# hmakelin/gisnav

Hardware: AMD Instinct MI355X
Metric: matched frame-pairs/sec + PnP poses/sec, 640x480 cam-vs-tile (higher is better)
Workload: dtype f32-accurate FFN / out-projection / match-head GEMMs (each f32 operand split into 2 fp16 terms = 22 significant bits, 3 fp16 MFMA partial products, f32 accumulate; fp16-range guard active); attention INPUT projections (q, k, v: 18 of 66 launches) on 2 partial products -- the fp16 high term of the ac

## Files before the change

gisnav_amd/_lib.py:

```python
from __future__ import annotations

import ctypes as C
import os

HERE = os.path.dirname(os.path.abspath(__file__))
LIB_PATH = os.environ.get("GISNAV_AMD_LIB") or os.path.join(HERE, "libgisnav_amd.so")

c_f32p = C.POINTER(C.c_float)
c_f64p = C.POINTER(C.c_double)
c_i32p = C.POINTER(C.c_int32)
c_i64p = C.POINTER(C.c_int64)
c_u8p = C.POINTER(C.c_uint8)
VP = C.c_void_p

SIGNATURES = {
    "gn_version": (C.c_char_p, []),
    "gn_last_error": (C.c_char_p, [VP]),
    "gn_create": (C.c_int, [C.c_int, C.c_int, C.c_int, C.c_int, C.POINTER(VP)]),
    "gn_create_ex": (C.c_int, [C.c_int, C.c_int, C.c_int, C.c_int, C.c_int, C.POINTER(VP)]),
    "gn_set_image_size": (C.c_int, [VP, C.c_float, C.c_float, C.c_float, C.c_float]),
    "gn_resize": (C.c_int, [VP, C.c_int]),
    "gn_destroy": (None, [VP]),
    "gn_load_tensor": (C.c_int, [VP, C.c_char_p, VP, c_i64p, C.c_int]),
    "gn_missing_tensors": (C.c_int, [VP]),
# ... 13 lines not shown
                                    VP, VP, VP, VP, C.c_double, VP, VP, VP, VP]),
    "gn_estimate_cov": (C.c_int, [VP, C.c_int, C.c_int, VP, VP, VP, C.c_int, VP, VP, VP, C.c_int, VP, C.c_int, C.c_int,
                                  c_f64p, C.c_int, VP, VP, VP, VP, VP, C.c_double, VP, VP, VP, VP]),
    "gn_pnp_ransac_report": (C.c_int, [VP, C.c_int, VP, VP, VP, C.c_int, c_f64p, C.c_int, C.c_float, C.c_double, C.c_int,
                                       VP, VP, VP, VP, C.c_double, VP, VP, VP, VP, VP, VP, VP]),
    "gn_estimate_report": (C.c_int, [VP, C.c_int, C.c_int, VP, VP, VP, C.c_int, VP, VP, VP, C.c_int, VP, C.c_int, C.c_int,
                                     c_f64p, C.c_int, VP, VP, VP, VP, VP, C.c_double, VP, VP, VP, VP, VP, VP, VP, VP, VP]),
    "gn_set_distortion": (C.c_int, [VP, c_f64p, C.c_int]),
    "gn_get_distortion": (C.c_int, [VP, c_f64p]),
    "gn_gather_points_scored": (C.c_int, [VP, C.c_int, C.c_int, VP, C.c_int, VP, C.c_int, VP, VP, VP, VP, C.c_int, C.c_int, VP, VP, VP]),
    "gn_set_dem_format": (C.c_int, [VP, C.c_int, C.c_double, C.c_double, C.c_int, C.c_double]),
    "gn_get_dem_format": (C.c_int, [VP, C.POINTER(C.c_int), c_f64p, c_f64p, C.POINTER(C.c_int), c_f64p]),
    "gn_dem_last_dropped": (C.c_int, [VP, C.c_int, c_i32p, VP]),
    "gn_set_ransac": (C.c_int, [VP, C.c_int, C.c_float, C.c_double]),
    "gn_get_ransac": (C.c_int, [VP, C.POINTER(C.c_int), c_f32p, c_f64p]),
    "gn_ransac_last_counts": (C.c_int, [VP, C.c_int, c_i32p, c_i32p, VP]),
    "gn_undistort_points": (C.c_int, [VP, C.c_int, VP, VP, C.c_int, c_f64p, C.c_int, VP, VP]),
    "gn_set_pair_cameras": (C.c_int, [VP, VP, C.c_int, C.c_int]),
    "gn_get_pair_cameras": (C.c_int, [VP, C.POINTER(VP), C.POINTER(C.c_int), C.POINTER(C.c_int)]),
    "gn_set_overlap": (C.c_int, [VP, C.c_int]),
    "gn_flush": (C.c_int, [VP, VP]),
    "gn_set_substreams": (C.c_int, [VP, C.c_int]),
    "gn_set_active_kpts": (C.c_int, [VP, C.c_int]),
    "gn_set_deferred_join": (C.c_int, [VP, C.c_int]),
    "gn_set_guard": (C.c_int, [VP, C.c_int]),
    "gn_get_guard_status": (C.c_int, [VP, VP, C.POINTER(C.c_int32), C.POINTER(C.c_int64)]),
    "gn_set_certify": (C.c_int, [VP, C.c_int, C.c_float, C.c_float]),
    "gn_set_ffn_products": (C.c_int, [VP, C.c_int]),
    "gn_get_ffn_level": (C.c_int, [VP, C.POINTER(C.c_int32), c_f32p, c_f32p, c_i64p]),
    "gn_set_ffn_level_eps": (C.c_int, [VP, C.c_float, C.c_float, C.c_int]),
    "gn_get_ffn_level1": (C.c_int, [VP, c_f32p, c_i64p]),
    "gn_set_ffn_level_eps1": (C.c_int, [VP, C.c_float]),
    "gn_debug_ffn_level_sim": (C.c_int, [C.c_int, C.c_int, VP, VP, VP, C.c_int, VP, VP]),
    "gn_fused_projection_status": (C.c_int, [VP]),
    "gn_device_numa_node": (C.c_int, [C.c_int]),
    "gn_get_certify_stats": (C.c_int, [VP, c_i64p]),
    "gn_reset_certify_stats": (C.c_int, [VP]),
    "gn_set_certify_ladder": (C.c_int, [VP, C.c_int, C.c_float]),
    "gn_get_certify_ladder_stats": (C.c_int, [VP, c_i64p]),
    "gn_calibrate_certify": (C.c_int, [VP, C.c_int, C.c_int, VP, VP, VP, C.c_int, VP, VP, VP, C.c_int, C.c_float, C.c_float, c_f32p, c_f32p, VP]),
    "gn_get_uncertain": (C.c_int, [VP, C.c_int, c_i32p, VP]),
    "gn_source_digest": (C.c_char_p, []),
    "gn_vo_match": (C.c_int, [VP, C.c_int, VP, VP, C.c_int, VP, VP, C.c_int, C.c_double, VP, VP, VP, VP, VP, VP]),
    "gn_vo_estimate": (C.c_int, [VP, C.c_int, C.c_int, VP, VP, VP, C.c_int, VP, VP, VP, C.c_int, c_f64p, C.c_double, C.c_int,
                                 VP, VP, VP, VP, VP, VP]),
    "gn_vo_estimate_cov": (C.c_int, [VP, C.c_int, C.c_int, VP, VP, VP, C.c_int, VP, VP, VP, C.c_int, c_f64p, C.c_double, C.c_int,
                                     VP, VP, VP, VP, VP, C.c_double, VP, VP, VP, VP]),
    "gn_vo_estimate_report": (C.c_int, [VP, C.c_int, C.c_int, VP, VP, VP, C.c_int, VP, VP, VP, C.c_int, c_f64p, C.c_double, C.c_int,
                                        VP, VP, VP, VP, VP, C.c_double, VP, VP, VP, VP, VP, VP, VP, VP, VP]),
    "gn_rotate_crop_center": (C.c_int, [VP, VP, C.c_int, C.c_int, C.c_double, C.c_int, C.c_int, VP, c_f64p, VP]),
    "gn_stereo_reference_dem": (C.c_int, [VP, VP, VP, C.c_int, C.c_int, C.c_double, C.c_int, C.c_int, C.c_double, C.c_int, C.c_int, VP, VP, c_f64p, VP]),
    "gn_stereo_reference": (C.c_int, [VP, VP, VP, C.c_int, C.c_int, C.c_double, C.c_int, C.c_int, VP, VP, c_f64p, VP]),
    "gn_proj_to_affine": (C.c_int, [C.c_char_p, c_f64p]),
    "gn_wgs84_to_ecef": (C.c_int, [C.c_double, C.c_double, C.c_double, c_f64p]),
    "gn_pose_to_earth": (C.c_int, [c_f64p, c_f64p, c_f64p, C.c_int, C.c_int, c_f64p, c_f64p, c_f64p]),
    "gn_pose_cov_to_camera": (C.c_int, [c_f64p, c_f64p, c_f64p, c_f64p]),
    "gn_pose_cov_to_earth": (C.c_int, [c_f64p, c_f64p, c_f64p, c_f64p, C.c_int, C.c_int, c_f64p]),
    "gn_sift_detect_and_compute": (C.c_int, [VP, VP, C.c_int, C.c_int, C.c_int, VP, VP, VP, VP, C.POINTER(C.c_int32), VP]),
    "gn_sift_detect_and_compute_batch": (C.c_int, [VP, VP, C.c_int, C.c_int, C.c_int, C.c_int, VP, VP, VP, VP, C.POINTER(C.c_int32), VP]),
    "gn_sift_last_totals": (C.c_int, [VP, C.c_int, C.POINTER(C.c_int32)]),
    "gn_sift_set_params": (C.c_int, [VP, C.c_int, C.c_double, C.c_double, C.c_double]),
    "gn_sift_get_params": (C.c_int, [VP, C.POINTER(C.c_int), c_f64p, c_f64p, c_f64p]),
    "gn_sp_load_tensor": (C.c_int, [VP, C.c_char_p, VP, c_i64p, C.c_int]),
    "gn_sp_detect_and_describe": (C.c_int, [VP, VP, C.c_int, C.c_int, C.c_int, C.c_int, VP, VP, VP, C.POINTER(C.c_int32), VP]),
    "gn_sp_set_arithmetic": (C.c_int, [VP, C.c_int]),
    "gn_loftr_create": (C.c_int, [C.c_int, C.c_int, C.c_int, C.c_int, C.c_int, C.POINTER(VP)]),
# ... 86 lines not shown
```

gisnav_amd/csrc/gn_api.hip:

```cpp
#include "gn_common.h"

#include <cstdio>
#include <cstring>
#include <cmath>
#include <cctype>
#include <algorithm>
#include <memory>
#include <tuple>

using namespace gn;

namespace {

thread_local std::string g_err;

struct Linear { float* w = nullptr; float* b = nullptr; int out = 0, in = 0; uint16_t* wp = nullptr; float acc_scale = 1.f;
                uint16_t* wf = nullptr; int frag_order = -1;
                uint16_t* wf2 = nullptr;
                uint16_t* wfn = nullptr; };

struct Block {
  Linear proj_in;
  Linear proj_out;
  Linear ffn0;
// ... 44 lines not shown
  o.B = n;
  pair_arrays(o, [&](size_t bytes, bool, auto*& p) { if (p) p = byte_offset(p, b0 * bytes); }, o);
  return o;
}

template <typename... T> struct Restore {
  std::tuple<T&...> ref; std::tuple<T...> val;
  explicit Restore(T&... r) : ref(r...), val(r...) {}
  ~Restore() { ref = val; }
  Restore(const Restore&) = delete;
  Restore& operator=(const Restore&) = delete;
};

enum { kWsAlways = 1, kWsF16x2 = 2 , kWsNotF32 = 4 , kWsFirstUse = 8 , kWsPnpStage = 16  };
inline long long lists_stride_of(long long km) { return gn::kTileListBase + 2 * (km / 128) + 8 * ((km + 255) / 256); }
#define GN_WORKSPACES(X)                                                                                                         \
  X(float, desc, T2 * kInDim, kWsAlways, "desc") X(float, cos_t, T2 * kFreq, kWsAlways, "cos") X(float, sin_t, T2 * kFreq, kWsAlways, "sin") \
  X(float, extent, 4, kWsAlways, "extent") X(int32_t, nvalid, 2, kWsAlways, "nvalid")                                            \
  X(float, x, T2 * kDim, kWsAlways, "x") X(float, qkv, T2 * 3 * kDim, kWsAlways, "qkv") X(float, ctx, T2 * kDim, kWsAlways, "ctx") \
  X(float, msg, T2 * kDim, kWsAlways, "msg") X(float, h, T2 * 2 * kDim, kWsAlways, "h") X(float, md, T2 * kDim, kWsAlways, "md") \
  X(float, ls, T2, kWsAlways, "ls")                                                                                              \
            \
  X(uint16_t, desc_p, 2 * T2 * kInDim, kWsF16x2, "desc_p") X(uint16_t, x_p, 2 * T2 * kDim, kWsF16x2, "x_p")                      \
  X(uint16_t, ctx_p, 2 * T2 * kDim, kWsF16x2, nullptr) X(uint16_t, msg_p, 2 * T2 * kDim, kWsF16x2, "msg_p")                      \
  X(uint16_t, h_p, 2 * T2 * 2 * kDim, kWsF16x2, nullptr) X(uint16_t, md_p, 2 * T2 * kDim, kWsF16x2, nullptr)                     \
   \
  X(float, rot4, slicing ? T2 * 4 : T2 * 2 * kFreq, kWsF16x2, "rot4")                                                            \
  X(uint16_t, qkb, T2 * 2 * kDim, kWsNotF32, "qkb") X(uint16_t, vtb, T2 * kDim, kWsNotF32, "vtb")  \
   \
  X(float, rowmax, np, kWsAlways, "rowmax") X(float, rowlog, np, kWsAlways, "rowlog") X(float, colmax, np, kWsAlways, "colmax")  \
  X(float, collog, np, kWsAlways, "collog") X(float, max0, np, kWsAlways, "max0") X(int32_t, m0, np, kWsAlways, "m0")            \
  X(int32_t, m1, np, kWsAlways, "m1") X(float, max0b, np, kWsAlways, "max0b") X(float, rpart_c, 8 * np, kWsAlways, nullptr)      \
  X(int32_t, uncert, 1, kWsAlways, "uncert") X(int32_t, uncert_alt, 1, kWsAlways, nullptr) X(int32_t, uncert_alt2, 1, kWsAlways, nullptr) \
  X(float, colbest, np, kWsAlways, nullptr) X(float, col2, np, kWsAlways, nullptr)                                               \
                 \
  X(float, cpart_m, (np / 32) * np, kWsAlways, nullptr) X(float, cpart_s, (np / 32) * np, kWsAlways, nullptr)                    \
  X(int32_t, cpart_i, (np / 32) * np, kWsAlways, nullptr) X(float, rpart_a, 8 * np, kWsAlways, nullptr)                          \
  X(float, rpart_b, 8 * np, kWsAlways, nullptr) X(unsigned int, tickets, 2, kWsAlways, nullptr)                                  \
     \
  X(int64_t, e_idx, km * 2, kWsAlways, nullptr) X(float, e_score, km, kWsAlways, "e_score") X(float, e_mkp, km * 2, kWsAlways, "e_mkp") \
  X(float, e_obj, km * 3, kWsAlways, "e_obj") X(uint8_t, mask_ws, km * 16, kWsAlways, nullptr) X(float, pts_ws, km * 5, kWsAlways, nullptr) \
  X(gn::HypResult, hyp_ws, 16, kWsAlways, "hyp")                                                                                 \
   \
  X(int32_t, dem_dropped, 1, kWsAlways, "dem_dropped")                                                                           \
                             \
  X(uint8_t, rmask_ws, km * (gn::kRansacRound + 1), kWsAlways, "ransac_mask") X(gn::RansacState, rstate_ws, 1, kWsAlways, "ransac_state") \
  X(int, lists, lists_stride_of(km), kWsAlways, "lists")  \
   \
  X(int32_t, pr_ind, T2, kWsAlways, "prune_ind") X(int32_t, pr_prune, T2, kWsAlways, nullptr) X(int32_t, pr_dst, T2, kWsAlways, nullptr) \
  X(int32_t, pr_counts, 2 * kMaxLayers, kWsAlways, "prune_counts") X(int32_t, pr_nin, 2, kWsAlways, nullptr) X(float, pr_z, T2, kWsAlways, "prune_z") \
     \
  X(float, sim, np * np, kWsFirstUse, "sim")                                                                                     \
                                                    \
  X(float, o_mkp0, km * 2, kWsPnpStage, nullptr) X(float, o_obj0, km * 3, kWsPnpStage, nullptr) X(int32_t, o_nmatch0, 1, kWsPnpStage, nullptr) \
  X(float, o_mkp1, km * 2, kWsPnpStage, nullptr) X(float, o_obj1, km * 3, kWsPnpStage, nullptr) X(int32_t, o_nmatch1, 1, kWsPnpStage, nullptr) \
           \
  X(double, o_cams0, GN_PAIR_CAMERA_DOUBLES, kWsPnpStage, nullptr) X(double, o_cams1, GN_PAIR_CAMERA_DOUBLES, kWsPnpStage, nullptr)

struct Workspace {
#define X(type, field, per_pair, when, name) type* field = nullptr;
  GN_WORKSPACES(X)
#undef X
};
template <typename F> void for_each_workspace(Workspace& w, long long np, long long km, bool slicing, F&& f) {
  const long long T2 = 2 * np;
#define X(type, field, per_pair, when, name) f(w.field, (long long)(per_pair), (int)(when), (const char*)(name));
// ... 68 lines not shown
  std::map<std::string, bool> loaded;
  std::vector<std::string> required;
  Workspace ws;
  size_t Tmax = 0;
  int planes_mode = 0;
  float* attn_part = nullptr; unsigned int* attn_tickets = nullptr;
  int attn_split = 1;
  int attn_variant = 4;
  int stop_after = 0;
  int launch_count = 0;
  int no_planes = 0;
  int dbg_planes = 0;
  uint16_t* dbg_wp = nullptr; size_t dbg_wp_n = 0;
  int dbg_out = 0;
  uint16_t* dbg_yp = nullptr; size_t dbg_yp_n = 0;
  int dbg_vt_skip = 0;
  int dbg_reuse = 0;
  uint16_t* dbg_ap = nullptr; size_t dbg_ap_n = 0;
  int gemm_variant = -1;
  int defer_join = 0, sub_last_B = 0, sub_last_np = 0;
  int sub_serial = 0;
  int cu_mask_mode = 0;
  int use_lists = 1;
  int ncu = 256;
  int fused_proj_status = -1;
  bool fused_proj_pending = true;
  int fused_proj_off = 0;
  int qkv_in_tail = 1;
  int skinny = 1;
  int auto_level = 3; float cert_eps_lvl[2] = {-1.f, -1.f}, cert_eps_one = -1.f; long long auto_pairs = 0, auto_wide = 0, auto_narrow = 0, auto_one = 0, auto_calls_lvl[2] = {0, 0}, auto_calls_one = 0, auto_switches = 0;
  int auto_ok1 = 0;
  int ffn_products = 3;
  int qkv_products = 2;
  unsigned long long* tile_feedback = nullptr;
  int n_sub = 1; hipStream_t sub_s[8] = {}; hipEvent_t ev_fork = nullptr; hipEvent_t ev_join[8] = {}; bool sub_pending[8] = {};
  int overlap = 0; unsigned long long calls = 0;
  hipStream_t s_pnp = nullptr; hipEvent_t ev_gather[2][8] = {}, ev_pnp[2][8] = {}; bool pnp_pending[2][8] = {}, pnp_recorded[2][8] = {};
  hipEvent_t ev_head[8] = {};
  int prep_fused = 1;
  int sift_h = 0, sift_w = 0; std::vector<void*> sift_allocs; SiftPyramid sift_py; float* sift_tmp = nullptr;
  float* sift_dk = nullptr; std::vector<std::vector<float>> sift_kernels; std::vector<int> sift_koff;
  int sift_layers = 3; double sift_contrast = 0.04, sift_edge = 10.0, sift_sigma = 1.6;
  int sift_ws_layers = 0; double sift_ws_sigma = 0.0;
  int4* sift_cand = nullptr; int* sift_counts = nullptr; SiftKeypoint* sift_kp = nullptr;
  int sift_max_cand = 0, sift_max_kp = 0, sift_raw_cap = 0, sift_batch = 0; long long sift_kp_stride = 0;
  std::vector<int32_t> sift_totals;
  struct SpConv { float* wf = nullptr; float* b = nullptr; int cout = 0, cin = 0, taps = 0, cout_pad = 0; bool have_w = false, have_b = false;
                  uint16_t* wfh = nullptr; float acc_scale = 1.f; };
  SpConv sp[12];
  std::vector<void*> sp_allocs; int sp_h = 0, sp_w = 0, sp_chunk = 0, sp_cap = 0, sp_max = 0;
  float *sp_x = nullptr, *sp_y = nullptr, *sp_z = nullptr, *sp_maps[3] = {};
  int *sp_cand = nullptr, *sp_counts = nullptr, *sp_index = nullptr;
  float* vo_norm2 = nullptr; int32_t* vo_nn_idx = nullptr; float* vo_nn_dist = nullptr; uint8_t* vo_good = nullptr;
  std::vector<void*> allocs;
  std::vector<void*> ws_allocs;
  bool timing = false;
  hipEvent_t ev[2 * 128];
  int ev_stage[128]; int n_ev = 0; bool ev_ready = false;
  float stage_ms[ST_COUNT] = {0};
  bool ktiming = false;
  std::vector<hipEvent_t> kev;
  std::vector<double> kflops;
  std::vector<double> kbytes;
  std::vector<int> kclass;
  std::vector<const char*> kname;
  size_t kused = 0;
// ... 173 lines not shown
  GemmArgs g;
  memset(&g, 0, sizeof g);
  g.Wp = L.wp; g.wp_plane = (long long)L.out * L.in; g.acc_scale = L.acc_scale;
  g.A = A; g.lda = lda; g.A2 = nullptr; g.lda2 = 0; g.K1 = L.in;
  g.W = L.w; g.ldw = L.in; g.bias = L.b; g.Y = Y; g.ldy = ldy; g.M = M; g.N = L.out; g.K = L.in;
  return g;
}

static void attn_split(gn_ctx* c, AttnArgs& a) {
  const int blocks = a.npad / 128 * kHeads * a.BS;
  int S = 1;
  while (S < 4 && S < c->attn_split && blocks * S * 2 <= (c->attn_split >= 8 ? 512 : 256) && a.npad / 64 >= 4 * S) S *= 2;
  if (c->attn_part && c->attn_tickets && c->attn_split && c->n_sub <= 1 && S > 1) { a.nsplit = S; a.part = c->attn_part; a.tickets = c->attn_tickets; }
}

void attention(gn_ctx* c, const AttnArgs& a, hipStream_t s) {
  if (c->precision != GN_PREC_F32 && c->attn_f16 == 2) launch_attention_f16x2(a, s);
  else if (c->precision != GN_PREC_F32) launch_attention_bf16(a, s); else launch_attention_f32(a, s);
}

void timed_attention(gn_ctx* c, const AttnArgs& a, bool bf16v2, hipStream_t s) {
  timed_launch(c, s, 1, 4.0 * a.BS * kHeads * (double)a.npad * a.npad * kHeadDim,
               (double)a.BS * a.npad * kDim * (a.qb ? 2.0 + 2.0 + 2.0 : 12.0) + (double)a.BS * a.npad * kDim * 4.0,
               nullptr, [&] { if (bf16v2) launch_attention_bf16_v2(a, s); else attention(c, a, s); });
}

bool qkv_projection_applies(const gn_ctx* c, const View& w, const Block& blk, int T, int np, int vt_perm) {
  return c->planes_mode && c->qkv_fused && blk.proj_in.wf && w.x_p && w.qkb && w.vtb && w.rot4 && T % 128 == 0 && np % 128 == 0 && (vt_perm & 1) &&
         (T / 128 >= 128 || c->qkv_fused == 2);
}
bool skinny_applies(const gn_ctx* c, int T, int np) {
  return (c->skinny & 3) && c->planes_mode && c->x_planes_only && T % 32 == 0 && np > 0 && ((c->skinny & 3) == 2 || T / np <= 4);
}
bool qkv_projection(gn_ctx* c, const View& w, const Block& blk, bool cross, int T, int np, int vt_perm, hipStream_t s) {
  const bool skinny = skinny_applies(c, T, np) && !(c->skinny & 4) && c->qkv_fused && blk.proj_in.wf && w.x_p && w.qkb && w.vtb && w.rot4 && np % 32 == 0 && vt_perm == 1 && !c->qkv_stamps;
  if (!skinny && !qkv_projection_applies(c, w, blk, T, np, vt_perm)) return false;
  QkvArgs q;
  q.xp = w.x_p; q.wf = blk.proj_in.wf; q.acc_scale = blk.proj_in.acc_scale; q.bias = blk.proj_in.b;
  q.rot4 = w.rot4; q.rot_stride = (long long)c->Tmax; q.qkb = w.qkb; q.ldyb = cross ? kDim : 2 * kDim; q.vt = w.vtb; q.npad = np;
  q.qscale = 0.125f; q.scale = 0.35355339059327373f; q.vt_perm = vt_perm; q.T = T;
  q.half_fmt = c->attn_f16; q.ovf = (c->attn_f16 && c->guard) ? w.ovf : nullptr;
  q.tiles = (c->use_lists && w.lists && !c->qkv_stamps) ? w.lists : nullptr;
  q.products = c->qkv_products == 3 ? 3 : 2; q.ncu = c->ncu;
  q.dbg_ts = (c->qkv_stamps && w.sim) ? reinterpret_cast<long long*>(w.sim) : nullptr;
  const double N = cross ? 2.0 * kDim : 3.0 * kDim;
  timed_launch(c, s, 0, 2.0 * T * N * kDim, 4.0 * T * kDim + 2.0 * T * N + 4.0 * N * kDim + (cross ? 0.0 : 2.0 * 4.0 * T * kFreq),
               nullptr, [&] { if (skinny) launch_skinny_qkv(q, cross, s); else launch_qkv(q, cross, s); });
  return true;
}

int build_composed(gn_ctx* ctx, Block& blk) {
  if (!blk.comp_dirty) return GN_OK;
  const Linear &F = blk.ffn0, &P = blk.proj_out;
  if (!ctx->planes_mode || !F.w || !F.b || !P.w || !P.b || F.out != 2 * kDim || F.in != 2 * kDim || P.out != kDim || P.in != kDim) return GN_OK;
  const int H = 2 * kDim, D = kDim;
  std::vector<float> w1((size_t)H * H), b1(H), wo((size_t)D * D), bo(D);
  GN_HIP(hipMemcpy(w1.data(), F.w, w1.size() * 4, hipMemcpyDeviceToHost));
  GN_HIP(hipMemcpy(b1.data(), F.b, b1.size() * 4, hipMemcpyDeviceToHost));
  GN_HIP(hipMemcpy(wo.data(), P.w, wo.size() * 4, hipMemcpyDeviceToHost));
  GN_HIP(hipMemcpy(bo.data(), P.b, bo.size() * 4, hipMemcpyDeviceToHost));
  std::vector<float> wc((size_t)H * H), bc(H);
  std::vector<double> row(D);
  float mx = 0.f;
  for (int h = 0; h < H; ++h) {
    const float* w1h = &w1[(size_t)h * H];
    for (int k = 0; k < D; ++k) { row[k] = 0.0; wc[(size_t)h * H + k] = w1h[k]; }
    double bb = b1[h];
    for (int f = 0; f < D; ++f) {
      const double wm = w1h[D + f];
      const float* wof = &wo[(size_t)f * D];
      for (int k = 0; k < D; ++k) row[k] += wm * wof[k];
      bb += wm * bo[f];
    }
    for (int k = 0; k < D; ++k) wc[(size_t)h * H + D + k] = (float)row[k];
    bc[h] = (float)bb;
    for (int k = 0; k < H; ++k) { const float av = fabsf(wc[(size_t)h * H + k]); if (av > mx) mx = av; }
// ... 7 lines not shown
  if (!blk.wfc) { int rc = dalloc(ctx, &blk.wfc, frag.size()); if (rc != GN_OK) return rc; }
  if (!blk.b1c) { int rc = dalloc(ctx, &blk.b1c, (size_t)H); if (rc != GN_OK) return rc; }
  GN_HIP(hipMemcpy(blk.wfc, frag.data(), frag.size() * sizeof(uint16_t), hipMemcpyHostToDevice));
  GN_HIP(hipMemcpy(blk.b1c, bc.data(), bc.size() * sizeof(float), hipMemcpyHostToDevice));
  blk.wfc_scale = ldexpf(1.0f, -e);
  blk.comp_dirty = false;
  return GN_OK;
}

int ensure_composed(gn_ctx* ctx) {
  if (!ctx->planes_mode || !ctx->ffn_compose) return GN_OK;
  for (int i = 0; i < ctx->n_layers; ++i) {
    int rc = build_composed(ctx, ctx->self_blk[i]); if (rc != GN_OK) return rc;
    rc = build_composed(ctx, ctx->cross_blk[i]); if (rc != GN_OK) return rc;
  }
  return GN_OK;
}

bool tail_folds_out_proj(const gn_ctx* c, const Block& blk, int T) {
  return c->planes_mode && c->x_planes_only && c->ffn_fused == 3 && c->ffn_fold && blk.ffn0.wf && blk.ffn0.wf2 && blk.ffn3.wf && blk.proj_out.wf &&
         T % 64 == 0 && c->precision != GN_PREC_F32 && c->attn_variant >= 1;
}

bool tail_should_walk(const gn_ctx* c, int g) {
  if (!c->tile_feedback) return false;
  const unsigned long long word = __atomic_load_n(&c->tile_feedback[g], __ATOMIC_RELAXED);
  const unsigned all = (unsigned)(word >> 32), valid = (unsigned)word;
  return all > 0 && (unsigned long long)valid * 10u < (unsigned long long)all * 9u;
}

inline bool ffn_auto(const gn_ctx* c) { return c->ffn_products == 0 && c->cert_eps_lvl[0] >= 0.f && c->cert_eps_lvl[1] >= 0.f && c->certify >= 2; }
inline int ffn_level(const gn_ctx* c) { return c->attn_f16 == 2 ? 3 : c->ffn_products == 0 ? (ffn_auto(c) ? c->auto_level : 3) : c->ffn_products; }
inline float ffn_level_eps(const gn_ctx* c, int lvl) { return lvl == 1 ? c->cert_eps_one : c->cert_eps_lvl[lvl - 2]; }
inline float cert_eps_now(const gn_ctx* c) { return ffn_auto(c) ? ffn_level_eps(c, c->auto_level) : c->cert_eps; }
inline int ffn_alt_level(int lvl, int k) { return lvl == 1 ? 2 + k : (k == 0 ? 5 - lvl : 1); }
inline void ffn_window_reset(gn_ctx* c, int level) { c->auto_level = level; c->auto_pairs = c->auto_wide = c->auto_narrow = c->auto_one = 0; c->auto_ok1 = 0; }

bool ffn(gn_ctx* c, const View& w, const Block& blk, int T, hipStream_t s, bool keep_f32, const Block* next = nullptr, bool next_cross = false, int np = 0, int vt_perm = 0) {
  if (skinny_applies(c, T, np) && !(c->skinny & 8) && c->ffn_fused == 3 && c->ffn_compose && tail_folds_out_proj(c, blk, T) && blk.wfc && blk.b1c && !blk.comp_dirty && blk.ffn3.wfn &&
      w.h && w.ctx_p && gn::g_ffn_stamps == 0 && gn::g_ffn_shape == 0) {
    SkinnyTailArgs a;
    a.xp = w.x_p; a.cp = w.ctx_p; a.w1 = blk.wfc; a.w1_scale = blk.wfc_scale; a.b1 = blk.b1c; a.h = w.h; a.ln_g = blk.ln_g; a.ln_b = blk.ln_b;
    a.w2 = blk.ffn3.wfn; a.w2_scale = blk.ffn3.acc_scale; a.b2 = blk.ffn3.b; a.xp_out = w.x_p; a.y = keep_f32 ? w.x : nullptr;
    a.ovf = c->guard ? w.ovf : nullptr; a.T = T;
    if (!timed_launch(c, s, 0, 2.0 * T * 512.0 * 512.0, 4.0 * T * (256.0 + 256.0 + 512.0) + 4.0 * 512.0 * 512.0, nullptr, [&] { launch_skinny_h(a, s, c->skinny >> 4); })) return false;
    timed_launch(c, s, 0, 2.0 * T * 256.0 * 512.0, 4.0 * T * (512.0 + 256.0 + 256.0) + 4.0 * 256.0 * 512.0, nullptr, [&] { launch_skinny_out(a, s, c->skinny >> 4); });
    return false;
  }
  if (c->planes_mode && c->x_planes_only && c->ffn_fused == 3 && blk.ffn0.wf && blk.ffn3.wf && T % 64 == 0) {
    FfnArgs f;
    const bool fold = tail_folds_out_proj(c, blk, T);
    f.cp = fold ? w.ctx_p : nullptr; f.wos = blk.proj_out.wf; f.wo_scale = blk.proj_out.acc_scale; f.bo = blk.proj_out.b;
    f.xp = w.x_p; f.mp = w.msg_p; f.w1s = fold ? blk.ffn0.wf2 : blk.ffn0.wf; f.w1_scale = blk.ffn0.acc_scale; f.b1 = blk.ffn0.b; f.ln_g = blk.ln_g; f.ln_b = blk.ln_b;
    f.w2s = blk.ffn3.wf; f.w2_scale = blk.ffn3.acc_scale; f.b2 = blk.ffn3.b; f.yp = w.x_p; f.y = keep_f32 ? w.x : nullptr; f.T = T;
    const bool comp = fold && c->ffn_compose && blk.wfc && blk.b1c && !blk.comp_dirty;
    if (comp) { f.composed = 1; f.w1s = blk.wfc; f.w1_scale = blk.wfc_scale; f.b1 = blk.b1c; }
    f.ovf = c->guard ? w.ovf : nullptr;
    f.tiles = (c->use_lists && w.lists && gn::g_ffn_stamps == 0) ? w.lists : nullptr;
    f.walk = c->use_lists == 2 || (c->use_lists == 1 && tail_should_walk(c, w.g));
    f.ncu = c->ncu;
    f.composed = comp ? 1 : 0;
    f.products = (comp && ffn_level(c) <= 2) ? ffn_level(c) : 3;
    const bool fuse_qkv = next != nullptr && c->qkv_in_tail && !c->fused_proj_off && comp && ffn_selects_128(f) && gn::g_ffn_stamps == 0 && c->attn_f16 && c->qkv_products != 3 && !c->qkv_stamps &&
                          c->precision != GN_PREC_F32 && c->attn_variant >= 1 && qkv_projection_applies(c, w, *next, T, np, vt_perm) && !(vt_perm & 2);
    if (fuse_qkv) {
      f.qkv = next_cross ? 2 : 1;
      f.q_wf = next->proj_in.wf; f.q_acc_scale = next->proj_in.acc_scale; f.q_bias = next->proj_in.b;
      f.q_rot4 = w.rot4; f.q_rot_stride = (long long)c->Tmax; f.q_qkb = w.qkb; f.q_vt = w.vtb;
      f.q_qscale = 0.125f; f.q_scale = 0.35355339059327373f;
      f.npad = np;
    }
    if (c->use_lists) { f.nvalid = w.nvalid; f.npad = c->npad_run; }
    f.dbg_ts = gn::g_ffn_stamps ? reinterpret_cast<long long*>(w.sim) : nullptr;
    double flops = 2.0 * T * (512.0 * 512.0 + 256.0 * 512.0 + ((fold && !comp) ? 256.0 * 256.0 : 0.0));
    double bytes = 4.0 * T * (256.0 + 256.0 + 256.0 + 256.0) + 4.0 * (512.0 * 512.0 + 256.0 * 512.0);
    if (fuse_qkv) {
      const double N = next_cross ? 2.0 * kDim : 3.0 * kDim;
      flops += 2.0 * T * N * kDim;
      bytes += 2.0 * T * N + 4.0 * N * kDim + (next_cross ? 0.0 : 2.0 * 4.0 * T * kFreq);
    }
    return timed_launch(c, s, 0, flops, bytes, nullptr, [&] { launch_ffn_fused(f, s); }) && fuse_qkv;
  }
  GemmArgs g = gemm_args(w.x, kDim, blk.ffn0, w.h, 2 * kDim, T);
  g.A2 = w.msg; g.lda2 = kDim; g.K1 = kDim;
  if (c->planes_mode && T % 128 == 0 && (c->ffn_fused == 2 || (c->ffn_fused == 1 && T / 128 >= 256))) {
    g.ln_g = blk.ln_g; g.ln_b = blk.ln_b;
    gemm(c, w, EPI_LN_GELU, g, s);
  } else {
    gemm(c, w, EPI_BIAS, g, s);
    launch_ln_gelu(w.h, blk.ln_g, blk.ln_b, T, s, c->planes_mode ? w.h_p : nullptr, c->planes_mode && c->guard ? w.ovf : nullptr);
  }
  GemmArgs g3 = gemm_args(w.h, 2 * kDim, blk.ffn3, w.x, kDim, T);
  g3.resid = w.x; g3.ldr = kDim;
  if (c->planes_mode && c->x_planes_only) {
    uint16_t* xp = nullptr;
    if (planes_of(c, w, w.x, &xp)) { g3.residp = xp; g3.ldrp = kDim; g3.resid = nullptr; g3.drop_f32 = keep_f32 ? 0 : 1; }
  }
  gemm(c, w, EPI_RESIDUAL, g3, s);
  return false;
// ... 109 lines not shown
      }
      { StageTimer tm(c, s, ST_FFN); qkv_done = ffn(c, w, blk, T, s, i == c->n_layers - 1, (bf16v2 && i + 1 < c->n_layers && !pruning) ? &c->self_blk[i + 1] : nullptr, false, np, vt_perm); }
      if (pruning && i + 1 < c->n_layers && !(c->stop_after && c->launch_count >= c->stop_after)) {
        StageTimer tm(c, s, ST_PREP);
        const bool planes_only = c->planes_mode && c->x_planes_only;
        PruneArgs pa;
        pa.x = planes_only ? nullptr : w.x; pa.xp = c->planes_mode ? w.x_p : nullptr; pa.z_from_planes = planes_only ? 1 : 0;
        pa.cos_t = w.cos_t; pa.sin_t = w.sin_t; pa.rot4 = w.rot4; pa.rot_stride = (long long)c->Tmax;
        pa.ind = w.pr_ind; pa.prune = w.pr_prune; pa.dst = w.pr_dst; pa.nvalid = w.nvalid; pa.counts = w.pr_counts; pa.layer = i; pa.z = w.pr_z;
        pa.w = c->matchability[i].w; pa.b = c->matchability[i].b; pa.thresh = 1.0f - c->width_conf; pa.min_kpts = c->prune_min_kpts; pa.BS = BS; pa.npad = np;
        timed_launch(c, s, 0, 2.0 * T * kDim, (double)T * (pa.x ? 3.0 : 0.0) * 4.0 * kDim + (double)T * (pa.xp ? 3.0 : 0.0) * 4.0 * kDim, "k_prune", [&] { launch_prune(pa, s); });
        if (c->use_lists && w.lists) launch_tile_lists(w.nvalid, BS, np, w.lists, nullptr, s);
      }
    }
  }
  {
    StageTimer tm(c, s, ST_HEAD);
    const int li = c->n_layers - 1;
    GemmArgs g = gemm_args(w.x, kDim, c->final_proj[li], w.md, kDim, T);
    g.scale = 0.25f; g.scale_cols = kDim;
    gemm(c, w, EPI_SCALE_COLS, g, s);
    launch_matchability(w.x, c->matchability[li].w, c->matchability[li].b, w.ls, T, s);
    HeadArgs hd;
    hd.n_in = pruning ? w.pr_nin : nullptr;
    hd.sim = w.sim; hd.ls = w.ls; hd.nvalid = w.nvalid; hd.B = B; hd.npad = np; hd.threshold = c->threshold;
    hd.rowmax = w.rowmax; hd.rowlog = w.rowlog; hd.colmax = w.colmax; hd.collog = w.collog;
    hd.m0 = w.m0; hd.max0 = w.max0; hd.m1 = w.m1;
    hd.ovf = (c->planes_mode && c->guard) ? w.ovf : nullptr;
    hd.max0b = w.max0b; hd.rpart_c = w.rpart_c; hd.uncert = c->certify ? w.uncert : nullptr;
    hd.cert_eps = (c->precision == GN_PREC_F32) ? c->cert_eps_f32 : cert_eps_now(c);
    if (hd.uncert && c->precision != GN_PREC_F32 && ffn_auto(c)) {
      hd.uncert_alt = w.uncert_alt; hd.cert_eps_alt = ffn_level_eps(c, ffn_alt_level(c->auto_level, 0));
      hd.uncert_alt2 = w.uncert_alt2; hd.cert_eps_alt2 = ffn_level_eps(c, ffn_alt_level(c->auto_level, 1));
    }
    hd.idx = v.idx; hd.score = v.score; hd.n_match = v.n_match; hd.kmax = c->npad;
    hd.md = c->planes_mode ? (const void*)w.md_p : (const void*)w.md; hd.md_f32 = c->planes_mode ? 0 : 1;
    hd.cpart_m = w.cpart_m; hd.cpart_s = w.cpart_s; hd.cpart_i = w.cpart_i; hd.rpart_a = w.rpart_a; hd.rpart_b = w.rpart_b; hd.tickets = w.tickets;
    hd.dbg_ts = (c->head_stamps && w.sim) ? reinterpret_cast<long long*>(w.sim) : nullptr;
    if (c->cal_cols) { hd.colbest = w.colbest; hd.col2 = w.col2; }
    if (c->head_fused || !w.sim) {
      timed_launch(c, s, 0, 2.0 * 2.0 * B * (double)np * np * kDim,
                   2.0 * (4.0 * T * kDim) + 4.0 * T * 4.0 + 8.0 * B * np * 3.0,
                   "k_head_fused (2 sweeps)", [&] { launch_match_head_fused(hd, s); });
      if (pruning) launch_unprune_idx(v.idx, v.n_match, w.pr_ind, B, np, c->npad, s);
      return GN_OK;
    }
    GemmArgs gs;
    memset(&gs, 0, sizeof gs);
    gs.A = w.md; gs.lda = kDim; gs.K1 = kDim; gs.W = w.md + (size_t)np * kDim; gs.ldw = kDim;
    gs.Y = w.sim; gs.ldy = np; gs.M = np; gs.N = np; gs.K = kDim; gs.acc_scale = 1.f;
    gs.strideA = gs.strideW = 2LL * np * kDim; gs.strideY = (long long)np * np;
    timed_gemm(c, w, EPI_PLAIN, gs, B, s);
    launch_match_head(hd, s);
    if (pruning) launch_unprune_idx(v.idx, v.n_match, w.pr_ind, B, np, c->npad, s);
  }
  return GN_OK;
}

int alloc_workspaces(gn_ctx* ctx, int when) {
  int rc = GN_OK;
  for_each_workspace(ctx->ws, ctx->npad, ctx->npad, false, [&](auto*& p, long long per_pair, int exists, const char*) {
    if (rc == GN_OK && (exists & when)) rc = ws_alloc(ctx, &p, (size_t)ctx->max_batch * per_pair);
  });
  return rc;
}

// ... 17 lines not shown
  if (ctx->precision == GN_PREC_F16X2_BF16_ATTN) ctx->planes_mode = 1;
  int rc = alloc_workspaces(ctx, kWsAlways | (ctx->planes_mode ? kWsF16x2 : 0) | (ctx->precision != GN_PREC_F32 ? kWsNotF32 : 0) | (ctx->s_pnp ? kWsPnpStage : 0));
  if (rc == GN_OK && ctx->precision != GN_PREC_F32) rc = ws_alloc(ctx, &ctx->attn_part, (size_t)256 * 4 * 34 * 64);
  if (rc == GN_OK && ctx->precision != GN_PREC_F32) rc = ws_alloc(ctx, &ctx->attn_tickets, 256);
  if (rc == GN_OK) rc = ws_alloc(ctx, &ctx->vo_norm2, T);
  if (rc == GN_OK) rc = ws_alloc(ctx, &ctx->vo_nn_idx, B * np * 2);
  if (rc == GN_OK) rc = ws_alloc(ctx, &ctx->vo_nn_dist, B * np * 2);
  if (rc == GN_OK) rc = ws_alloc(ctx, &ctx->vo_good, B * np);
  if (rc == GN_OK) rc = ws_alloc(ctx, &ctx->ovf_base, 16);
  ctx->last_pnp_valid = false;
  ctx->prune_last_np = 0; ctx->prune_last_B = 0; ctx->prune_last_on = false;
  return rc;
}

__global__ void k_count_diff(const uint4* a, const uint4* b, size_t n, unsigned int* cnt) {
  bool d = false;
  for (size_t i = (size_t)blockIdx.x * blockDim.x + threadIdx.x; i < n; i += (size_t)gridDim.x * blockDim.x) {
    const uint4 x = a[i], y = b[i];
    d |= (x.x != y.x) | (x.y != y.y) | (x.z != y.z) | (x.w != y.w);
  }
  const unsigned long long bal = __ballot(d);
  if ((threadIdx.x & 63) == 0 && bal) atomicAdd(cnt, (unsigned int)__popcll(bal));
}

int selfcheck_fused_projection(gn_ctx* c) {
  gn_ctx* ctx = c;
  const View w = view_of(c);
  c->fused_proj_pending = false;
  c->fused_proj_status = -1;
  c->fused_proj_off = 0;
  const int np = c->npad;
  GN_HIP(hipDeviceSynchronize());
  if (!c->planes_mode || !c->qkv_in_tail || !c->attn_f16 || c->attn_f16 == 2 || c->qkv_products == 3 || !c->ffn_compose || c->ffn_fused != 3 || !c->x_planes_only || c->n_layers < 1 ||
      !c->qkv_fused || !w.rot4 || !w.lists || !w.msg_p || !w.h_p || c->feature < 0 || gn::g_ffn_stamps != 0 || gn::g_ffn_shape != 0) return GN_OK;
  int B = (256 * 128 + 2 * np - 1) / (2 * np);
  if (B > c->max_batch) return GN_OK;
  const int T = B * 2 * np;
  std::vector<float> h((size_t)T * kDim);
  unsigned long long st = 0x9E3779B97F4A7C15ull;
  auto rnd = [&]() { st ^= st << 13; st ^= st >> 7; st ^= st << 17; return (float)((st >> 40) & 0xFFFF) * (1.0f / 32768.0f) - 1.0f; };
  for (int pass = 0; pass < 2; ++pass) {
    for (auto& v : h) v = 1.5f * rnd();
    float* dst = pass == 0 ? w.x : w.ctx;
    GN_HIP(hipMemcpy(dst, h.data(), h.size() * sizeof(float), hipMemcpyHostToDevice));
    launch_split_hm16(dst, pass == 0 ? w.x_p : w.ctx_p, T, kDim, 1.0f, 0);
  }
  {
    std::vector<float> cs((size_t)T * kFreq), sn((size_t)T * kFreq);
    for (size_t i = 0; i < cs.size(); ++i) { const float th = 3.14159265f * rnd(); cs[i] = cosf(th); sn[i] = sinf(th); }
    GN_HIP(hipMemcpy(w.cos_t, cs.data(), cs.size() * sizeof(float), hipMemcpyHostToDevice));
    GN_HIP(hipMemcpy(w.sin_t, sn.data(), sn.size() * sizeof(float), hipMemcpyHostToDevice));
    launch_rot_table(w.cos_t, w.sin_t, w.rot4, T, (long long)c->Tmax, 0);
    std::vector<int32_t> nv(2 * (size_t)B, np);
    GN_HIP(hipMemcpy(w.nvalid, nv.data(), nv.size() * sizeof(int32_t), hipMemcpyHostToDevice));
    launch_tile_lists(w.nvalid, 2 * B, np, w.lists, nullptr, 0);
  }
  const size_t xbytes = (size_t)T * kDim * 4, qbytes = (size_t)T * 2 * kDim * 2, vbytes = (size_t)T * kDim * 2;
  uint16_t* const keep_q = w.h_p;
  uint16_t* const keep_v = w.h_p + (size_t)T * 2 * kDim;
  GN_HIP(hipMemcpy(w.msg_p, w.x_p, xbytes, hipMemcpyDeviceToDevice));
  unsigned int* cnt = c->ovf_base + 12;
  GN_HIP(hipMemset(cnt, 0, sizeof(unsigned int)));
  bool applicable = true;
  {
    const Restore keep(c->use_lists, c->qkv_in_tail, c->guard, c->ktiming, c->launch_count, c->stop_after, c->npad_run, c->ffn_products);
    const int prod0 = c->ffn_products;
    c->ktiming = false; c->stop_after = 0; c->guard = 0; c->npad_run = np;
    const int nblk = c->n_layers > 1 ? 1 : 0;
    const int lvs[3] = {3, prod0 == 1 ? 1 : 2, 1};
    const int n_lv = prod0 == 0 ? 3 : (prod0 == 2 || prod0 == 1) ? 2 : 1;
    for (int lv = 0; lv < n_lv && applicable; ++lv)
    for (int cross = 0; cross < 2 && applicable; ++cross)
      for (int walk = 0; walk < 2 && applicable; ++walk) {
        c->ffn_products = lvs[lv];
        const Block& tail = cross ? c->self_blk[0] : c->cross_blk[0];
        const Block* next = cross ? &c->cross_blk[0] : &c->self_blk[nblk];
        c->use_lists = walk ? 2 : 3;
        GN_HIP(hipMemcpyAsync(w.x_p, w.msg_p, xbytes, hipMemcpyDeviceToDevice, 0));
        GN_HIP(hipMemsetAsync(w.qkb, 0, qbytes, 0)); GN_HIP(hipMemsetAsync(w.vtb, 0, vbytes, 0));
        c->qkv_in_tail = 1;
        if (!ffn(c, w, tail, T, 0, false, next, cross != 0, np, 1)) { applicable = false; break; }
        GN_HIP(hipMemcpyAsync(keep_q, w.qkb, qbytes, hipMemcpyDeviceToDevice, 0));
        GN_HIP(hipMemcpyAsync(keep_v, w.vtb, vbytes, hipMemcpyDeviceToDevice, 0));
        GN_HIP(hipMemcpyAsync(w.x_p, w.msg_p, xbytes, hipMemcpyDeviceToDevice, 0));
        GN_HIP(hipMemsetAsync(w.qkb, 0, qbytes, 0)); GN_HIP(hipMemsetAsync(w.vtb, 0, vbytes, 0));
        c->qkv_in_tail = 0;
        ffn(c, w, tail, T, 0, false, next, cross != 0, np, 1);
        if (!qkv_projection(c, w, *next, cross != 0, T, np, 1, 0)) { applicable = false; break; }
        hipLaunchKernelGGL(k_count_diff, dim3(1024), dim3(256), 0, 0, reinterpret_cast<const uint4*>(keep_q), reinterpret_cast<const uint4*>(w.qkb), (cross ? qbytes / 2 : qbytes) / 16, cnt);
        hipLaunchKernelGGL(k_count_diff, dim3(1024), dim3(256), 0, 0, reinterpret_cast<const uint4*>(keep_v), reinterpret_cast<const uint4*>(w.vtb), vbytes / 16, cnt);
      }
  }
  unsigned int diffs = 0;
  GN_HIP(hipStreamSynchronize(0));
  GN_HIP(hipMemcpy(&diffs, cnt, sizeof diffs, hipMemcpyDeviceToHost));
  GN_HIP(hipMemset(w.x_p, 0, xbytes)); GN_HIP(hipMemset(w.ctx_p, 0, xbytes)); GN_HIP(hipMemset(w.msg_p, 0, xbytes)); GN_HIP(hipMemset(w.h_p, 0, qbytes + vbytes));
  GN_HIP(hipMemset(w.qkb, 0, qbytes)); GN_HIP(hipMemset(w.vtb, 0, vbytes)); GN_HIP(hipMemset(w.x, 0, xbytes)); GN_HIP(hipMemset(w.ctx, 0, xbytes));
  GN_HIP(hipMemset(cnt, 0, sizeof(unsigned int)));
  if (!applicable) return GN_OK;
  c->fused_proj_status = diffs == 0 ? 1 : 0;
  if (diffs != 0) {
    c->fused_proj_off = 1;
    fprintf(stderr, "[gisnav_amd] the projection fused behind the block tail differs from the separate k_qkv launches in %u 16-byte words on this context's weights: "
                    "fusion switched off for this context (results stay correct, ~4 %% slower)\n", diffs);
  }
  return GN_OK;
}

int ffn_level_next(int level, int* ok1_run, long long pairs, long long n1, long long n2, long long n3, bool have1) {
  const bool ok2 = (n2 - n3) * 64 <= pairs, ok1 = have1 && (n1 - n3) * 64 <= pairs;
  int next = level;
  if (level == 3) next = ok2 ? 2 : 3;
  else if (level == 2) {
    if (!ok2) next = 3;
    else { *ok1_run = ok1 ? *ok1_run + 1 : 0; next = *ok1_run >= 2 ? 1 : 2; }
  } else next = ok1 ? 1 : (ok2 ? 2 : 3);
  if (next != 2) *ok1_run = 0;
  return next;
}

void ffn_level_update(gn_ctx* c, int B, const int32_t* flags, const int32_t* alt, const int32_t* alt2, int lvl) {
  if (!ffn_auto(c) || c->precision == GN_PREC_F32 || lvl < 1 || lvl > 3) return;
  ++(lvl == 1 ? c->auto_calls_one : c->auto_calls_lvl[lvl - 2]);
  int n[4] = {0, 0, 0, 0};
  const int la = ffn_alt_level(lvl, 0), lb = ffn_alt_level(lvl, 1);
  for (int b = 0; b < B; ++b) { n[lvl] += flags[b] == 1; n[la] += alt[b] == 1; n[lb] += alt2[b] == 1; }
  c->auto_pairs += B; c->auto_one += n[1]; c->auto_wide += n[2]; c->auto_narrow += n[3];
  if (c->auto_pairs < 64) return;
  const int next = ffn_level_next(c->auto_level, &c->auto_ok1, c->auto_pairs, c->auto_one, c->auto_wide, c->auto_narrow, c->cert_eps_one >= 0.f);
  if (next != c->auto_level) ++c->auto_switches;
  c->auto_level = next;
  c->auto_pairs = c->auto_wide = c->auto_narrow = c->auto_one = 0;
}

struct ExactF32 : Restore<int, int, int, int, int> {
  explicit ExactF32(gn_ctx* c) : Restore(c->precision, c->planes_mode, c->gemm_variant, c->no_planes, c->attn_f16) {
    c->precision = GN_PREC_F32; c->planes_mode = 0; c->gemm_variant = 3; c->no_planes = 1; c->attn_f16 = 0;
  }
};
struct MidLevel : Restore<int, int, int, float> {
  explicit MidLevel(gn_ctx* c) : Restore(c->attn_f16, c->ffn_products, c->dbg_trip_group, c->cert_eps) {
    c->attn_f16 = 2; c->ffn_products = 3; c->dbg_trip_group = 0; c->cert_eps = c->cert_eps_mid;
  }
};
struct F32x3 : Restore<int, int, int, int> {
  explicit F32x3(gn_ctx* c) : Restore(c->planes_mode, c->gemm_variant, c->no_planes, c->attn_f16) {
    c->planes_mode = 0; c->gemm_variant = 5; c->no_planes = 1; c->attn_f16 = 0;
  }
};
inline bool ladder_active(const gn_ctx* c) { return c->ladder && c->cert_eps_mid >= 0.f && c->precision != GN_PREC_F32 && c->planes_mode && c->attn_f16 != 2; }

template <typename F> int rerun_pairs(gn_ctx* ctx, hipStream_t s, const Call& v, F& run, const std::vector<int>& flagged, std::vector<int32_t>& rflags) {
  const int nf = (int)flagged.size();
  const bool contiguous = flagged.back() - flagged.front() + 1 == nf;
  int rc = GN_OK;
  Call st = slice(v, 0, nf);
  if (!contiguous) {
    auto place = [&](char* base) {
      size_t off = 0;
      pair_arrays(st, [&](size_t bytes, bool, auto*& p) {
        if (!p) return;
        if (base) p = reinterpret_cast<std::remove_reference_t<decltype(p)>>(base + off);
        off = (off + nf * bytes + 255) & ~(size_t)255;
      }, st);
      return off;
// ... 8 lines not shown
  }
  auto copy_pair = [&](const Call& dst, size_t bd, const Call& src, size_t bs, bool outputs) {
    hipError_t e = hipSuccess;
    pair_arrays(v, [&](size_t bytes, bool out, auto* d, auto* q) {
      if (d && out == outputs && e == hipSuccess)
        e = hipMemcpyAsync(const_cast<void*>(static_cast<const void*>(byte_offset(d, bd * bytes))), byte_offset(q, bs * bytes), bytes, hipMemcpyDeviceToDevice, s);
    }, dst, src);
    return e;
  };
  if (!contiguous)
    for (int k = 0; k < nf; ++k) GN_HIP(copy_pair(st, k, v, flagged[k], false));
  {
    const Restore keep(ctx->cert_inner, ctx->in_group);
    ctx->cert_inner = true; ctx->in_group = true;
    rc = contiguous ? run(view_of(ctx, flagged.front()), slice(v, flagged.front(), nf)) : run(view_of(ctx), st);
  }
  if (rc != GN_OK) return rc;
  if (!contiguous)
    for (int k = 0; k < nf; ++k) GN_HIP(copy_pair(v, flagged[k], st, k, true));
  GN_HIP(hipMemcpyAsync(ctx->uncert_host, ctx->ws.uncert, (size_t)v.B * sizeof(int32_t), hipMemcpyDeviceToHost, s));
  GN_HIP(hipStreamSynchronize(s));
  rflags.resize(nf);
  for (int k = 0; k < nf; ++k) rflags[k] = ctx->uncert_host[contiguous ? flagged[k] : k];
  return GN_OK;
}

template <typename F> int certify_rerun(gn_ctx* ctx, hipStream_t s, const Call& v, F&& run, const int32_t* flags_ready = nullptr, int flags_level = 0) {
  const int B = v.B;
  if (!flags_ready) {
    GN_HIP(hipMemcpyAsync(ctx->uncert_host, ctx->ws.uncert, (size_t)B * sizeof(int32_t), hipMemcpyDeviceToHost, s));
    if (ffn_auto(ctx)) {
      GN_HIP(hipMemcpyAsync(ctx->uncert_host + ctx->max_batch, ctx->ws.uncert_alt, (size_t)B * sizeof(int32_t), hipMemcpyDeviceToHost, s));
      GN_HIP(hipMemcpyAsync(ctx->uncert_host + 2 * ctx->max_batch, ctx->ws.uncert_alt2, (size_t)B * sizeof(int32_t), hipMemcpyDeviceToHost, s));
    }
    GN_HIP(hipStreamSynchronize(s));
    flags_ready = ctx->uncert_host;
  }
  ffn_level_update(ctx, B, flags_ready, flags_ready + ctx->max_batch, flags_ready + 2 * ctx->max_batch, flags_level ? flags_level : ctx->auto_level);
  ++ctx->cert_calls; ctx->cert_pairs += B;
  std::vector<int> flagged, margin;
  for (int b = 0; b < B; ++b) {
    const int f = flags_ready[b];
    if (f == 1) ++ctx->cert_flag_margin; else if (f == 2) ++ctx->cert_flag_range;
    if (f != 0) flagged.push_back(b);
    if (f == 1) margin.push_back(b);
  }
  if (flagged.empty()) return GN_OK;
  if (ctx->precision == GN_PREC_F32) { ctx->cert_f32_marginal += (long long)flagged.size(); return GN_OK; }
  std::vector<int32_t> rflags;
  if (ladder_active(ctx) && !margin.empty()) {
    std::vector<int> still(flagged.size() - margin.size());
    std::copy_if(flagged.begin(), flagged.end(), still.begin(), [&](int b) { return flags_ready[b] != 1; });
    int rc = GN_OK;
    { const MidLevel mid(ctx); rc = rerun_pairs(ctx, s, v, run, margin, rflags); }
    if (rc != GN_OK) return rc;
    ctx->mid_rerun += (long long)margin.size();
    for (size_t k = 0; k < margin.size(); ++k) {
      if (rflags[k] == 0) ++ctx->mid_certified;
      else { ++ctx->mid_passed; still.push_back(margin[k]); }
    }
    std::sort(still.begin(), still.end());
    flagged.swap(still);
    if (flagged.empty()) return GN_OK;
  }
  int rc = GN_OK;
  { const ExactF32 f32(ctx); rc = rerun_pairs(ctx, s, v, run, flagged, rflags); }
  ctx->cert_rerun += (long long)flagged.size();
  if (rc != GN_OK) return rc;
  for (int32_t f : rflags) if (f != 0) ++ctx->cert_f32_marginal;
  return GN_OK;
}

enum { kCalExactF32 = 0, kCalMid = -1 };
struct CalPass { std::vector<float> best, second, colbest, col2; unsigned int trip = 0u; };
int cal_pass(gn_ctx* ctx, const Call& w, int arith, bool cols, std::vector<int32_t>* nv, CalPass& out, hipStream_t s) {
  const View vw = view_of(ctx);
  int rc = GN_OK;
  {
    const Restore keep(ctx->in_group, ctx->cal_cols, ctx->ffn_products);
    ctx->in_group = true;
    ctx->cal_cols = cols;
    if (arith == kCalExactF32) { const ExactF32 f32(ctx); rc = run_matcher(ctx, vw, w, s); }
    else if (arith == kCalMid) { const MidLevel mid(ctx); rc = run_matcher(ctx, vw, w, s); }
    else { ctx->ffn_products = arith; rc = run_matcher(ctx, vw, w, s); }
  }
  if (rc != GN_OK) return rc;
  const size_t n = (size_t)w.B * ctx->npad_run;
  out.best.resize(n); out.second.resize(n);
  if (cols) { out.colbest.resize(n); out.col2.resize(n); }
  auto get = [&](void* dst, const void* src, size_t bytes) { return hipMemcpy(dst, src, bytes, hipMemcpyDeviceToHost) == hipSuccess; };
  const bool ok = hipStreamSynchronize(s) == hipSuccess && get(out.best.data(), vw.max0, n * 4) && get(out.second.data(), vw.max0b, n * 4) &&
                  (!nv || get(nv->data(), vw.nvalid, nv->size() * 4)) &&
                  (!cols || (get(out.colbest.data(), vw.colbest, n * 4) && get(out.col2.data(), vw.col2, n * 4))) &&
                  (arith == kCalExactF32 || !ctx->planes_mode || !ctx->guard || get(&out.trip, vw.ovf, 4));
  return ok ? GN_OK : GN_ERR_HIP;
}

double max_diff(const CalPass& a, const CalPass& e, const std::vector<int32_t>& nv, int Bp, size_t np, bool cols, float L, long long* entries = nullptr) {
  double mx = 0.0, mx_all = 0.0; long long n_near = 0, n_all = 0;
  auto take = [&](float bm, float be, float sm, float se) {
    const double d1 = std::fabs((double)bm - be), d2 = std::fabs((double)sm - se);
    const double d = std::max(std::isfinite(d1) ? d1 : (double)INFINITY, std::isfinite(d2) ? d2 : 0.0);
    ++n_all; mx_all = std::max(mx_all, d);
    if (std::max(bm, be) >= L - 1.f) { ++n_near; mx = std::max(mx, d); }
  };
  for (int b = 0; b < Bp; ++b) {
    const int n0 = nv[2 * b], n1 = nv[2 * b + 1];
    if (n0 < 2 || n1 < 2) continue;
    for (int i = 0; i < n0; ++i) { const size_t o = (size_t)b * np + i; take(a.best[o], e.best[o], a.second[o], e.second[o]); }
    for (int j = 0; cols && j < n1; ++j) { const size_t o = (size_t)b * np + j; take(a.colbest[o], e.colbest[o], a.col2[o], e.col2[o]); }
  }
  if (entries) *entries = n_near ? n_near : n_all;
  return n_near ? mx : mx_all;
}

int check_fwd(gn_ctx* ctx, int B, int stride_q, int stride_r) {
  if (!ctx) return fail(nullptr, GN_ERR_ARG, "null context");
// ... 99 lines not shown
    a.dist = ctx->dist_on;
    for (int i = 0; i < 5; ++i) a.dk[i] = ctx->dist[i];
  }
  a.to_pixels = to_pixels ? 1 : 0; a.out = out;
  launch_undistort(a, (hipStream_t)stream);
  GN_HIP(hipGetLastError());
  return GN_OK;
}

int gn_create_ex(int device, int max_batch, int max_kpts, int precision, int feature, gn_ctx** out) {
  gn_ctx* ctx = nullptr;
  if (!out || max_batch < 1 || max_kpts < 2) return fail(nullptr, GN_ERR_ARG, "bad gn_create argument");
  if (precision != GN_PREC_F32 && precision != GN_PREC_BF16_ATTN && precision != GN_PREC_F32X3_BF16_ATTN &&
      precision != GN_PREC_F16X2_BF16_ATTN && precision != GN_PREC_F16X2_F16_ATTN && precision != GN_PREC_F16X2_F16X2_ATTN)
    return fail(nullptr, GN_ERR_ARG, "bad precision");
  if (precision == GN_PREC_F16X2_F16X2_ATTN && feature != GN_FEATURE_SIFT)
    return fail(nullptr, GN_ERR_ARG, "GN_PREC_F16X2_F16X2_ATTN: SIFT-LightGlue contexts only (the SuperPoint extractor has no split-attention schedule)");
  const int precision_api = precision;
  if (precision == GN_PREC_F16X2_F16_ATTN || precision == GN_PREC_F16X2_F16X2_ATTN) precision = GN_PREC_F16X2_BF16_ATTN;
  GN_HIP(hipSetDevice(device));
  hipDeviceProp_t prop;
  GN_HIP(hipGetDeviceProperties(&prop, device));
  if (strncmp(prop.gcnArchName, "gfx950", 6) != 0)
    return fail(nullptr, GN_ERR_ARCH, std::string("device is ") + prop.gcnArchName + ", this library is built for gfx950 only");
  ctx = new gn_ctx();
  if (feature != GN_FEATURE_SIFT && feature != GN_FEATURE_SUPERPOINT) { delete ctx; return fail(nullptr, GN_ERR_ARG, "bad feature type"); }
  ctx->device = device; ctx->max_batch = max_batch; ctx->precision = precision; ctx->feature = feature;
  ctx->precision_api = precision_api; ctx->attn_f16 = precision_api == GN_PREC_F16X2_F16_ATTN ? 1 : precision_api == GN_PREC_F16X2_F16X2_ATTN ? 2 : 0;
  ctx->gemm_variant = precision == GN_PREC_F16X2_BF16_ATTN ? 6 : precision == GN_PREC_F32X3_BF16_ATTN ? 5 : 3;
  { const int rc_ws = alloc_workspace(ctx, max_kpts); if (rc_ws != GN_OK) { gn_destroy(ctx); return rc_ws; } }
  if (hipHostMalloc((void**)&ctx->ovf_host, (16 + 4096 + 16) * sizeof(unsigned int), hipHostMallocDefault) != hipSuccess) { gn_destroy(ctx); return fail(nullptr, GN_ERR_HIP, "hipHostMalloc failed"); }
  memset(ctx->ovf_host, 0, (16 + 4096 + 16) * sizeof(unsigned int));
  ctx->tile_feedback = reinterpret_cast<unsigned long long*>(ctx->ovf_host + 16 + 4096);
  if (hipHostMalloc((void**)&ctx->uncert_host, (size_t)3 * max_batch * sizeof(int32_t), hipHostMallocDefault) != hipSuccess) { gn_destroy(ctx); return fail(nullptr, GN_ERR_HIP, "hipHostMalloc failed"); }
  memset(ctx->uncert_host, 0, (size_t)3 * max_batch * sizeof(int32_t));
  for (auto& pd : ctx->cert_pend) {
    if (hipHostMalloc((void**)&pd.flags, (size_t)3 * max_batch * sizeof(int32_t), hipHostMallocDefault) != hipSuccess ||
        hipEventCreateWithFlags(&pd.ev, hipEventDisableTiming) != hipSuccess) { gn_destroy(ctx); return fail(nullptr, GN_ERR_HIP, "certificate slots: allocation failed"); }
  }
  ctx->ncu = prop.multiProcessorCount > 0 ? prop.multiProcessorCount : 256;
  for (int i = 0; i < 256; ++i) hipEventCreate(&ctx->ev[i]);
  ctx->ev_ready = true;
  auto req = [&](const std::string& n) { ctx->required.push_back(n + ".weight"); ctx->required.push_back(n + ".bias"); };
  if (feature == GN_FEATURE_SIFT) req("input_proj");
  ctx->required.push_back("posenc.Wr.weight");
  for (int i = 0; i < kMaxLayers; ++i) {
    const std::string ps = "transformers." + std::to_string(i) + ".self_attn.", pc = "transformers." + std::to_string(i) + ".cross_attn.";
    req(ps + "Wqkv"); req(ps + "out_proj"); req(ps + "ffn.0"); req(ps + "ffn.1"); req(ps + "ffn.3");
    req(pc + "to_qk"); req(pc + "to_v"); req(pc + "to_out"); req(pc + "ffn.0"); req(pc + "ffn.1"); req(pc + "ffn.3");
    req("log_assignment." + std::to_string(i) + ".final_proj");
    req("log_assignment." + std::to_string(i) + ".matchability");
  }
  *out = ctx;
  return GN_OK;
}

int gn_resize(gn_ctx* ctx, int max_kpts) {
  if (!ctx || max_kpts < 2) return fail(ctx, GN_ERR_ARG, "bad gn_resize argument");
  if (((max_kpts + 127) / 128) * 128 == ctx->npad) return GN_OK;
  GN_HIP(hipSetDevice(ctx->device));
  GN_HIP(hipDeviceSynchronize());
  for (void* p : ctx->ws_allocs) hipFree(p);
  ctx->ws_allocs.clear();
  for (bool& b : ctx->sub_pending) b = false;
  auto broken = [&](int rc) { for (void* p : ctx->ws_allocs) hipFree(p); ctx->ws_allocs.clear(); ctx->npad = 0; ctx->npad_run = 0; return rc; };
  { const int rc = alloc_workspace(ctx, max_kpts); if (rc != GN_OK) return broken(rc); }
  if (ctx->s_pnp) for (auto& slot : ctx->pnp_pending) for (bool& b : slot) b = false;
  return GN_OK;
}

// ... 154 lines not shown
          for (int s3 = 0; s3 < 3; ++s3) {
            const int src = hh * 192 + d * 3 + s3, dst = s3 * kDim + hh * kHeadDim + d;
            memcpy(&tmp[(size_t)dst * in], host + (size_t)src * in, in * sizeof(float));
          }
      Linear& L = blk.proj_in;
      L.frag_order = 0;
      if (is_w) { rc = upload(&L.w, tmp.data(), tmp.size()); } else { rc = upload(&L.b, tmp.data(), tmp.size()); }
      L.out = 3 * kDim; L.in = kDim;
      if (is_w && rc == GN_OK) rc = build_planes(ctx, L);
    } else if (self && leaf == "out_proj") { blk.comp_dirty = true; blk.proj_out.frag_order = 0; rc = load_linear(blk.proj_out, kDim, kDim, 0, kDim); }
    else if (cross && leaf == "to_qk") { blk.proj_in.frag_order = 0; rc = load_linear(blk.proj_in, kDim, kDim, 0, 2 * kDim); }
    else if (cross && leaf == "to_v") { blk.proj_in.frag_order = 0; rc = load_linear(blk.proj_in, kDim, kDim, kDim, 2 * kDim); }
    else if (cross && leaf == "to_out") { blk.comp_dirty = true; blk.proj_out.frag_order = 0; rc = load_linear(blk.proj_out, kDim, kDim, 0, kDim); }
    else if (leaf == "ffn.0") { blk.comp_dirty = true; blk.ffn0.frag_order = 0; rc = load_linear(blk.ffn0, 2 * kDim, 2 * kDim, 0, 2 * kDim); }
    else if (leaf == "ffn.3") { blk.ffn3.frag_order = 1; rc = load_linear(blk.ffn3, kDim, 2 * kDim, 0, kDim); }
    else if (leaf == "ffn.1") {
      if (d0 != 2 * kDim || d1 != 1) return shape_err();
      rc = upload(is_w ? &blk.ln_g : &blk.ln_b, host, 2 * kDim);
    } else return fail(ctx, GN_ERR_NAME, "unknown tensor " + name);
  } else if (base.compare(0, 15, "log_assignment.") == 0) {
    const int i = atoi(base.c_str() + 15);
    if (i < 0 || i >= kMaxLayers) return fail(ctx, GN_ERR_NAME, "layer index out of range in " + name);
    const std::string leaf = base.substr(base.find('.', 15) + 1);
    if (leaf == "final_proj") rc = load_linear(ctx->final_proj[i], kDim, kDim, 0, kDim);
    else if (leaf == "matchability") {
      if (is_w) { if (ndim != 2 || d0 != 1 || d1 != kDim) return shape_err(); rc = upload(&ctx->matchability[i].w, host, kDim); }
      else { if (d0 != 1) return shape_err(); rc = upload(&ctx->matchability[i].b, host, 1); }
    } else return fail(ctx, GN_ERR_NAME, "unknown tensor " + name);
  } else {
    return fail(ctx, GN_ERR_NAME, "unknown tensor " + name);
  }
  if (rc == GN_OK) {
    ctx->loaded[name] = true; ctx->fused_proj_pending = true;
    ctx->cert_eps_lvl[0] = ctx->cert_eps_lvl[1] = ctx->cert_eps_one = -1.f; ffn_window_reset(ctx, 3);
    ctx->cert_eps_mid = -1.f;
    if (ctx->cert_eps_src >= 2) { ctx->cert_eps = INFINITY; ctx->cert_eps_src = 3; }
  }
  return rc;
}

namespace {
int match_impl(gn_ctx* ctx, const View& vw, int B, int kpt_format,
               const float* desc_q, const float* kpt_q, const int32_t* n_q, int stride_q,
               const float* desc_r, const float* kpt_r, const int32_t* n_r, int stride_r,
               int64_t* idx, float* score, int32_t* n_match, void* stream) {
  int rc = check_fwd(ctx, B, stride_q, stride_r);
  if (rc != GN_OK) return rc;
  const int kfmt = kpt_format & 0xff;
  if (kfmt != GN_KPT_LAF && kfmt != GN_KPT_XYSA && kfmt != GN_KPT_RECORD) return fail(ctx, GN_ERR_ARG, "bad kpt_format");
  if (kfmt == GN_KPT_RECORD && ctx->feature != GN_FEATURE_SIFT) return fail(ctx, GN_ERR_ARG, "GN_KPT_RECORD (KEYPOINT_DTYPE wire records) needs a SIFT context");
  if (((!desc_q || !desc_r) && kfmt != GN_KPT_RECORD) || !kpt_q || !n_q || !kpt_r || !n_r || !idx || !score || !n_match)
    return fail(ctx, GN_ERR_ARG, "null pointer passed to gn_match");
  hipStream_t s = (hipStream_t)stream;
  ctx->n_ev = 0;
  if (!ctx->in_group) ctx->ovf_groups_last = 1;
  Call v(ctx->feature, ctx->npad, B, kpt_format, desc_q, kpt_q, n_q, stride_q, desc_r, kpt_r, n_r, stride_r);
  v.idx = idx; v.score = score; v.n_match = n_match;
  rc = run_matcher(ctx, vw, v, s);
  if (rc != GN_OK) return rc;
  if (ctx->certify >= 2 && !ctx->in_group && !ctx->cert_inner) {
    rc = certify_rerun(ctx, s, v, [&](const View& rw, const Call& w) { return run_matcher(ctx, rw, w, s); });
    if (rc != GN_OK) return rc;
  } else if (ctx->planes_mode && ctx->guard == 2 && ctx->certify < 2) {
    GN_HIP(hipMemcpyAsync(ctx->ovf_host, vw.ovf, sizeof(unsigned int), hipMemcpyDeviceToHost, s));
    GN_HIP(hipStreamSynchronize(s));
    if (*ctx->ovf_host != 0u) {
      ++ctx->guard_trips;
// ... 45 lines not shown
  for (char* c = bus; *c; ++c) *c = (char)tolower((unsigned char)*c);
  const std::string path = std::string("/sys/bus/pci/devices/") + bus + "/numa_node";
  FILE* f = fopen(path.c_str(), "r");
  if (!f) return -1;
  int node = -1;
  if (fscanf(f, "%d", &node) != 1) node = -1;
  fclose(f);
  return node;
}

int gn_fused_projection_status(const gn_ctx* ctx) { return ctx ? ctx->fused_proj_status : GN_ERR_ARG; }

int gn_set_ffn_products(gn_ctx* ctx, int products) {
  if (!ctx || products < 0 || products > 3) return GN_ERR_ARG;
  if (products != ctx->ffn_products) {
    ffn_window_reset(ctx, 3);
    ctx->fused_proj_pending = true;
  }
  ctx->ffn_products = products;
  return GN_OK;
}

int gn_set_ffn_level_eps(gn_ctx* ctx, float eps2, float eps3, int level) {
  if (!ctx || !(eps2 >= 0.f) || !(eps3 >= 0.f) || level < 1 || level > 3) return GN_ERR_ARG;
  ctx->cert_eps_lvl[0] = std::max(eps2, eps3); ctx->cert_eps_lvl[1] = eps3;
  if (ctx->cert_eps_one >= 0.f) ctx->cert_eps_one = std::max(ctx->cert_eps_one, ctx->cert_eps_lvl[0]);
  ffn_window_reset(ctx, (level == 1 && !(ctx->cert_eps_one >= 0.f)) ? 2 : level);
  return GN_OK;
}

int gn_set_ffn_level_eps1(gn_ctx* ctx, float eps1) {
  if (!ctx || !(eps1 >= 0.f)) return GN_ERR_ARG;
  ctx->cert_eps_one = std::max(eps1, std::max(ctx->cert_eps_lvl[0], ctx->cert_eps_lvl[1]));
  return GN_OK;
}

int gn_get_ffn_level1(gn_ctx* ctx, float* eps1, int64_t* calls1) {
  if (!ctx) return GN_ERR_ARG;
  if (eps1) *eps1 = ctx->cert_eps_one;
  if (calls1) *calls1 = ctx->auto_calls_one;
  return GN_OK;
}

int gn_debug_ffn_level_sim(int n_calls, int B, const int32_t* f1, const int32_t* f2, const int32_t* f3, int have1, int32_t* levels_out, int64_t* out4) {
  if (n_calls < 0 || B < 1 || !f1 || !f2 || !f3) return GN_ERR_ARG;
  std::unique_ptr<gn_ctx> c(new gn_ctx);
  c->ffn_products = 0; c->certify = 2; c->precision = GN_PREC_F16X2_BF16_ATTN;
  c->cert_eps_lvl[0] = 2.f; c->cert_eps_lvl[1] = 1.f; c->cert_eps_one = have1 ? 3.f : -1.f;
  const int32_t* f[4] = {nullptr, f1, f2, f3};
  for (int i = 0; i < n_calls; ++i) {
    const int lvl = c->auto_level;
    if (levels_out) levels_out[i] = lvl;
    const size_t o = (size_t)i * B;
    ffn_level_update(c.get(), B, f[lvl] + o, f[ffn_alt_level(lvl, 0)] + o, f[ffn_alt_level(lvl, 1)] + o, lvl);
  }
  if (out4) { out4[0] = c->auto_level; out4[1] = c->auto_switches; out4[2] = c->auto_calls_lvl[0]; out4[3] = c->auto_calls_one; }
  return GN_OK;
}

int gn_get_ffn_level(gn_ctx* ctx, int32_t* level, float* eps2, float* eps3, int64_t* out4) {
  if (!ctx) return GN_ERR_ARG;
  if (level) *level = ffn_level(ctx);
  if (eps2) *eps2 = ctx->cert_eps_lvl[0];
  if (eps3) *eps3 = ctx->cert_eps_lvl[1];
  if (out4) { out4[0] = ctx->auto_calls_lvl[0]; out4[1] = ctx->auto_calls_lvl[1]; out4[2] = ctx->auto_switches; out4[3] = ffn_auto(ctx) ? 1 : 0; }
  return GN_OK;
}

int gn_set_certify(gn_ctx* ctx, int mode, float eps, float eps_f32) {
  if (!ctx || mode < 0 || mode > 3) return GN_ERR_ARG;
  if (ctx->certify == 3 && mode != 3 && (ctx->cert_pend[0].active || ctx->cert_pend[1].active))
    return fail(ctx, GN_ERR_ARG, "gn_set_certify: deferred certificates are still open -- gn_flush first");
  if (mode > 0 && ctx->width_conf > 0.f)
    return fail(ctx, GN_ERR_ARG, "gn_set_certify: the margin certificate cannot run with point pruning on (gn_set_width_pruning): its eps bounds |P - P_f32| on the same "
                                 "token set, and a fast mode may prune a different set -- gn_set_width_pruning(ctx, -1, -1) first");
  ctx->certify = mode;
  if (eps >= 0.f) { ctx->cert_eps = eps; ctx->cert_eps_src = 1; }
  if (eps_f32 >= 0.f) ctx->cert_eps_f32 = eps_f32;
  return GN_OK;
}

int gn_calibrate_certify(gn_ctx* ctx, int B, int kpt_format,
                         const float* desc_q, const float* kpt_q, const int32_t* n_q, int stride_q,
                         const float* desc_r, const float* kpt_r, const int32_t* n_r, int stride_r,
                         float safety, float floor_eps, float* measured_host, float* eps_host, void* stream) {
  int rc = check_fwd(ctx, B, stride_q, stride_r);
  if (rc != GN_OK) return rc;
  if (!(safety >= 1.f) || !(floor_eps >= 0.f)) return fail(ctx, GN_ERR_ARG, "gn_calibrate_certify: safety must be >= 1, floor_eps >= 0");
  if (ctx->precision == GN_PREC_F32) return fail(ctx, GN_ERR_ARG, "gn_calibrate_certify: this context already computes in exact f32");
  if (ctx->width_conf > 0.f)
    return fail(ctx, GN_ERR_ARG, "gn_calibrate_certify: point pruning is on (gn_set_width_pruning): the measured eps would compare scores of different token sets -- "
                                 "gn_set_width_pruning(ctx, -1, -1) first");
  if (ctx->n_sub > 1 || ctx->overlap) { const int rcf = gn_flush(ctx, stream); if (rcf != GN_OK) return rcf; }
  hipStream_t s = (hipStream_t)stream;
  const size_t np = (size_t)ctx->npad_run;
  int32_t* nm = nullptr;
  GN_HIP(hipMalloc((void**)&nm, (size_t)B * sizeof(int32_t)));
  Call v(ctx->feature, ctx->npad, B, kpt_format, desc_q, kpt_q, n_q, stride_q, desc_r, kpt_r, n_r, stride_r);
  v.idx = ctx->ws.e_idx; v.score = ctx->ws.e_score; v.n_match = nm;
  const int setting = ctx->ffn_products;
  const int n_lv = setting == 0 ? 3 : 1;
  const int lv[3] = {setting == 0 ? 1 : setting, 2, 3};
  const float L = ctx->threshold > 0.f ? logf(ctx->threshold) : -INFINITY;
  CalPass whole[4];
  std::vector<int32_t> nv(2 * (size_t)B);
  unsigned int tripped = 0u;
  const bool lad = ctx->ladder && ctx->planes_mode && ctx->attn_f16 != 2;
  for (int pass = 0; pass <= n_lv && rc == GN_OK; ++pass) {
    rc = cal_pass(ctx, v, pass == n_lv ? kCalExactF32 : lv[pass], pass == n_lv && lad, &nv, whole[pass], s);
    tripped |= whole[pass].trip;
  }
  double mid_mx = -1.0;
  for (int mp = 0; lad && mp < 2 && rc == GN_OK && !tripped; ++mp) {
    CalPass mid;
    rc = cal_pass(ctx, slice(v, 0, mp == 0 ? B : 1), kCalMid, true, nullptr, mid, s);
    if (rc != GN_OK) break;
    tripped |= mid.trip;
    mid_mx = std::max(mid_mx, max_diff(mid, whole[n_lv], nv, mp == 0 ? B : 1, np, true, L));
  }
  double var_mx[3] = {0.0, 0.0, 0.0};
  int32_t* nr1 = nullptr;
  if (rc == GN_OK && !tripped && nv[0] >= 2 && nv[1] >= 2 && hipMalloc((void**)&nr1, sizeof(int32_t)) != hipSuccess) rc = GN_ERR_HIP;
  Call v1 = slice(v, 0, 1);
  v1.n_r = nr1;
  for (int var = 0; nr1 && rc == GN_OK && var < 3; ++var) {
    const int32_t nr_cut = var == 0 ? nv[1] : std::min(nv[1], var == 1 ? 128 : 2);
    if (hipMemcpy(nr1, &nr_cut, sizeof nr_cut, hipMemcpyHostToDevice) != hipSuccess) { rc = GN_ERR_HIP; break; }
    CalPass p[4];
    unsigned int trip = 0u;
    for (int pass = 0; pass <= n_lv && rc == GN_OK; ++pass) {
      rc = cal_pass(ctx, v1, pass == n_lv ? kCalExactF32 : lv[pass], false, nullptr, p[pass], s);
      trip |= p[pass].trip;
    }
    if (rc != GN_OK || trip) continue;
    for (int k = 0; k < n_lv; ++k) var_mx[k] = std::max(var_mx[k], max_diff(p[k], p[n_lv], nv, 1, np, false, L));
  }
  if (nr1) hipFree(nr1);
  hipFree(nm);
  if (rc != GN_OK) return rc == GN_ERR_HIP ? fail(ctx, rc, "gn_calibrate_certify: a HIP call failed") : rc;
  if (tripped) return fail(ctx, GN_ERR_ARG, "gn_calibrate_certify: the sample left the fp16 range of this precision mode (nothing to calibrate: such calls are re-run as a whole)");
  float eps_of[3] = {0.f, 0.f, 0.f}, mx_of[3] = {0.f, 0.f, 0.f};
  for (int k = 0; k < n_lv; ++k) {
    long long rows = 0;
    double mx = max_diff(whole[k], whole[n_lv], nv, B, np, false, L, &rows);
    if (!std::isfinite(mx)) return fail(ctx, GN_ERR_ARG, "gn_calibrate_certify: non-finite scores in the sample");
    if (rows == 0) return fail(ctx, GN_ERR_ARG, "gn_calibrate_certify: the sample holds no pair with at least two keypoints per side (nothing to measure)");
    if (!std::isfinite(var_mx[k])) return fail(ctx, GN_ERR_ARG, "gn_calibrate_certify: non-finite scores in the one-pair passes");
    mx = std::max(mx, var_mx[k]);
    mx_of[k] = (float)mx; eps_of[k] = std::max(floor_eps, safety * (float)mx);
  }
  if (setting == 0) {
    ctx->cert_eps_lvl[1] = eps_of[2]; ctx->cert_eps_lvl[0] = std::max(eps_of[1], eps_of[2]); ctx->cert_eps_one = std::max(eps_of[0], ctx->cert_eps_lvl[0]);
    ffn_window_reset(ctx, 3);
  }
  if (lad && mid_mx >= 0.0) {
    if (!std::isfinite(mid_mx)) return fail(ctx, GN_ERR_ARG, "gn_calibrate_certify: non-finite scores in the middle level's pass");
    ctx->cert_eps_mid = std::max(floor_eps, safety * (float)mid_mx);
    ctx->cert_mid_measured = (float)mid_mx;
  }
  const int rep = n_lv - 1;
  ctx->cert_eps = eps_of[rep]; ctx->cert_eps_src = 2;
  if (measured_host) *measured_host = mx_of[rep];
  if (eps_host) *eps_host = eps_of[rep];
  return GN_OK;
}

int gn_get_certify_stats(gn_ctx* ctx, int64_t* out8) {
  if (!ctx || !out8) return GN_ERR_ARG;
  out8[0] = ctx->cert_calls; out8[1] = ctx->cert_pairs; out8[2] = ctx->cert_flag_margin; out8[3] = ctx->cert_flag_range;
  out8[4] = ctx->cert_rerun; out8[5] = ctx->cert_f32_marginal; out8[6] = ctx->certify; out8[7] = ctx->cert_eps_src;
  return GN_OK;
}

int gn_set_certify_ladder(gn_ctx* ctx, int enable, float eps_mid) {
  if (!ctx) return GN_ERR_ARG;
  if (enable && (!ctx->planes_mode || ctx->attn_f16 == 2 || ctx->feature != GN_FEATURE_SIFT))
    return fail(ctx, GN_ERR_ARG, "gn_set_certify_ladder: the ladder needs a SIFT context of GN_PREC_F16X2_BF16_ATTN or GN_PREC_F16X2_F16_ATTN "
                                 "(its middle level is GN_PREC_F16X2_F16X2_ATTN's arithmetic on the same planes; exact f32 has nothing to ladder)");
  ctx->ladder = enable ? 1 : 0;
  if (eps_mid >= 0.f) ctx->cert_eps_mid = eps_mid;
  return GN_OK;
}

int gn_get_certify_ladder_stats(gn_ctx* ctx, int64_t* out4) {
  if (!ctx || !out4) return GN_ERR_ARG;
  uint32_t bits = 0;
  memcpy(&bits, &ctx->cert_eps_mid, sizeof bits);
  out4[0] = ctx->mid_rerun; out4[1] = ctx->mid_certified; out4[2] = ctx->mid_passed; out4[3] = ctx->cert_eps_mid >= 0.f ? (int64_t)bits : -1;
  return GN_OK;
}

int gn_reset_certify_stats(gn_ctx* ctx) {
  if (!ctx) return GN_ERR_ARG;
  ctx->cert_calls = ctx->cert_pairs = ctx->cert_flag_margin = ctx->cert_flag_range = ctx->cert_rerun = ctx->cert_f32_marginal = 0;
  ctx->mid_rerun = ctx->mid_certified = ctx->mid_passed = 0;
  ctx->auto_calls_lvl[0] = ctx->auto_calls_lvl[1] = ctx->auto_calls_one = ctx->auto_switches = 0;
  return GN_OK;
}

int gn_get_uncertain(gn_ctx* ctx, int B, int32_t* host_flags, void* stream) {
  if (!ctx || !host_flags || B < 1 || B > ctx->max_batch) return GN_ERR_ARG;
  if (!ctx->certify) return fail(ctx, GN_ERR_ARG, "gn_get_uncertain: the certificate is off (gn_set_certify)");
  GN_HIP(hipSetDevice(ctx->device));
  GN_HIP(hipMemcpyAsync(ctx->uncert_host, ctx->ws.uncert, (size_t)B * sizeof(int32_t), hipMemcpyDeviceToHost, (hipStream_t)stream));
  GN_HIP(hipStreamSynchronize((hipStream_t)stream));
  memcpy(host_flags, ctx->uncert_host, (size_t)B * sizeof(int32_t));
  return GN_OK;
}

namespace {
int gather_impl(gn_ctx* ctx, const DemFormat& f, int32_t* dropped, int B, int kpt_format, const float* kpt_q, int stride_q, const float* kpt_r, int stride_r,
                int64_t* idx, float* score, int32_t* n_match, const uint8_t* dem, int H, int W, float* mkp_q, float* obj, void* stream) {
  if (!ctx || !kpt_q || !kpt_r || !idx || !n_match || !mkp_q || !obj || B < 1 || B > ctx->max_batch)
    return fail(ctx, GN_ERR_ARG, "bad gn_gather_points argument");
  if (dem && (H < 1 || W < 1)) return fail(ctx, GN_ERR_ARG, "bad DEM shape");
  GN_HIP(hipSetDevice(ctx->device));
  DemGatherArgs d;
  GatherArgs& g = d.g;
  g.kpt_q = kpt_q; g.stride_q = stride_q; g.kpt_r = kpt_r; g.stride_r = stride_r; g.kpt_format = kpt_format & 0xff;
  g.idx = idx; g.n_match = n_match; g.kmax = ctx->npad; g.B = B; g.dem = dem; g.H = H; g.W = W; g.mkp_q = mkp_q; g.obj = obj;
  StageTimer tm(ctx, (hipStream_t)stream, ST_GATHER);
  if (!dem || dem_format_is_default(f)) launch_gather(g, (hipStream_t)stream);
  else {
    d.f = f; d.idx = idx; d.score = score; d.n_match = n_match; d.dropped = dropped;
    launch_gather_dem(d, (hipStream_t)stream);
  }
  GN_HIP(hipGetLastError());
  return GN_OK;
}
// ... 257 lines not shown
  hipStream_t s = (hipStream_t)stream;
  if ((ctx->defer_join || ctx->certify == 3) && (ctx->sub_last_B != B || ctx->sub_last_np != ctx->npad_run)) {
    const int rcj = gn_flush(ctx, stream);
    if (rcj != GN_OK) return rcj;
  }
  ctx->sub_last_B = B; ctx->sub_last_np = ctx->npad_run;
  ctx->prune_last_B = B;
  ctx->ovf_groups_last = groups;
  GN_HIP(hipEventRecord(ctx->ev_fork, s));
  const int slot = (int)(ctx->calls++ & 1);
  if (ctx->certify == 3) { const int rcj = join_pnp(ctx, s); if (rcj != GN_OK) return rcj; }
  int rc_all = GN_OK, b0 = 0;
  for (int g = 0; g < groups; ++g) {
    const int Bg = B / groups + (g < B % groups ? 1 : 0);
    hipStream_t sg = ctx->sub_serial ? ctx->sub_s[0] : ctx->sub_s[g];
    GN_HIP(hipStreamWaitEvent(sg, ctx->ev_fork, 0));
    ctx->in_group = true;
    const int rc = estimate_impl(ctx, view_of(ctx, b0, g), slice(v, b0, Bg), sg, slot);
    ctx->in_group = false;
    if (rc != GN_OK && rc_all == GN_OK) rc_all = rc;
    GN_HIP(hipEventRecord(ctx->ev_join[g], sg));
    ctx->sub_pending[g] = true;
    b0 += Bg;
  }
  if (ctx->certify == 3 && rc_all == GN_OK) {
    for (int g = 0; g < groups; ++g) GN_HIP(hipStreamWaitEvent(s, ctx->ev_head[g], 0));
    const int slot = ctx->cert_slot;
    gn_ctx::CertPending& p = ctx->cert_pend[slot];
    if (p.active) { const int rcr = cert_resolve(ctx, slot, s); if (rcr != GN_OK) return rcr; }
    GN_HIP(hipMemcpyAsync(p.flags, ctx->ws.uncert, (size_t)B * sizeof(int32_t), hipMemcpyDeviceToHost, s));
    if (ffn_auto(ctx)) {
      GN_HIP(hipMemcpyAsync(p.flags + ctx->max_batch, ctx->ws.uncert_alt, (size_t)B * sizeof(int32_t), hipMemcpyDeviceToHost, s));
      GN_HIP(hipMemcpyAsync(p.flags + 2 * ctx->max_batch, ctx->ws.uncert_alt2, (size_t)B * sizeof(int32_t), hipMemcpyDeviceToHost, s));
    } else memset(p.flags + ctx->max_batch, 0, (size_t)2 * ctx->max_batch * sizeof(int32_t));
    GN_HIP(hipEventRecord(p.ev, s));
    p.active = true; p.level = ffn_auto(ctx) ? ctx->auto_level : -1; p.npad_run = ctx->npad_run;
    p.call = v;
    if (K9) { memcpy(p.K9, K9, sizeof p.K9); p.call.K9 = p.K9; }
    ctx->cert_slot ^= 1;
    return cert_resolve(ctx, slot ^ 1, s);
  }
  if (!ctx->defer_join || ctx->certify == 2) { const int rcj = gn_flush(ctx, stream); if (rcj != GN_OK && rc_all == GN_OK) rc_all = rcj; }
  if (ctx->certify == 2 && rc_all == GN_OK) {
    rc_all = certify_rerun(ctx, s, v, [&](const View& rw, const Call& w) { return estimate_impl(ctx, rw, w, s); });
  }
  return rc_all;
}
}

int gn_estimate(gn_ctx* ctx, int B, int kpt_format,
                const float* desc_q, const float* kpt_q, const int32_t* n_q, int stride_q,
                const float* desc_r, const float* kpt_r, const int32_t* n_r, int stride_r,
                const uint8_t* dem, int H, int W, const double* K9, int min_matches,
                double* R, double* t, int32_t* n_match, int32_t* n_inliers, uint8_t* ok, void* stream) {
  return estimate_call(ctx, B, kpt_format, desc_q, kpt_q, n_q, stride_q, desc_r, kpt_r, n_r, stride_r, dem, H, W, K9, min_matches,
                       R, t, n_match, n_inliers, ok, 0.0, nullptr, nullptr, nullptr, stream);
}

int gn_estimate_cov(gn_ctx* ctx, int B, int kpt_format,
                    const float* desc_q, const float* kpt_q, const int32_t* n_q, int stride_q,
                    const float* desc_r, const float* kpt_r, const int32_t* n_r, int stride_r,
                    const uint8_t* dem, int H, int W, const double* K9, int min_matches,
                    double* R, double* t, int32_t* n_match, int32_t* n_inliers, uint8_t* ok,
                    double sigma_px, double* cov_rt, double* sigma_hat, uint8_t* cov_ok, void* stream) {
  if (!cov_rt || !sigma_hat || !cov_ok) return fail(ctx, GN_ERR_ARG, "gn_estimate_cov: null covariance output");
  return estimate_call(ctx, B, kpt_format, desc_q, kpt_q, n_q, stride_q, desc_r, kpt_r, n_r, stride_r, dem, H, W, K9, min_matches,
                       R, t, n_match, n_inliers, ok, sigma_px, cov_rt, sigma_hat, cov_ok, stream);
}

// ... 673 lines not shown
  else if (which == 5) ctx->planes_mode = (value && ctx->ws.x_p) ? 1 : 0;
  else if (which == 6) ctx->dbg_reuse = value;
  else if (which == 7) ctx->dbg_out = value;
  else if (which == 10) ctx->ffn_fused = value;
  else if (which == 11) ctx->x_planes_only = value;
  else if (which == 8) gn::g_p2_wide = value;
  else if (which == 9) ctx->dbg_vt_skip = value;
  else if (which == 12) gn::g_ffn_stamps = value;
  else if (which == 13) ctx->ffn_fold = value;
  else if (which == 14) gn::g_ffn_shape = value;
  else if (which == 15) ctx->pnp_stamps = value;
  else if (which == 16) ctx->head_fused = value;
  else if (which == 17) ctx->head_stamps = value;
  else if (which == 19) ctx->qkv_fused = value;
  else if (which == 20) ctx->qkv_stamps = value;
  else if (which == 21) ctx->sp_split = value;
  else if (which == 34) gn::g_sp_conv_s = value;
  else if (which == 40) gn::g_sp_select_stream = value;
  else if (which == 41) gn::g_gemm_m64 = value;
  else if (which == 42) gn::g_lf_conv_knob = value;
  else if (which == 43) gn::g_attn_f32_ks = value;
  else if (which == 44) gn::g_gemm_r64 = value;
  else if (which == 46) gn::g_sp_fuse1 = value;
  else if (which == 47) { ctx->fused_proj_pending = value == 0; }
  else if (which == 39) ctx->sp_stop = value;
  else if (which == 35) {
    ctx->sp_ts_layer = value;
    if (value > 0 && ctx->sp_ts == nullptr) { void* q = nullptr; if (hipMalloc(&q, (size_t)8192 * 32 * sizeof(long long)) == hipSuccess) { ctx->sp_ts = (long long*)q; ctx->sp_allocs_dbg = q; } }
    if (ctx->sp_ts != nullptr) hipMemset(ctx->sp_ts, 0, (size_t)8192 * 32 * sizeof(long long));
  }
  else if (which == 23) ctx->attn_split = value;
  else if (which == 25) ctx->dbg_trip_group = value;
  else if (which == 26) ctx->sub_serial = value;
  else if (which == 27) ctx->qkv_products = value == 3 ? 3 : 2;
  else if (which == 28) ctx->ffn_compose = value;
  else if (which == 31) ctx->use_lists = value;
  else if (which == 32) ctx->qkv_in_tail = value ? 1 : 0;
  else if (which == 33) ctx->skinny = value;
  else if (which == 48) ctx->prep_fused = value ? 1 : 0;
  else if (which == 49) ctx->pnp_rounds = value ? 1 : 0;
  else if (which == 50) gn::g_sift_general_blur = value ? 1 : 0;
  else if (which == 29) {
    GN_HIP(hipSetDevice(ctx->device));
    for (int i = 0; i < 8; ++i) if (ctx->sub_s[i]) { hipStreamSynchronize(ctx->sub_s[i]); hipEventDestroy(ctx->ev_join[i]); hipStreamDestroy(ctx->sub_s[i]); ctx->sub_s[i] = nullptr; ctx->ev_join[i] = nullptr; }
    ctx->cu_mask_mode = value;
    if (ctx->n_sub > 1) { const int n = ctx->n_sub; ctx->n_sub = 1; return gn_set_substreams(ctx, n); }
  }
  else return GN_ERR_ARG;
  return GN_OK;
}

int gn_debug_epnp(gn_ctx* ctx, int n, const double* pws, const double* us, double* out, void* stream) {
  if (!ctx || n < 1 || !pws || !us || !out) return GN_ERR_ARG;
  GN_HIP(hipSetDevice(ctx->device));
  launch_epnp_debug(pws, us, out, n, (hipStream_t)stream);
  GN_HIP(hipGetLastError());
  return GN_OK;
}

int gn_debug_lds_dma_probe(gn_ctx* ctx, const float* pattern, unsigned int* out, int blocks, int spin, void* stream) {
  if (!ctx || !pattern || !out || blocks < 1) return GN_ERR_ARG;
  GN_HIP(hipSetDevice(ctx->device));
  launch_lds_dma_probe(pattern, out, blocks, spin, (hipStream_t)stream);
  GN_HIP(hipGetLastError());
  return GN_OK;
}

// ... 96 lines not shown
```

gisnav_amd/csrc/gn_common.h:

```cpp
#pragma once
#include <hip/hip_runtime.h>
#include <stdint.h>
#include <string>
#include <vector>
#include <map>

#include "../../include/gisnav_amd.h"

namespace gn {

constexpr int kDim = 256;
constexpr int kHeads = 4;
constexpr int kHeadDim = 64;
constexpr int kInDim = 128;
constexpr int kFreq = 32;
constexpr int kMaxLayers = 9;
constexpr int kRecordFloats = 133;

typedef float f32x4 __attribute__((ext_vector_type(4)));
typedef float f32x16 __attribute__((ext_vector_type(16)));
typedef short bf16x8 __attribute__((ext_vector_type(8)));

__device__ __forceinline__ float gelu_erf(float y) {
  const float t = fminf(fabsf(y) * 0.70710678118654752440f, 4.0f);
// ... 204 lines not shown
  float* x; uint16_t* xp;
  uint16_t* desc_p;
  float* rot4; long long rot_stride;
  unsigned int* ovf_clear; unsigned int ovf_init;
};
void launch_prep(const PrepArgs& a, hipStream_t s);
void launch_ln_gelu(float* h, const float* gamma, const float* beta, int rows, hipStream_t s,
                    uint16_t* hp = nullptr, unsigned int* ovf = nullptr);
void launch_matchability(const float* x, const float* w, const float* b, float* ls, int rows, hipStream_t s);

struct HeadArgs {
  const float* sim;
  const float* ls;
  const int32_t* nvalid;
  int B; int npad; float threshold;
  float* rowmax; float* rowlog; float* colmax; float* collog;
  int32_t* m0; float* max0; int32_t* m1;
  int64_t* idx; float* score; int32_t* n_match; int kmax;
  const unsigned int* ovf;
  const void* md;
  int md_f32;
  float* cpart_m; float* cpart_s; int32_t* cpart_i;
  float* rpart_a; float* rpart_b;
  unsigned int* tickets;
  long long* dbg_ts;
  float* max0b;
  float* rpart_c;
  int32_t* uncert;
  float cert_eps;
  int32_t* uncert_alt = nullptr;
  float cert_eps_alt = -1.f;
  int32_t* uncert_alt2 = nullptr;
  float cert_eps_alt2 = -1.f;
  float* colbest = nullptr;
  float* col2 = nullptr;
  const int32_t* n_in = nullptr;
};
void launch_match_head(const HeadArgs& a, hipStream_t s);
void launch_match_head_fused(const HeadArgs& a, hipStream_t s);

struct GatherArgs {
  const float* kpt_q; int stride_q; const float* kpt_r; int stride_r; int kpt_format;
  const int64_t* idx; const int32_t* n_match; int kmax; int B;
  const uint8_t* dem; int H; int W;
  float* mkp_q; float* obj;
};
void launch_gather(const GatherArgs& a, hipStream_t s);

struct DemFormat { int type = 0; double scale = 1.0, offset = 0.0; int has_nodata = 0; double nodata = 0.0; };
inline bool dem_format_is_default(const DemFormat& f) { return f.type == 0 && f.scale == 1.0 && f.offset == 0.0 && !f.has_nodata; }
inline size_t dem_elem_bytes(int type) { return type == 0 ? 1 : type == 3 ? 4 : 2; }
struct DemGatherArgs {
  GatherArgs g;
  DemFormat f;
  int64_t* idx = nullptr; float* score = nullptr; int32_t* n_match = nullptr; int32_t* dropped = nullptr;
};
void launch_gather_dem(const DemGatherArgs& a, hipStream_t s);

struct HypResult { double R[9]; double t[3]; int good; int valid; };

#ifndef GN_RANSAC_ROUND
#define GN_RANSAC_ROUND 64
#endif
constexpr int kRansacRound = GN_RANSAC_ROUND;
struct RansacState {
  int niters;
// ... 114 lines not shown
```

gisnav_amd/csrc/gn_ffn128.hip:

```cpp
#include "gn_common.h"
#include <algorithm>
#include "gn_ffn_util.h"

namespace gn {

namespace {

#define GN_PIN() __builtin_amdgcn_sched_barrier(0)

__device__ __forceinline__ float resid_lo(unsigned int h, float y) { float r; asm("v_fma_mix_f32 %0, %1, -1.0, %2 op_sel:[0,0,0] op_sel_hi:[1,0,0]" : "=v"(r) : "v"(h), "v"(y)); return r; }
__device__ __forceinline__ float addh_lo(unsigned int h, float y) { float r; asm("v_fma_mix_f32 %0, %1, 1.0, %2 op_sel:[0,0,0] op_sel_hi:[1,0,0]" : "=v"(r) : "v"(h), "v"(y)); return r; }
__device__ __forceinline__ float addh_hi(unsigned int h, float y) { float r; asm("v_fma_mix_f32 %0, %1, 1.0, %2 op_sel:[1,0,0] op_sel_hi:[1,0,0]" : "=v"(r) : "v"(h), "v"(y)); return r; }
__device__ __forceinline__ float resid_hi(unsigned int h, float y) { float r; asm("v_fma_mix_f32 %0, %1, -1.0, %2 op_sel:[1,0,0] op_sel_hi:[1,0,0]" : "=v"(r) : "v"(h), "v"(y)); return r; }

constexpr float kErf2C[5] = {1.1510913372039795f, 0.4592547118663788f, 0.05256116762757301f, -0.007397464942187071f, 0.0005204487242735922f};
constexpr float kErf2Clamp = 5.75f;

template <int ABL, bool COMP, bool LOOP = false, int QKV = 0, int PROD = 3>
__global__ __launch_bounds__(256) void k_ffn128(FfnArgs a_in) {
  static_assert(PROD == 3 || ((PROD == 2 || PROD == 1) && COMP), "two partial products / one: composed form only");
  constexpr bool HI = PROD != 3;
  constexpr int NJ = 4, NI = 4, NO = 2, NW = 4, TM = 128;
  constexpr int KT = TM * 128;
  constexpr int RING = 8 * KT;
// ... 639 lines not shown
  float amax2 = 0.f;
  uint4 xh[QKV != 0 ? RW / 2 : 1];
#pragma unroll
  for (int it = 0; it < RW / 2; ++it) {
    const int rowl = RW * wave + 2 * it;
    const f32x4 ya = *reinterpret_cast<const f32x4*>(yt + (rowl + hh) * YP + f0), yb = *reinterpret_cast<const f32x4*>(yt + (rowl + hh) * YP + f0 + 4);
    const unsigned int xhw[4] = {rh[it].x, rh[it].y, rh[it].z, rh[it].w}, xmw[4] = {rm[it].x, rm[it].y, rm[it].z, rm[it].w};
    f32x2v v[4], t[4];
#pragma unroll
    for (int k = 0; k < 4; ++k) {
      const f32x2v yk = k < 2 ? (f32x2v){ya[2 * k], ya[2 * k + 1]} : (f32x2v){yb[2 * k - 4], yb[2 * k - 3]};
      const f32x2v bk = k < 2 ? (f32x2v){bias_a[2 * k], bias_a[2 * k + 1]} : (f32x2v){bias_b[2 * k - 4], bias_b[2 * k - 3]};
      const f32x2v f = yk * splat2(s2) + bk;
      v[k] = (f32x2v){addh_lo(xhw[k], addh_lo(xmw[k], f[0])), addh_hi(xhw[k], addh_hi(xmw[k], f[1]))};
    }
    unsigned int hw[4], mw[4];
#pragma unroll
    for (int k = 0; k < 4; ++k) { amax2 = fmaxf(amax2, fmaxf(fabsf(v[k][0]), fabsf(v[k][1]))); hw[k] = __builtin_bit_cast(unsigned int, __builtin_convertvector(v[k], f16x2v)); }
#pragma unroll
    for (int k = 0; k < 4; ++k) t[k] = (f32x2v){resid_lo(hw[k], v[k][0]), resid_hi(hw[k], v[k][1])};
#pragma unroll
    for (int k = 0; k < 4; ++k) mw[k] = __builtin_bit_cast(unsigned int, __builtin_convertvector(t[k], f16x2v));
    __builtin_amdgcn_raw_buffer_store_b128((u32x4_t){hw[0], hw[1], hw[2], hw[3]}, yrs, roff, rowl * 1024, 0);
    __builtin_amdgcn_raw_buffer_store_b128((u32x4_t){mw[0], mw[1], mw[2], mw[3]}, yrs, roff + 32, rowl * 1024, 0);
    if constexpr (QKV != 0) xh[it] = make_uint4(hw[0], hw[1], hw[2], hw[3]);
    if (a.y != nullptr) {
      __builtin_amdgcn_raw_buffer_store_b128(__builtin_bit_cast(u32x4_t, (f32x4){v[0][0], v[0][1], v[1][0], v[1][1]}), frs, foff, rowl * 1024, 0);
      __builtin_amdgcn_raw_buffer_store_b128(__builtin_bit_cast(u32x4_t, (f32x4){v[2][0], v[2][1], v[3][0], v[3][1]}), frs, foff + 16, rowl * 1024, 0);
    }
    GN_PIN();
  }
  ovf_commit(a.ovf, amax2);
  if constexpr (QKV != 0) {
    constexpr bool CROSS = QKV == 2;
    constexpr int NPASS = CROSS ? 2 : 3;
    constexpr int NQK = CROSS ? kDim : 2 * kDim;
    constexpr int ROT = 8 * KT;
    constexpr int RQ = 4;
    const int slot = bm / a.npad, i0 = bm - slot * a.npad;
    f32x4 rq[CROSS ? 1 : 8];
    if constexpr (!CROSS) {
#pragma unroll
      for (int k = 0; k < 8; ++k) {
        const int e = tid + 256 * k;
        rq[k] = reinterpret_cast<const f32x4*>(a.q_rot4)[(size_t)(e >> 7) * a.q_rot_stride + (size_t)(bm + (e & 127))];
      }
    }
    __syncthreads();
    {
      int l_ = lane;
      asm volatile("" : "+v"(l_));
      const int oc = l_ & 31, rp = l_ >> 5;
      const int ch = 4 * ((oc >> 1) & 1) + (oc & 1);
#pragma unroll
      for (int it = 0; it < RW / 2; ++it) {
        const int row = RW * wave + 2 * it + rp;
        *reinterpret_cast<uint4*>(smem + (oc >> 2) * KT + row * 128 + ((ch ^ swz(row)) * 16)) = xh[it];
      }
    }
    if constexpr (!CROSS) {
#pragma unroll
      for (int k = 0; k < 8; ++k) *reinterpret_cast<f32x4*>(smem + ROT + (tid + 256 * k) * 16) = rq[k];
    }
    window(0);
    window(1);
    f16x8 qa[RQ][2][2];
    f16x8 qb[3][2];
    auto read_q = [&](int gp) __attribute__((always_inline)) {
      const int ks = gp >> 1, jp = gp & 1;
      const int off = (ks >> 1) * KT + jp * 8192;
#pragma unroll
      for (int jl = 0; jl < 2; ++jl) qb[gp % 3][jl] = *reinterpret_cast<const f16x8*>(smem + bo[off >> 16][jl][2 * (ks & 1)] + (off & 65535));
    };
    const float ascale = a.q_acc_scale;
    const __amdgpu_buffer_rsrc_t qrs = __builtin_amdgcn_make_buffer_rsrc(a.q_qkb + (size_t)bm * NQK, 0, TM * NQK * 2, 0x00020000);
    float amaxq = 0.f;
    __syncthreads();
#pragma unroll
    for (int pass = 0; pass < NPASS; ++pass) {
      const bool vpass = pass == NPASS - 1;
      const __amdgpu_buffer_rsrc_t wq = __builtin_amdgcn_make_buffer_rsrc(const_cast<uint16_t*>(a.q_wf) + (size_t)(8 * pass + 2 * wave) * 16 * 2 * 512, 0, 2 * 16 * 2 * 1024, 0x00020000);
      auto load_q = [&](int slot_, int ks, int i2, int pl) __attribute__((always_inline)) { qa[slot_][i2][pl] = ldw(wq, ((i2 * 16 + ks) * 2 + pl) * 1024); };
#pragma unroll
      for (int q = 0; q < RQ; ++q)
#pragma unroll
        for (int i2 = 0; i2 < 2; ++i2)
#pragma unroll
          for (int pl = 0; pl < 2; ++pl) load_q(q, q, i2, pl);
      f32x4 bias4[2][4];
      if (!vpass) {
#pragma unroll
        for (int i2 = 0; i2 < 2; ++i2)
#pragma unroll
          for (int g = 0; g < 4; ++g) bias4[i2][g] = *reinterpret_cast<const f32x4*>(a.q_bias + 32 * (8 * pass + 2 * wave + i2) + 8 * g + 4 * hh);
      }
      f32x16 qacc[2][NJ];
#pragma unroll
      for (int i2 = 0; i2 < 2; ++i2)
#pragma unroll
        for (int j = 0; j < NJ; ++j)
#pragma unroll
          for (int r = 0; r < 16; ++r) qacc[i2][j][r] = 0.f;
      read_q(0);
      read_q(1);
      GN_PIN();
#pragma unroll
      for (int ks = 0; ks < 16; ++ks) {
#pragma unroll
        for (int jp = 0; jp < 2; ++jp) {
          const int gp = 2 * ks + jp;
          if (gp + 2 < 32) read_q(gp + 2);
#pragma unroll
          for (int p = 0; p < 2; ++p)
#pragma unroll
            for (int jl = 0; jl < 2; ++jl)
#pragma unroll
              for (int i2 = 0; i2 < 2; ++i2) {
                const int j = 2 * jp + jl, m = 8 * jp + 4 * p + 2 * jl + i2;
                const f16x8 w = qa[ks % RQ][i2][p == 0 ? 1 : 0], x = qb[gp % 3][jl];
                qacc[i2][j] = vpass ? __builtin_amdgcn_mfma_f32_32x32x16_f16(x, w, qacc[i2][j], 0, 0, 0)
                                    : __builtin_amdgcn_mfma_f32_32x32x16_f16(w, x, qacc[i2][j], 0, 0, 0);
                if (m % 4 == 1 && ks >= 1 && ks + RQ - 1 < 16) load_q((ks - 1) % RQ, ks + RQ - 1, (m / 4) >> 1, (m / 4) & 1);
                GN_PIN();
              }
        }
      }
      if (!vpass) {
        const unsigned int qlo = (unsigned int)((ql * NQK + 8 * hh) * 2);
#pragma unroll
        for (int i2 = 0; i2 < 2; ++i2) {
          const int tile = 8 * pass + 2 * wave + i2;
#pragma unroll
          for (int j = 0; j < NJ; ++j) {
            uint2 pk[4];
#pragma unroll
            for (int g = 0; g < 4; ++g) {
              f32x4 v = {qacc[i2][j][4 * g], qacc[i2][j][4 * g + 1], qacc[i2][j][4 * g + 2], qacc[i2][j][4 * g + 3]};
              v.x = v.x * ascale; v.y = v.y * ascale; v.z = v.z * ascale; v.w = v.w * ascale;
              asm volatile("" : "+v"(v.x), "+v"(v.y), "+v"(v.z), "+v"(v.w));
              v.x += bias4[i2][g].x; v.y += bias4[i2][g].y; v.z += bias4[i2][g].z; v.w += bias4[i2][g].w;
              asm volatile("" : "+v"(v.x), "+v"(v.y), "+v"(v.z), "+v"(v.w));
              if (CROSS) {
                v.x *= a.q_scale; v.y *= a.q_scale; v.z *= a.q_scale; v.w *= a.q_scale;
                asm volatile("" : "+v"(v.x), "+v"(v.y), "+v"(v.z), "+v"(v.w));
              } else {
                const f32x4 rot = *reinterpret_cast<const f32x4*>(smem + ROT + ((8 * i2 + 2 * g + hh) * 128 + 32 * j + ql) * 16);
                f32x4 o;
                o.x = v.x * rot.x + (-v.y) * rot.z;
                o.y = v.y * rot.x + v.x * rot.z;
                o.z = v.z * rot.y + (-v.w) * rot.w;
                o.w = v.w * rot.y + v.z * rot.w;
                v = o;
                if (pass == 0) { v.x *= a.q_qscale; v.y *= a.q_qscale; v.z *= a.q_qscale; v.w *= a.q_qscale; asm volatile("" : "+v"(v.x), "+v"(v.y), "+v"(v.z), "+v"(v.w)); }
              }
              pk[g].x = pack16<true>(v.x, v.y);
// ... 27 lines not shown
                const float lo = qacc[i2][j][8 * m + 2 * e] * ascale + bias;
                const float hi = qacc[i2][j][8 * m + 2 * e + 1] * ascale + bias;
                w4[e] = pack16<true>(lo, hi);
                ovf_track(amaxq, lo, hi);
              }
              __builtin_amdgcn_raw_buffer_store_b128((u32x4_t){w4[0], w4[1], w4[2], w4[3]}, vrs, vlo, (32 * j + 16 * m) * 2, 0);
            }
        }
      }
      GN_PIN();
    }
    ovf_commit(a.ovf, amaxq);
  }
  if (ABL & 8) {
    stamp(9);
    if (a.dbg_ts != nullptr && lane == 0)
      for (int k = 0; k < 12; ++k) a.dbg_ts[((size_t)blockIdx.x * NW + wave) * 12 + k] = ts[k];
    if ((ABL & 128) && a.dbg_ts != nullptr && lane == 0)
      for (int k = 0; k < 16; ++k) a.dbg_ts[(size_t)gridDim.x * NW * 12 + ((size_t)blockIdx.x * NW + wave) * 16 + k] = ts2[k];
  }
  if (!LOOP) break;
  __syncthreads();
  }
}
#undef GN_PIN
}

#ifdef GN_FFN128_LEVEL1_TU
void launch_ffn128_level1(const FfnArgs& b, dim3 grid, bool walk, int stamps, int qv, hipStream_t s) {
  const dim3 block(256);
#define GN_F1(Q) do { if (stamps == 8) hipLaunchKernelGGL((k_ffn128<8, true, false, 0, 1>), grid, block, 0, s, b); \
                      else if (walk) hipLaunchKernelGGL((k_ffn128<0, true, true, Q, 1>), grid, block, 0, s, b); \
                      else hipLaunchKernelGGL((k_ffn128<0, true, false, Q, 1>), grid, block, 0, s, b); } while (0)
  if (qv == 1) { GN_F1(1); g_last_kernel = walk ? "k_ffn128<0, true, true, 1, 1>" : "k_ffn128<0, true, false, 1, 1>"; }
  else if (qv == 2) { GN_F1(2); g_last_kernel = walk ? "k_ffn128<0, true, true, 2, 1>" : "k_ffn128<0, true, false, 2, 1>"; }
  else { GN_F1(0); g_last_kernel = walk ? "k_ffn128<0, true, true, 0, 1>" : "k_ffn128<0, true, false, 0, 1>"; }
#undef GN_F1
}
#else
void launch_ffn128_level1(const FfnArgs& b, dim3 grid, bool walk, int stamps, int qv, hipStream_t s);

void launch_ffn128(const FfnArgs& a, int stamps, hipStream_t s) {
  const int ncu = a.ncu > 0 ? a.ncu : device_cu_count();
  const bool walk = a.tiles != nullptr && a.walk && stamps == 0;
  const dim3 grid(walk ? std::min(a.T / 128, ncu) : a.T / 128), block(256);
  FfnArgs b = a;
  if (!walk) b.tiles = nullptr;
  if (walk || stamps != 0) b.nvalid = nullptr;
  if (a.composed && a.products == 1 && (stamps == 0 || stamps == 8)) {
    launch_ffn128_level1(b, grid, walk, stamps, stamps == 0 ? a.qkv : 0, s);
    return;
  }
  if (a.composed && a.products == 2 && (stamps == 0 || stamps == 8)) {
#define GN_F2(Q) do { if (stamps == 8) hipLaunchKernelGGL((k_ffn128<8, true, false, Q, 2>), grid, block, 0, s, b); \
                      else if (walk) hipLaunchKernelGGL((k_ffn128<0, true, true, Q, 2>), grid, block, 0, s, b); \
                      else hipLaunchKernelGGL((k_ffn128<0, true, false, Q, 2>), grid, block, 0, s, b); } while (0)
    const int qv = stamps == 0 ? a.qkv : 0;
    if (qv == 1) { GN_F2(1); g_last_kernel = walk ? "k_ffn128<0, true, true, 1, 2>" : "k_ffn128<0, true, false, 1, 2>"; }
    else if (qv == 2) { GN_F2(2); g_last_kernel = walk ? "k_ffn128<0, true, true, 2, 2>" : "k_ffn128<0, true, false, 2, 2>"; }
    else { GN_F2(0); g_last_kernel = walk ? "k_ffn128<0, true, true, 0, 2>" : "k_ffn128<0, true, false, 0, 2>"; }
#undef GN_F2
    return;
  }
  if (a.composed && a.qkv != 0 && stamps == 0) {
    if (a.qkv == 1) {
      if (walk) hipLaunchKernelGGL((k_ffn128<0, true, true, 1>), grid, block, 0, s, b); else hipLaunchKernelGGL((k_ffn128<0, true, false, 1>), grid, block, 0, s, b);
      g_last_kernel = walk ? "k_ffn128<0, true, true, 1, 3>" : "k_ffn128<0, true, false, 1, 3>";
// ... 27 lines not shown
```

gisnav_amd/csrc/gn_match_head.hip:

```cpp
#include <type_traits>

#include "gn_common.h"

namespace gn {

namespace {
__device__ inline float wave_sum(float v) {
#pragma unroll
  for (int o = 32; o > 0; o >>= 1) v += __shfl_xor(v, o);
  return v;
}
__device__ inline float wave_max(float v) {
#pragma unroll
  for (int o = 32; o > 0; o >>= 1) v = fmaxf(v, __shfl_xor(v, o));
  return v;
}

__global__ __launch_bounds__(256) void k_row_stats(HeadArgs a) {
  const int lane = threadIdx.x & 63, b = blockIdx.y;
  const int i = blockIdx.x * 4 + (threadIdx.x >> 6);
  const int n0 = a.nvalid[2 * b], n1 = a.nvalid[2 * b + 1];
  if (i >= n0) return;
  const float* row = a.sim + ((size_t)b * a.npad + i) * a.npad;
  float m = -INFINITY;
// ... 75 lines not shown
  float best = -INFINITY; int bi = 0x7fffffff;
  if (j < n1) {
    const float* base = a.sim + ro * a.npad + j;
    const float cm = a.colmax[ro + j], cl = a.collog[ro + j];
    const float lj = a.ls[(size_t)(2 * b + 1) * a.npad + j];
    const float* lsi = a.ls + (size_t)(2 * b) * a.npad;
    for (int i = g; i < n0; i += kColGroups) {
      const float p = score_at(base[(size_t)i * a.npad], a.rowmax[ro + i], a.rowlog[ro + i], cm, cl, lsi[i], lj);
      if (p > best || bi == 0x7fffffff) { best = p; bi = i; }
    }
  }
  rv[g][c] = best; ri[g][c] = bi;
  __syncthreads();
  if (g == 0 && j < n1) {
#pragma unroll
    for (int k = 1; k < kColGroups; ++k) {
      const float ob = rv[k][c]; const int oi = ri[k][c];
      if (oi != 0x7fffffff && (bi == 0x7fffffff || ob > best || (ob == best && oi < bi))) { best = ob; bi = oi; }
    }
    a.m1[ro + j] = bi;
  }
}

__global__ __launch_bounds__(256) void k_compact(HeadArgs a) {
  __shared__ int wcount[4];
  __shared__ int base_s;
  const int b = blockIdx.x, tid = threadIdx.x, lane = tid & 63, wave = tid >> 6;
  const int n0 = a.nvalid[2 * b], n1 = a.nvalid[2 * b + 1];
  const size_t ro = (size_t)b * a.npad;
  if (tid == 0) base_s = 0;
  __syncthreads();
  const bool nomatch = (a.n_in ? a.n_in[2 * b] : n0) < 2 || (a.n_in ? a.n_in[2 * b + 1] : n1) < 2 || n0 < 1 || n1 < 1;
  if (nomatch || (a.ovf != nullptr && *a.ovf != 0u)) {
    if (tid == 0) { a.n_match[b] = 0; if (a.uncert) a.uncert[b] = nomatch ? 0 : 2; if (a.uncert_alt) a.uncert_alt[b] = 0; if (a.uncert_alt2) a.uncert_alt2[b] = 0; }
    return;
  }
  if (tid == 0 && a.uncert) a.uncert[b] = 1;
  if (tid == 0 && a.uncert_alt) a.uncert_alt[b] = 1;
  if (tid == 0 && a.uncert_alt2) a.uncert_alt2[b] = 1;
  for (int i0 = 0; i0 < n0; i0 += 256) {
    const int i = i0 + tid;
    bool valid = false; int j = 0; float sc = 0.f;
    if (i < n0) {
      j = a.m0[ro + i];
      sc = expf(a.max0[ro + i]);
      valid = (a.m1[ro + j] == i) && (sc > a.threshold);
    }
    const unsigned long long bal = __ballot(valid);
    const int before = __popcll(bal & ((1ull << lane) - 1ull));
    if (lane == 0) wcount[wave] = __popcll(bal);
    __syncthreads();
    int off = base_s;
    for (int w = 0; w < wave; ++w) off += wcount[w];
    if (valid) {
      const size_t k = (size_t)b * a.kmax + off + before;
      a.idx[2 * k] = i; a.idx[2 * k + 1] = j;
      a.score[k] = sc;
    }
    __syncthreads();
    if (tid == 0) base_s += wcount[0] + wcount[1] + wcount[2] + wcount[3];
    __syncthreads();
  }
  if (tid == 0) a.n_match[b] = base_s;
}

typedef _Float16 f16x8 __attribute__((ext_vector_type(8)));
typedef __attribute__((address_space(1))) const void* gptr_t;
typedef __attribute__((address_space(3))) void* lptr_t;
constexpr int kHeadKT = 64 * 128;
constexpr int kHeadTile = 8 * kHeadKT;
constexpr int kHeadRows = 128;
constexpr int kHeadMaxSplit = 8;
// ... 260 lines not shown
  __syncthreads();
  stamp(4);
  if (!s_last) return;
  const int nparts = nact;
  int* const m1s = reinterpret_cast<int*>(smem) + 64;
  for (int i = tid; S > 1 && i < n0; i += 512) {
    float pa[kHeadMaxSplit], pb[kHeadMaxSplit], pc[kHeadMaxSplit];
#pragma unroll
    for (int e = 0; e < kHeadMaxSplit; ++e) {
      const size_t pr = ((size_t)b * kHeadMaxSplit + min(e, S - 1)) * np + i;
      pa[e] = ld_dev(a.rpart_a + pr); pb[e] = ld_dev(a.rpart_b + pr);
      pc[e] = SWEEP == 2 ? ld_dev(a.rpart_c + pr) : 0.f;
    }
    if (SWEEP == 1) {
      float m = -INFINITY, sm = 0.f;
#pragma unroll
      for (int e = 0; e < kHeadMaxSplit; ++e) if (e < S) lse_merge(m, sm, pa[e], pb[e]);
      a.rowmax[ro + i] = m; a.rowlog[ro + i] = logf(sm);
    } else {
      float bv = -INFINITY; int bj = 0x7fffffff; float b2 = -INFINITY;
#pragma unroll
      for (int e = 0; e < kHeadMaxSplit; ++e) {
        if (e >= S) continue;
        b2 = fmaxf(fmaxf(b2, pc[e]), fminf(bv, pa[e]));
        if (arg_better(pa[e], __float_as_int(pb[e]), bv, bj)) { bv = pa[e]; bj = __float_as_int(pb[e]); }
      }
      st_dev(a.m0 + ro + i, bj); st_dev(a.max0 + ro + i, bv); st_dev(a.max0b + ro + i, b2);
    }
  }
  const bool cert = a.uncert != nullptr && a.cert_eps >= 0.f;
  const bool cert2 = cert && a.uncert_alt != nullptr && a.cert_eps_alt >= 0.f;
  const float Lth = a.threshold > 0.f ? logf(a.threshold) : -INFINITY;
  const bool cert3 = cert && a.uncert_alt2 != nullptr && a.cert_eps_alt2 >= 0.f;
  int unc = 0, unc2 = 0, unc3 = 0;
  for (int j = tid; j < n1; j += 512) {
    float m = -INFINITY, sm = 0.f; int bi = 0x7fffffff; float m2 = -INFINITY;
    for (int p0 = 0; p0 < nparts; p0 += 16) {
      float pm[16], ps[16], p2[16];
#pragma unroll
      for (int e = 0; e < 16; ++e) {
        const size_t po = ((size_t)b * npart + min(p0 + e, nparts - 1)) * np + j;
        pm[e] = ld_dev(a.cpart_m + po);
        ps[e] = SWEEP == 1 ? ld_dev(a.cpart_s + po) : __int_as_float(ld_dev(a.cpart_i + po));
        p2[e] = SWEEP == 2 ? ld_dev(a.cpart_s + po) : 0.f;
      }
#pragma unroll
      for (int e = 0; e < 16; ++e) {
        if (p0 + e >= nparts) continue;
        if (SWEEP == 1) lse_merge(m, sm, pm[e], ps[e]);
        else {
          m2 = fmaxf(fmaxf(m2, p2[e]), fminf(m, pm[e]));
          if (arg_better(pm[e], __float_as_int(ps[e]), m, bi)) { m = pm[e]; bi = __float_as_int(ps[e]); }
        }
      }
    }
    if (SWEEP == 1) { a.colmax[ro + j] = m; a.collog[ro + j] = logf(sm); }
    else {
      a.m1[ro + j] = bi; m1s[j] = bi;
      if (a.colbest != nullptr) { a.colbest[ro + j] = m; a.col2[ro + j] = m2; }
      if (cert && m >= Lth - a.cert_eps && !(m - m2 > 2.f * a.cert_eps)) unc = 1;
      if (cert2 && m >= Lth - a.cert_eps_alt && !(m - m2 > 2.f * a.cert_eps_alt)) unc2 = 1;
      if (cert3 && m >= Lth - a.cert_eps_alt2 && !(m - m2 > 2.f * a.cert_eps_alt2)) unc3 = 1;
    }
  }
  stamp(5);
  if (SWEEP == 1) return;
  asm volatile("s_waitcnt vmcnt(0)" ::: "memory");
  __syncthreads();
  int* const wcount = reinterpret_cast<int*>(smem);
  int* const base_s = wcount + 8;
  if (tid == 0) *base_s = 0;
  __syncthreads();
  if (nomatch || (a.ovf != nullptr && *a.ovf != 0u)) {
    if (tid == 0) { a.n_match[b] = 0; if (a.uncert) a.uncert[b] = nomatch ? 0 : 2; if (a.uncert_alt) a.uncert_alt[b] = 0; if (a.uncert_alt2) a.uncert_alt2[b] = 0; }
    return;
  }
  for (int ib = 0; ib < n0; ib += 512) {
    const int i = ib + tid;
    bool valid = false; int j = 0; float sc = 0.f;
    if (i < n0) {
      j = ld_dev(a.m0 + ro + i);
      const float best = ld_dev(a.max0 + ro + i);
      sc = expf(best);
      valid = (m1s[j] == i) && (sc > a.threshold);
      if (cert) {
        const float second = ld_dev(a.max0b + ro + i);
        if (best >= Lth - a.cert_eps && !(best - second > 2.f * a.cert_eps)) unc = 1;
        if (fabsf(best - Lth) <= a.cert_eps) unc = 1;
        if (cert2 && ((best >= Lth - a.cert_eps_alt && !(best - second > 2.f * a.cert_eps_alt)) || fabsf(best - Lth) <= a.cert_eps_alt)) unc2 = 1;
        if (cert3 && ((best >= Lth - a.cert_eps_alt2 && !(best - second > 2.f * a.cert_eps_alt2)) || fabsf(best - Lth) <= a.cert_eps_alt2)) unc3 = 1;
      }
    }
    const unsigned long long bal = __ballot(valid);
    const int before = __popcll(bal & ((1ull << lane) - 1ull));
    if (lane == 0) wcount[wave] = __popcll(bal);
    __syncthreads();
    int off = *base_s;
    for (int w = 0; w < wave; ++w) off += wcount[w];
    if (valid) {
      const size_t k = (size_t)b * a.kmax + off + before;
      a.idx[2 * k] = i; a.idx[2 * k + 1] = j;
      a.score[k] = sc;
    }
    __syncthreads();
    if (tid == 0) { int tot = 0; for (int w = 0; w < 8; ++w) tot += wcount[w]; *base_s += tot; }
    __syncthreads();
  }
  if (tid == 0) a.n_match[b] = *base_s;
  if (a.uncert) {
    const int any = __syncthreads_or(unc);
    if (tid == 0) a.uncert[b] = (cert && any) ? 1 : 0;
    if (a.uncert_alt) {
      const int any2 = __syncthreads_or(unc2);
      if (tid == 0) a.uncert_alt[b] = (cert2 && any2) ? 1 : 0;
    }
    if (a.uncert_alt2) {
      const int any3 = __syncthreads_or(unc3);
      if (tid == 0) a.uncert_alt2[b] = (cert3 && any3) ? 1 : 0;
    }
  }
  stamp(6);
}

__global__ __launch_bounds__(256) void k_gather(GatherArgs a) {
  const int b = blockIdx.y, k = blockIdx.x * 256 + threadIdx.x;
  if (k >= a.n_match[b]) return;
  const size_t o = (size_t)b * a.kmax + k;
  const int iq = (int)a.idx[2 * o], ir = (int)a.idx[2 * o + 1];
  const int w = a.kpt_format == GN_KPT_LAF ? 6 : a.kpt_format == GN_KPT_RECORD ? kRecordFloats : 4;
  const int xo = a.kpt_format == GN_KPT_LAF ? 2 : 0, yo = a.kpt_format == GN_KPT_LAF ? 5 : 1;
  const float* kq = a.kpt_q + ((size_t)b * a.stride_q + iq) * w;
  const float* kr = a.kpt_r + ((size_t)b * a.stride_r + ir) * w;
  a.mkp_q[2 * o] = kq[xo]; a.mkp_q[2 * o + 1] = kq[yo];
  const float xr = kr[xo], yr = kr[yo];
  float z = 0.f;
  if (a.dem != nullptr) {
    int xi = (int)floorf(xr), yi = (int)floorf(yr);
    xi = min(max(xi, 0), a.W - 1); yi = min(max(yi, 0), a.H - 1);
    z = (float)a.dem[((size_t)b * a.H + yi) * a.W + xi];
  }
  a.obj[3 * o] = xr; a.obj[3 * o + 1] = yr; a.obj[3 * o + 2] = z;
}
}

void launch_match_head_fused(const HeadArgs& a, hipStream_t s) {
  const int nrb = a.npad / kHeadRows, ntile = a.npad / 64;
  int S = 1;
  while (S < kHeadMaxSplit && 2 * S <= ntile && nrb * a.B * S < 256) S *= 2;
  const dim3 grid(nrb, a.B, S), block(512);
  if (a.md_f32) {
    hipLaunchKernelGGL((k_head_fused<true, 1>), grid, block, 0, s, a);
// ... 23 lines not shown
```

gisnav_amd/csrc/gn_qkv.hip:

```cpp
#include "gn_common.h"
#include <algorithm>

namespace gn {

namespace {
typedef _Float16 f16x8 __attribute__((ext_vector_type(8)));

__device__ __forceinline__ int swz(int row) { return (row ^ (row >> 3)) & 7; }

constexpr int TM = 128;
constexpr int KT = TM * 128;
constexpr int NJ = TM / 32;

template <bool CROSS, bool F16 = false, int NP = 3>
__global__ __launch_bounds__(512) void k_qkv(QkvArgs a) {
  constexpr int NQK = CROSS ? kDim : 2 * kDim;
  constexpr int NPASS = CROSS ? 2 : 3;
  __shared__ __attribute__((aligned(1024))) unsigned char smem[8 * KT + (CROSS ? 0 : 32768)];
  const int n_work = a.tiles != nullptr ? a.tiles[0] : a.T / TM;
#pragma unroll 1
  for (int work = blockIdx.x; work < n_work; work += gridDim.x) {
  int tid = threadIdx.x;
  asm volatile("" : "+v"(tid));
  const int lane = tid & 63, wave = __builtin_amdgcn_readfirstlane(tid >> 6);
  const int hh = lane >> 5, ql = lane & 31;
  const int bm = (a.tiles != nullptr ? a.tiles[kTileListBase + work] : work) * TM;
  long long ts[8];
  auto stamp = [&](int k) __attribute__((always_inline)) { if (a.dbg_ts) ts[k] = (long long)__builtin_amdgcn_s_memtime(); };
  stamp(0);

  {
    const int srow = tid >> 3, schunk = tid & 7;
#pragma unroll
    for (int half = 0; half < 2; ++half) {
      const int row = srow + 64 * half;
      const unsigned char* xsrc = reinterpret_cast<const unsigned char*>(a.xp) + (size_t)(bm + row) * 1024 + schunk * 16;
      const int sdst = row * 128 + ((schunk ^ swz(row)) * 16);
      uint4 xt[8];
#pragma unroll
      for (int q = 0; q < 8; ++q) xt[q] = *reinterpret_cast<const uint4*>(xsrc + q * 128);
#pragma unroll
      for (int q = 0; q < 8; ++q) *reinterpret_cast<uint4*>(smem + q * KT + sdst) = xt[q];
    }
  }
  int brow[NJ], bsw[NJ];
#pragma unroll
  for (int j = 0; j < NJ; ++j) { brow[j] = (32 * j + ql) * 128; bsw[j] = swz(32 * j + ql); }
  f16x8 fb[2][NJ][2];
  auto read_b = [&](int buf, int ks) __attribute__((always_inline)) {
#pragma unroll
    for (int j = 0; j < NJ; ++j)
#pragma unroll
      for (int pl = 0; pl < 2; ++pl)
        fb[buf][j][pl] = *reinterpret_cast<const f16x8*>(smem + (ks >> 1) * KT + brow[j] + (((4 * (ks & 1) + 2 * pl + hh) ^ bsw[j]) * 16));
  };
  const uint4* const wf = reinterpret_cast<const uint4*>(a.wf) + lane;
  constexpr int RA = CROSS ? 8 : 6;
  f16x8 fa[RA][2];
  const float ascale = a.acc_scale;
  const int slot = bm / a.npad, i0 = bm - slot * a.npad;
  __syncthreads();
  stamp(1);

  f32x4 rot[NJ][4];
  f32x4* const rot_park = reinterpret_cast<f32x4*>(smem + 8 * KT) + (wave & 1) * 16 * 64 + lane;
#pragma unroll
  for (int pass = 0; pass < NPASS; ++pass) {
    const bool vpass = pass == NPASS - 1;
    const int tile = 8 * pass + wave;
    auto load_a = [&](int slot_, int ks) __attribute__((always_inline)) {
#pragma unroll
      for (int pl = 0; pl < 2; ++pl) fa[slot_][pl] = __builtin_bit_cast(f16x8, wf[(size_t)((tile * 16 + ks) * 2 + pl) * 64]);
    };
#pragma unroll
    for (int q = 0; q < RA; ++q) load_a(q, q);
    f32x16 acc[NJ];
#pragma unroll
    for (int j = 0; j < NJ; ++j)
#pragma unroll
      for (int r = 0; r < 16; ++r) acc[j][r] = 0.f;
    read_b(0, 0);
#pragma unroll
    for (int ks = 0; ks < 16; ++ks) {
      const int rs = ks % RA, cb = ks & 1;
      if (ks + 1 < 16) read_b(cb ^ 1, ks + 1);
#pragma unroll
      for (int p = 0; p < 3; ++p)
#pragma unroll
        for (int j = 0; j < NJ; ++j) {
          if (NP == 2 && p == 1) continue;
          const f16x8 w = fa[rs][p == 0 ? 1 : 0], x = fb[cb][j][p == 1 ? 1 : 0];
          acc[j] = vpass ? __builtin_amdgcn_mfma_f32_32x32x16_f16(x, w, acc[j], 0, 0, 0)
                         : __builtin_amdgcn_mfma_f32_32x32x16_f16(w, x, acc[j], 0, 0, 0);
        }
      if (ks + RA < 16) load_a(rs, ks + RA);
      __builtin_amdgcn_sched_barrier(0);
    }
    stamp(2 + 2 * pass);
    float amax = 0.f;
    if (!vpass) {
      f32x4 bias4[4];
#pragma unroll
      for (int g = 0; g < 4; ++g) bias4[g] = *reinterpret_cast<const f32x4*>(a.bias + 32 * tile + 8 * g + 4 * hh);
      if (!CROSS && pass == 0) {
#pragma unroll
        for (int j = 0; j < NJ; ++j)
#pragma unroll
          for (int g = 0; g < 4; ++g) {
            const int fg = ((32 * wave + 8 * g + 4 * hh) & 63) >> 2;
            rot[j][g] = *reinterpret_cast<const f32x4*>(a.rot4 + ((size_t)fg * a.rot_stride + (size_t)(bm + 32 * j + ql)) * 4);
          }
      }
      if (!CROSS && pass == 1) {
#pragma unroll
        for (int j = 0; j < NJ; ++j)
#pragma unroll
          for (int g = 0; g < 4; ++g) rot[j][g] = rot_park[(4 * j + g) * 64];
      }
      __builtin_amdgcn_sched_barrier(0);
#pragma unroll
      for (int j = 0; j < NJ; ++j) {
        const size_t row = (size_t)(bm + 32 * j + ql);
        uint2 pk[4];
#pragma unroll
// ... 45 lines not shown
          for (int e = 0; e < 4; ++e) {
            const float lo = acc[j][8 * m + 2 * e] * ascale + bias;
            const float hi = acc[j][8 * m + 2 * e + 1] * ascale + bias;
            w4[e] = pack16<F16>(lo, hi);
            if (F16) ovf_track(amax, lo, hi);
          }
          if (!(a.vt_perm & 2)) *reinterpret_cast<uint4*>(dst + 32 * j + 8 * (2 * m + hh)) = make_uint4(w4[0], w4[1], w4[2], w4[3]);
        }
    }
    if (F16) ovf_commit(a.ovf, amax);
    stamp(3 + 2 * pass);
  }
  if (a.dbg_ts && lane == 0) {
    for (int k = 0; k < 8; ++k) a.dbg_ts[((size_t)blockIdx.x * 8 + wave) * 8 + k] = ts[k];
  }
  __syncthreads();
  }
}
}

int device_cu_count() {
  static int cache[64] = {0};
  int dev = 0;
  if (hipGetDevice(&dev) != hipSuccess || dev < 0 || dev >= 64) return 256;
  int n = __atomic_load_n(&cache[dev], __ATOMIC_RELAXED);
  if (n > 0) return n;
  if (hipDeviceGetAttribute(&n, hipDeviceAttributeMultiprocessorCount, dev) != hipSuccess || n <= 0) n = 256;
  __atomic_store_n(&cache[dev], n, __ATOMIC_RELAXED);
  return n;
}
void launch_qkv(const QkvArgs& a, bool cross, hipStream_t s) {
  const int ncu = a.ncu > 0 ? a.ncu : device_cu_count();
  const dim3 grid(a.tiles != nullptr ? std::min(a.T / TM, ncu) : a.T / TM), block(512);
  const int sel = (a.half_fmt ? 4 : 0) | (cross ? 2 : 0) | (a.products == 2 ? 1 : 0);
  switch (sel) {
    case 7: hipLaunchKernelGGL((k_qkv<true, true, 2>), grid, block, 0, s, a); g_last_kernel = "k_qkv<true, true, 2>"; break;
    case 6: hipLaunchKernelGGL((k_qkv<true, true, 3>), grid, block, 0, s, a); g_last_kernel = "k_qkv<true, true, 3>"; break;
    case 5: hipLaunchKernelGGL((k_qkv<false, true, 2>), grid, block, 0, s, a); g_last_kernel = "k_qkv<false, true, 2>"; break;
    case 4: hipLaunchKernelGGL((k_qkv<false, true, 3>), grid, block, 0, s, a); g_last_kernel = "k_qkv<false, true, 3>"; break;
    case 3: hipLaunchKernelGGL((k_qkv<true, false, 2>), grid, block, 0, s, a); g_last_kernel = "k_qkv<true, false, 2>"; break;
    case 2: hipLaunchKernelGGL((k_qkv<true, false, 3>), grid, block, 0, s, a); g_last_kernel = "k_qkv<true, false, 3>"; break;
    case 1: hipLaunchKernelGGL((k_qkv<false, false, 2>), grid, block, 0, s, a); g_last_kernel = "k_qkv<false, false, 2>"; break;
    default: hipLaunchKernelGGL((k_qkv<false, false, 3>), grid, block, 0, s, a); g_last_kernel = "k_qkv<false, false, 3>"; break;
  }
}

}
```

gisnav_amd/engine.py:

```python
from __future__ import annotations

import contextlib
import ctypes as C
import struct
from typing import Dict, Optional, Tuple

import numpy as np
import torch

from . import _lib
from .weights import canonical_state_dict

MIN_MATCHES = 15
FILTER_THRESHOLD = 0.5
RANSAC_ITERATIONS = 10
RANSAC_REPROJ_PX = 8.0
RANSAC_CONFIDENCE = 0.99



def check_ransac_iterations(iterations) -> int:
    if isinstance(iterations, bool) or not isinstance(iterations, (int, np.integer)):
        raise TypeError(f"ransac iterations must be an integer, got {type(iterations).__name__}")
    if not 1 <= int(iterations) <= _lib.GN_RANSAC_MAX_ITERATIONS:
# ... 233 lines not shown
        self._guard = {"off": 0, "flag": 1, "sync": 2}[guard]
        self.feature = feature
        self._feature = {"sift": _lib.GN_FEATURE_SIFT, "superpoint": _lib.GN_FEATURE_SUPERPOINT}[feature]
        self.desc_dim = 128 if feature == "sift" else 256
        ctx = C.c_void_p()
        _lib.check(None, self.lib.gn_create_ex(device, max_batch, max_kpts, _PRECISIONS[precision], self._feature, C.byref(ctx)), "gn_create_ex")
        self.ctx = ctx
        self.kmax = self.lib.gn_kmax(ctx)
        _lib.check(ctx, self.lib.gn_set_num_layers(ctx, n_layers), "gn_set_num_layers")
        _lib.check(ctx, self.lib.gn_set_filter_threshold(ctx, filter_threshold), "gn_set_filter_threshold")
        _lib.check(ctx, self.lib.gn_set_guard(ctx, self._guard), "gn_set_guard")
        if state_dict is not None:
            self.load_state_dict(state_dict)

    def guard_status(self):
        last, total = C.c_int32(0), C.c_int64(0)
        _lib.check(self.ctx, self.lib.gn_get_guard_status(self.ctx, self._stream(), C.byref(last), C.byref(total)), "gn_get_guard_status")
        return bool(last.value), int(total.value)

    def set_certify(self, mode, eps: Optional[float] = None, eps_f32: Optional[float] = None) -> None:
        m = {"off": 0, "flag": 1, "rerun": 2, "deferred": 3}.get(mode, mode)
        self._certify_mode, self._last_out_ptr = int(m), None
        _lib.check(self.ctx, self.lib.gn_set_certify(self.ctx, int(m), -1.0 if eps is None else float(eps), -1.0 if eps_f32 is None else float(eps_f32)),
                   "gn_set_certify")

    def fused_projection_status(self) -> int:
        return int(self.lib.gn_fused_projection_status(self.ctx))

    def set_ffn_products(self, products) -> None:
        p = 0 if products in ("auto", 0) else int(products)
        self._ffn_auto = p == 0
        _lib.check(self.ctx, self.lib.gn_set_ffn_products(self.ctx, p), "gn_set_ffn_products")

    def set_ffn_level_eps(self, eps_two: float, eps_three: float, level: int = 3, eps_one: Optional[float] = None) -> None:
        if eps_one is not None:
            _lib.check(self.ctx, self.lib.gn_set_ffn_level_eps1(self.ctx, float(eps_one)), "gn_set_ffn_level_eps1")
        _lib.check(self.ctx, self.lib.gn_set_ffn_level_eps(self.ctx, float(eps_two), float(eps_three), int(level)), "gn_set_ffn_level_eps")

    def ffn_level(self) -> Dict[str, float]:
        lvl, e2, e3, buf = C.c_int32(0), C.c_float(0.0), C.c_float(0.0), (C.c_int64 * 4)()
        _lib.check(self.ctx, self.lib.gn_get_ffn_level(self.ctx, C.byref(lvl), C.byref(e2), C.byref(e3), buf), "gn_get_ffn_level")
        e1, c1 = C.c_float(0.0), C.c_int64(0)
        _lib.check(self.ctx, self.lib.gn_get_ffn_level1(self.ctx, C.byref(e1), C.byref(c1)), "gn_get_ffn_level1")
        return {"level": int(lvl.value), "eps_two_products": float(e2.value), "eps_three_products": float(e3.value), "eps_one_product": float(e1.value),
                "calls_two_products": int(buf[0]), "calls_three_products": int(buf[1]), "calls_one_product": int(c1.value),
                "switches": int(buf[2]), "automatic": bool(buf[3])}

    def calibrate_certify(self, inputs: dict, safety: float = 4.0, floor_eps: float = 1.0e-5) -> Dict[str, float]:
        B = inputs["kpt_q"].shape[0]
        m, e = C.c_float(0.0), C.c_float(0.0)
        rc = self.lib.gn_calibrate_certify(self.ctx, B, inputs["kpt_format"],
                                           _ptr(inputs.get("desc_q")), _ptr(inputs["kpt_q"]), _ptr(inputs["n_q"]), inputs["kpt_q"].shape[1],
                                           _ptr(inputs.get("desc_r")), _ptr(inputs["kpt_r"]), _ptr(inputs["n_r"]), inputs["kpt_r"].shape[1],
                                           float(safety), float(floor_eps), C.byref(m), C.byref(e), self._stream())
        _lib.check(self.ctx, rc, "gn_calibrate_certify")
        lv = self.ffn_level()
        d = {"measured": float(m.value), "eps": float(e.value), "safety": float(safety)}
        if getattr(self, "_certify_ladder", False):
            d["eps_mid"] = self.certify_ladder_stats()["eps_mid"]
        if getattr(self, "_ffn_auto", False):
            d["eps_two_products"], d["eps_three_products"] = lv["eps_two_products"], lv["eps_three_products"]
            d["eps_one_product"] = lv["eps_one_product"]
        return d

    def set_certify_ladder(self, enable: bool, eps_mid: Optional[float] = None) -> None:
        _lib.check(self.ctx, self.lib.gn_set_certify_ladder(self.ctx, int(bool(enable)), -1.0 if eps_mid is None else float(eps_mid)),
                   "gn_set_certify_ladder")
        self._certify_ladder = bool(enable)

    def certify_ladder_stats(self) -> Dict[str, float]:
        buf = (C.c_int64 * 4)()
        _lib.check(self.ctx, self.lib.gn_get_certify_ladder_stats(self.ctx, buf), "gn_get_certify_ladder_stats")
        eps = None if buf[3] < 0 else struct.unpack("<f", struct.pack("<I", int(buf[3])))[0]
        return {"mid_rerun": int(buf[0]), "mid_certified": int(buf[1]), "passed_to_f32": int(buf[2]), "eps_mid": eps}

    def certify_stats(self, reset: bool = False) -> Dict[str, int]:
        buf = (C.c_int64 * 8)()
        _lib.check(self.ctx, self.lib.gn_get_certify_stats(self.ctx, buf), "gn_get_certify_stats")
        if reset:
            _lib.check(self.ctx, self.lib.gn_reset_certify_stats(self.ctx), "gn_reset_certify_stats")
        keys = ("calls", "pairs", "flagged_margin", "flagged_fp16_range", "rerun_pairs", "f32_marginal_pairs", "mode")
        d = {k: int(buf[i]) for i, k in enumerate(keys)}
        d["eps_source"] = {0: "default", 1: "stated", 2: "calibrated", 3: "discarded"}.get(int(buf[7]), str(int(buf[7])))
        d["rerun_fraction"] = (d["rerun_pairs"] / d["pairs"]) if d["pairs"] else 0.0
        return d

    def uncertain(self, B: int) -> np.ndarray:
        out = np.zeros(B, np.int32)
        _lib.check(self.ctx, self.lib.gn_get_uncertain(self.ctx, int(B), out.ctypes.data_as(_lib.c_i32p), self._stream()), "gn_get_uncertain")
        return out

    def __del__(self):
        ctx, self.ctx = getattr(self, "ctx", None), None
        if ctx:
            self.lib.gn_destroy(ctx)
# ... 554 lines not shown
```

include/gisnav_amd.h:

```cpp
#ifndef GISNAV_AMD_H
#define GISNAV_AMD_H

#include <stdint.h>

#ifdef __cplusplus
extern "C" {
#endif

typedef struct gn_ctx gn_ctx;

enum gn_status {
  GN_OK = 0,
  GN_ERR_ARG = -1,
  GN_ERR_HIP = -2,
  GN_ERR_NAME = -3,
  GN_ERR_SHAPE = -4,
  GN_ERR_WEIGHTS = -5,
  GN_ERR_ARCH = -6
};

enum gn_precision {
  GN_PREC_F32 = 0,
  GN_PREC_BF16_ATTN = 1,
  GN_PREC_F32X3_BF16_ATTN = 2,
  GN_PREC_F16X2_BF16_ATTN = 3,
  GN_PREC_F16X2_F16_ATTN = 4  ,
  GN_PREC_F16X2_F16X2_ATTN = 5
};

enum gn_kpt_format {
  GN_KPT_LAF = 0,
  GN_KPT_XYSA = 1,
  GN_KPT_RECORD = 2
};
#define GN_DESC_ROOTSIFT 0x100

const char* gn_version(void);
const char* gn_last_error(const gn_ctx* ctx);

int gn_set_guard(gn_ctx* ctx, int mode);
int gn_get_guard_status(gn_ctx* ctx, void* stream, int32_t* last_call_tripped, int64_t* trips_total);

int gn_set_certify(gn_ctx* ctx, int mode, float eps, float eps_f32);
int gn_set_ffn_products(gn_ctx* ctx, int products);
int gn_get_ffn_level(gn_ctx* ctx, int32_t* level, float* eps2, float* eps3, int64_t* out4);
int gn_set_ffn_level_eps(gn_ctx* ctx, float eps2, float eps3, int level);
int gn_get_ffn_level1(gn_ctx* ctx, float* eps1, int64_t* calls1);
int gn_set_ffn_level_eps1(gn_ctx* ctx, float eps1);
int gn_debug_ffn_level_sim(int n_calls, int B, const int32_t* f1, const int32_t* f2, const int32_t* f3, int have1, int32_t* levels_out, int64_t* out4);
int gn_fused_projection_status(const gn_ctx* ctx);
int gn_device_numa_node(int device);
int gn_get_certify_stats(gn_ctx* ctx, int64_t* out8);
int gn_reset_certify_stats(gn_ctx* ctx);
int gn_set_certify_ladder(gn_ctx* ctx, int enable, float eps_mid);
int gn_get_certify_ladder_stats(gn_ctx* ctx, int64_t* out4);
int gn_calibrate_certify(gn_ctx* ctx, int B, int kpt_format,
                         const float* desc_q, const float* kpt_q, const int32_t* n_q, int stride_q,
                         const float* desc_r, const float* kpt_r, const int32_t* n_r, int stride_r,
                         float safety, float floor_eps, float* measured_host, float* eps_host, void* stream);
int gn_get_uncertain(gn_ctx* ctx, int B, int32_t* host_flags, void* stream);
const char* gn_source_digest(void);

int gn_create(int device, int max_batch, int max_kpts, int precision, gn_ctx** out);
enum gn_feature { GN_FEATURE_SIFT = 0, GN_FEATURE_SUPERPOINT = 1 };
int gn_create_ex(int device, int max_batch, int max_kpts, int precision, int feature, gn_ctx** out);
int gn_set_image_size(gn_ctx* ctx, float w_q, float h_q, float w_r, float h_r);
int gn_resize(gn_ctx* ctx, int max_kpts);
void gn_destroy(gn_ctx* ctx);

int gn_load_tensor(gn_ctx* ctx, const char* name, const float* host_data, const int64_t* shape, int ndim);
int gn_missing_tensors(const gn_ctx* ctx);

int gn_set_num_layers(gn_ctx* ctx, int n_layers);
int gn_set_filter_threshold(gn_ctx* ctx, float th);

int gn_set_width_pruning(gn_ctx* ctx, float width_confidence, int min_kpts);
int gn_get_width_pruning(const gn_ctx* ctx, float* width_confidence, int* min_kpts);
int gn_get_prune(gn_ctx* ctx, int B, int32_t* prune_q, int32_t* prune_r);

int gn_match(gn_ctx* ctx, int B, int kpt_format,
             const float* desc_q, const float* kpt_q, const int32_t* n_q, int stride_q,
             const float* desc_r, const float* kpt_r, const int32_t* n_r, int stride_r,
// ... 175 lines not shown
```

Baseline: 6964.

## Add certified single-product QKV projection rung to adaptive FFN precision ladder

Result: faster. 7379, median of 6 (+6.0%).

```diff
diff --git a/gisnav_amd/_lib.py b/gisnav_amd/_lib.py
--- a/gisnav_amd/_lib.py
+++ b/gisnav_amd/_lib.py
@@ -69,6 +69,10 @@
     "gn_get_ffn_level1": (C.c_int, [VP, c_f32p, c_i64p]),
     "gn_set_ffn_level_eps1": (C.c_int, [VP, C.c_float]),
     "gn_debug_ffn_level_sim": (C.c_int, [C.c_int, C.c_int, VP, VP, VP, C.c_int, VP, VP]),
+    "gn_set_qkv_products": (C.c_int, [VP, C.c_int]),
+    "gn_get_qkv_level": (C.c_int, [VP, C.POINTER(C.c_int32), C.POINTER(C.c_int32), c_f32p, c_i64p]),
+    "gn_set_qkv_level_eps": (C.c_int, [VP, C.c_float]),
+    "gn_debug_ffn_level_sim_rung": (C.c_int, [C.c_int, C.c_int, VP, VP, VP, VP, C.c_int, C.c_int, VP, VP, VP]),
     "gn_fused_projection_status": (C.c_int, [VP]),
     "gn_device_numa_node": (C.c_int, [C.c_int]),
     "gn_get_certify_stats": (C.c_int, [VP, c_i64p]),
diff --git a/gisnav_amd/csrc/gn_api.hip b/gisnav_amd/csrc/gn_api.hip
--- a/gisnav_amd/csrc/gn_api.hip
+++ b/gisnav_amd/csrc/gn_api.hip
@@ -100,6 +100,7 @@
   X(float, collog, np, kWsAlways, "collog") X(float, max0, np, kWsAlways, "max0") X(int32_t, m0, np, kWsAlways, "m0")            \
   X(int32_t, m1, np, kWsAlways, "m1") X(float, max0b, np, kWsAlways, "max0b") X(float, rpart_c, 8 * np, kWsAlways, nullptr)      \
   X(int32_t, uncert, 1, kWsAlways, "uncert") X(int32_t, uncert_alt, 1, kWsAlways, nullptr) X(int32_t, uncert_alt2, 1, kWsAlways, nullptr) \
+  X(int32_t, uncert_alt3, 1, kWsAlways, nullptr)                                                                                 \
   X(float, colbest, np, kWsAlways, nullptr) X(float, col2, np, kWsAlways, nullptr)                                               \
                  \
   X(float, cpart_m, (np / 32) * np, kWsAlways, nullptr) X(float, cpart_s, (np / 32) * np, kWsAlways, nullptr)                    \
@@ -234,6 +235,8 @@
   int auto_ok1 = 0;
   int ffn_products = 3;
   int qkv_products = 2;
+  int qkv_set = 0, auto_rung = 0, qkv_force = 0;
+  float cert_eps_proj1 = -1.f; long long auto_proj1 = 0, auto_calls_proj1 = 0;
   unsigned long long* tile_feedback = nullptr;
   int n_sub = 1; hipStream_t sub_s[8] = {}; hipEvent_t ev_fork = nullptr; hipEvent_t ev_join[8] = {}; bool sub_pending[8] = {};
   int overlap = 0; unsigned long long calls = 0;
@@ -473,8 +476,11 @@
 bool skinny_applies(const gn_ctx* c, int T, int np) {
   return (c->skinny & 3) && c->planes_mode && c->x_planes_only && T % 32 == 0 && np > 0 && ((c->skinny & 3) == 2 || T / np <= 4);
 }
+inline bool proj_one(const gn_ctx* c);
+inline bool tail_is_bulk(const gn_ctx* c, int T);
 bool qkv_projection(gn_ctx* c, const View& w, const Block& blk, bool cross, int T, int np, int vt_perm, hipStream_t s) {
-  const bool skinny = skinny_applies(c, T, np) && !(c->skinny & 4) && c->qkv_fused && blk.proj_in.wf && w.x_p && w.qkb && w.vtb && w.rot4 && np % 32 == 0 && vt_perm == 1 && !c->qkv_stamps;
+  const bool one = c->qkv_products != 3 && proj_one(c) && tail_is_bulk(c, T) && qkv_projection_applies(c, w, blk, T, np, vt_perm);
+  const bool skinny = !one && skinny_applies(c, T, np) && !(c->skinny & 4) && c->qkv_fused && blk.proj_in.wf && w.x_p && w.qkb && w.vtb && w.rot4 && np % 32 == 0 && vt_perm == 1 && !c->qkv_stamps;
   if (!skinny && !qkv_projection_applies(c, w, blk, T, np, vt_perm)) return false;
   QkvArgs q;
   q.xp = w.x_p; q.wf = blk.proj_in.wf; q.acc_scale = blk.proj_in.acc_scale; q.bias = blk.proj_in.b;
@@ -482,7 +488,7 @@
   q.qscale = 0.125f; q.scale = 0.35355339059327373f; q.vt_perm = vt_perm; q.T = T;
   q.half_fmt = c->attn_f16; q.ovf = (c->attn_f16 && c->guard) ? w.ovf : nullptr;
   q.tiles = (c->use_lists && w.lists && !c->qkv_stamps) ? w.lists : nullptr;
-  q.products = c->qkv_products == 3 ? 3 : 2; q.ncu = c->ncu;
+  q.products = c->qkv_products == 3 ? 3 : one ? 1 : 2; q.ncu = c->ncu;
   q.dbg_ts = (c->qkv_stamps && w.sim) ? reinterpret_cast<long long*>(w.sim) : nullptr;
   const double N = cross ? 2.0 * kDim : 3.0 * kDim;
   timed_launch(c, s, 0, 2.0 * T * N * kDim, 4.0 * T * kDim + 2.0 * T * N + 4.0 * N * kDim + (cross ? 0.0 : 2.0 * 4.0 * T * kFreq),
@@ -556,9 +562,20 @@
 inline bool ffn_auto(const gn_ctx* c) { return c->ffn_products == 0 && c->cert_eps_lvl[0] >= 0.f && c->cert_eps_lvl[1] >= 0.f && c->certify >= 2; }
 inline int ffn_level(const gn_ctx* c) { return c->attn_f16 == 2 ? 3 : c->ffn_products == 0 ? (ffn_auto(c) ? c->auto_level : 3) : c->ffn_products; }
 inline float ffn_level_eps(const gn_ctx* c, int lvl) { return lvl == 1 ? c->cert_eps_one : c->cert_eps_lvl[lvl - 2]; }
-inline float cert_eps_now(const gn_ctx* c) { return ffn_auto(c) ? ffn_level_eps(c, c->auto_level) : c->cert_eps; }
+inline bool proj_one(const gn_ctx* c) {
+  if (c->attn_f16 != 1 || c->qkv_products == 3 || ffn_level(c) != 1) return false;
+  if (c->qkv_force != 0) return c->qkv_force > 0;
+  return c->qkv_set == 1 || (c->qkv_set == 0 && ffn_auto(c) && c->auto_rung != 0 && c->cert_eps_proj1 >= 0.f);
+}
+enum { kRung = 4 };
+inline int ffn_auto_state(const gn_ctx* c) { return (c->auto_level == 1 && proj_one(c)) ? (int)kRung : c->auto_level; }
+inline float cert_eps_now(const gn_ctx* c) { return ffn_auto(c) ? (ffn_auto_state(c) == kRung ? c->cert_eps_proj1 : ffn_level_eps(c, c->auto_level)) : c->cert_eps; }
+inline bool tail_is_bulk(const gn_ctx* c, int T) {
+  return c->planes_mode && c->x_planes_only && c->ffn_fused == 3 && c->ffn_fold && c->ffn_compose && T % 128 == 0 &&
+         (gn::g_ffn_shape == 128 || (gn::g_ffn_shape == 0 && T / 128 >= 256));
+}
 inline int ffn_alt_level(int lvl, int k) { return lvl == 1 ? 2 + k : (k == 0 ? 5 - lvl : 1); }
-inline void ffn_window_reset(gn_ctx* c, int level) { c->auto_level = level; c->auto_pairs = c->auto_wide = c->auto_narrow = c->auto_one = 0; c->auto_ok1 = 0; }
+inline void ffn_window_reset(gn_ctx* c, int level) { c->auto_level = level; c->auto_rung = 0; c->auto_pairs = c->auto_wide = c->auto_narrow = c->auto_one = c->auto_proj1 = 0; c->auto_ok1 = 0; }
 
 bool ffn(gn_ctx* c, const View& w, const Block& blk, int T, hipStream_t s, bool keep_f32, const Block* next = nullptr, bool next_cross = false, int np = 0, int vt_perm = 0) {
   if (skinny_applies(c, T, np) && !(c->skinny & 8) && c->ffn_fused == 3 && c->ffn_compose && tail_folds_out_proj(c, blk, T) && blk.wfc && blk.b1c && !blk.comp_dirty && blk.ffn3.wfn &&
@@ -589,6 +606,7 @@
                           c->precision != GN_PREC_F32 && c->attn_variant >= 1 && qkv_projection_applies(c, w, *next, T, np, vt_perm) && !(vt_perm & 2);
     if (fuse_qkv) {
       f.qkv = next_cross ? 2 : 1;
+      if (f.products == 1 && proj_one(c)) f.qkv += 2;
       f.q_wf = next->proj_in.wf; f.q_acc_scale = next->proj_in.acc_scale; f.q_bias = next->proj_in.b;
       f.q_rot4 = w.rot4; f.q_rot_stride = (long long)c->Tmax; f.q_qkb = w.qkb; f.q_vt = w.vtb;
       f.q_qscale = 0.125f; f.q_scale = 0.35355339059327373f;
@@ -764,6 +782,7 @@
     if (hd.uncert && c->precision != GN_PREC_F32 && ffn_auto(c)) {
       hd.uncert_alt = w.uncert_alt; hd.cert_eps_alt = ffn_level_eps(c, ffn_alt_level(c->auto_level, 0));
       hd.uncert_alt2 = w.uncert_alt2; hd.cert_eps_alt2 = ffn_level_eps(c, ffn_alt_level(c->auto_level, 1));
+      hd.uncert_alt3 = w.uncert_alt3; hd.cert_eps_alt3 = ffn_auto_state(c) == kRung ? c->cert_eps_one : (c->qkv_set == 0 ? c->cert_eps_proj1 : -1.f);
     }
     hd.idx = v.idx; hd.score = v.score; hd.n_match = v.n_match; hd.kmax = c->npad;
     hd.md = c->planes_mode ? (const void*)w.md_p : (const void*)w.md; hd.md_f32 = c->planes_mode ? 0 : 1;
@@ -847,7 +866,7 @@
   const int np = c->npad;
   GN_HIP(hipDeviceSynchronize());
   if (!c->planes_mode || !c->qkv_in_tail || !c->attn_f16 || c->attn_f16 == 2 || c->qkv_products == 3 || !c->ffn_compose || c->ffn_fused != 3 || !c->x_planes_only || c->n_layers < 1 ||
-      !c->qkv_fused || !w.rot4 || !w.lists || !w.msg_p || !w.h_p || c->feature < 0 || gn::g_ffn_stamps != 0 || gn::g_ffn_shape != 0) return GN_OK;
+      !c->qkv_fused || !w.rot4 || !w.lists || !w.msg_p || !w.h_p || c->feature < 0 || gn::g_ffn_stamps != 0 || (gn::g_ffn_shape != 0 && gn::g_ffn_shape != 128)) return GN_OK;
   int B = (256 * 128 + 2 * np - 1) / (2 * np);
   if (B > c->max_batch) return GN_OK;
   const int T = B * 2 * np;
@@ -878,16 +897,18 @@
   GN_HIP(hipMemset(cnt, 0, sizeof(unsigned int)));
   bool applicable = true;
   {
-    const Restore keep(c->use_lists, c->qkv_in_tail, c->guard, c->ktiming, c->launch_count, c->stop_after, c->npad_run, c->ffn_products);
+    const Restore keep(c->use_lists, c->qkv_in_tail, c->guard, c->ktiming, c->launch_count, c->stop_after, c->npad_run, c->ffn_products, c->qkv_force);
     const int prod0 = c->ffn_products;
     c->ktiming = false; c->stop_after = 0; c->guard = 0; c->npad_run = np;
     const int nblk = c->n_layers > 1 ? 1 : 0;
-    const int lvs[3] = {3, prod0 == 1 ? 1 : 2, 1};
+    int lvs[4] = {3, prod0 == 1 ? 1 : 2, 1, 1};
     const int n_lv = prod0 == 0 ? 3 : (prod0 == 2 || prod0 == 1) ? 2 : 1;
-    for (int lv = 0; lv < n_lv && applicable; ++lv)
+    const bool rung = c->attn_f16 == 1 && (c->qkv_set == 1 ? (prod0 == 0 || prod0 == 1) : (c->qkv_set == 0 && prod0 == 0));
+    lvs[n_lv] = 1;
+    for (int lv = 0; lv < n_lv + (rung ? 1 : 0) && applicable; ++lv)
     for (int cross = 0; cross < 2 && applicable; ++cross)
       for (int walk = 0; walk < 2 && applicable; ++walk) {
-        c->ffn_products = lvs[lv];
+        c->ffn_products = lvs[lv]; c->qkv_force = lv == n_lv ? 1 : -1;
         const Block& tail = cross ? c->self_blk[0] : c->cross_blk[0];
         const Block* next = cross ? &c->cross_blk[0] : &c->self_blk[nblk];
         c->use_lists = walk ? 2 : 3;
@@ -934,18 +955,31 @@
   return next;
 }
 
-void ffn_level_update(gn_ctx* c, int B, const int32_t* flags, const int32_t* alt, const int32_t* alt2, int lvl) {
-  if (!ffn_auto(c) || c->precision == GN_PREC_F32 || lvl < 1 || lvl > 3) return;
-  ++(lvl == 1 ? c->auto_calls_one : c->auto_calls_lvl[lvl - 2]);
-  int n[4] = {0, 0, 0, 0};
-  const int la = ffn_alt_level(lvl, 0), lb = ffn_alt_level(lvl, 1);
-  for (int b = 0; b < B; ++b) { n[lvl] += flags[b] == 1; n[la] += alt[b] == 1; n[lb] += alt2[b] == 1; }
-  c->auto_pairs += B; c->auto_one += n[1]; c->auto_wide += n[2]; c->auto_narrow += n[3];
+int ffn_level_next_rung(int level, int* rung, int* ok1_run, long long pairs, long long n0, long long n1, long long n2, long long n3, bool have1, bool have0) {
+  const bool ok0 = have0 && have1 && (n0 - n3) * 64 <= pairs;
+  if (level == 1 && *rung && ok0) return 1;
+  const bool was_rung = level == 1 && *rung;
+  const int next = ffn_level_next(level, ok1_run, pairs, n1, n2, n3, have1);
+  *rung = (level == 1 && !was_rung && next == 1 && ok0) ? 1 : 0;
+  return next;
+}
+
+void ffn_level_update(gn_ctx* c, int B, const int32_t* flags, const int32_t* alt, const int32_t* alt2, const int32_t* alt3, int lvl) {
+  if (!ffn_auto(c) || c->precision == GN_PREC_F32 || lvl < 1 || lvl > kRung) return;
+  const int tail = lvl == kRung ? 1 : lvl;
+  ++(tail == 1 ? c->auto_calls_one : c->auto_calls_lvl[tail - 2]);
+  if (lvl == kRung) ++c->auto_calls_proj1;
+  int n[5] = {0, 0, 0, 0, 0};
+  const int la = ffn_alt_level(tail, 0), lb = ffn_alt_level(tail, 1), lc = lvl == kRung ? 1 : (int)kRung;
+  for (int b = 0; b < B; ++b) { n[lvl] += flags[b] == 1; n[la] += alt[b] == 1; n[lb] += alt2[b] == 1; n[lc] += alt3 != nullptr && alt3[b] == 1; }
+  c->auto_pairs += B; c->auto_one += n[1]; c->auto_wide += n[2]; c->auto_narrow += n[3]; c->auto_proj1 += n[kRung];
   if (c->auto_pairs < 64) return;
-  const int next = ffn_level_next(c->auto_level, &c->auto_ok1, c->auto_pairs, c->auto_one, c->auto_wide, c->auto_narrow, c->cert_eps_one >= 0.f);
-  if (next != c->auto_level) ++c->auto_switches;
+  const int rung0 = c->auto_rung;
+  const int next = ffn_level_next_rung(c->auto_level, &c->auto_rung, &c->auto_ok1, c->auto_pairs, c->auto_proj1, c->auto_one, c->auto_wide, c->auto_narrow, c->cert_eps_one >= 0.f,
+                                       c->qkv_set == 0 && c->cert_eps_proj1 >= 0.f && c->attn_f16 == 1 && c->qkv_products != 3);
+  if (next != c->auto_level || c->auto_rung != rung0) ++c->auto_switches;
   c->auto_level = next;
-  c->auto_pairs = c->auto_wide = c->auto_narrow = c->auto_one = 0;
+  c->auto_pairs = c->auto_wide = c->auto_narrow = c->auto_one = c->auto_proj1 = 0;
 }
 
 struct ExactF32 : Restore<int, int, int, int, int> {
@@ -1020,11 +1054,13 @@
     if (ffn_auto(ctx)) {
       GN_HIP(hipMemcpyAsync(ctx->uncert_host + ctx->max_batch, ctx->ws.uncert_alt, (size_t)B * sizeof(int32_t), hipMemcpyDeviceToHost, s));
       GN_HIP(hipMemcpyAsync(ctx->uncert_host + 2 * ctx->max_batch, ctx->ws.uncert_alt2, (size_t)B * sizeof(int32_t), hipMemcpyDeviceToHost, s));
+      GN_HIP(hipMemcpyAsync(ctx->uncert_host + 3 * ctx->max_batch, ctx->ws.uncert_alt3, (size_t)B * sizeof(int32_t), hipMemcpyDeviceToHost, s));
     }
     GN_HIP(hipStreamSynchronize(s));
     flags_ready = ctx->uncert_host;
   }
-  ffn_level_update(ctx, B, flags_ready, flags_ready + ctx->max_batch, flags_ready + 2 * ctx->max_batch, flags_level ? flags_level : ctx->auto_level);
+  ffn_level_update(ctx, B, flags_ready, flags_ready + ctx->max_batch, flags_ready + 2 * ctx->max_batch, flags_ready + 3 * ctx->max_batch,
+                   flags_level ? flags_level : ffn_auto_state(ctx));
   ++ctx->cert_calls; ctx->cert_pairs += B;
   std::vector<int> flagged, margin;
   for (int b = 0; b < B; ++b) {
@@ -1059,18 +1095,19 @@
   return GN_OK;
 }
 
-enum { kCalExactF32 = 0, kCalMid = -1 };
+enum { kCalExactF32 = 0, kCalMid = -1, kCalProj1 = 4 };
 struct CalPass { std::vector<float> best, second, colbest, col2; unsigned int trip = 0u; };
 int cal_pass(gn_ctx* ctx, const Call& w, int arith, bool cols, std::vector<int32_t>* nv, CalPass& out, hipStream_t s) {
   const View vw = view_of(ctx);
   int rc = GN_OK;
   {
-    const Restore keep(ctx->in_group, ctx->cal_cols, ctx->ffn_products);
+    const Restore keep(ctx->in_group, ctx->cal_cols, ctx->ffn_products, ctx->qkv_force);
+    ctx->qkv_force = arith == kCalProj1 ? 1 : (ctx->ffn_products == 0 ? -1 : 0);
     ctx->in_group = true;
     ctx->cal_cols = cols;
     if (arith == kCalExactF32) { const ExactF32 f32(ctx); rc = run_matcher(ctx, vw, w, s); }
     else if (arith == kCalMid) { const MidLevel mid(ctx); rc = run_matcher(ctx, vw, w, s); }
-    else { ctx->ffn_products = arith; rc = run_matcher(ctx, vw, w, s); }
+    else { ctx->ffn_products = arith == kCalProj1 ? 1 : arith; rc = run_matcher(ctx, vw, w, s); }
   }
   if (rc != GN_OK) return rc;
   const size_t n = (size_t)w.B * ctx->npad_run;
@@ -1236,10 +1273,10 @@
   if (hipHostMalloc((void**)&ctx->ovf_host, (16 + 4096 + 16) * sizeof(unsigned int), hipHostMallocDefault) != hipSuccess) { gn_destroy(ctx); return fail(nullptr, GN_ERR_HIP, "hipHostMalloc failed"); }
   memset(ctx->ovf_host, 0, (16 + 4096 + 16) * sizeof(unsigned int));
   ctx->tile_feedback = reinterpret_cast<unsigned long long*>(ctx->ovf_host + 16 + 4096);
-  if (hipHostMalloc((void**)&ctx->uncert_host, (size_t)3 * max_batch * sizeof(int32_t), hipHostMallocDefault) != hipSuccess) { gn_destroy(ctx); return fail(nullptr, GN_ERR_HIP, "hipHostMalloc failed"); }
-  memset(ctx->uncert_host, 0, (size_t)3 * max_batch * sizeof(int32_t));
+  if (hipHostMalloc((void**)&ctx->uncert_host, (size_t)4 * max_batch * sizeof(int32_t), hipHostMallocDefault) != hipSuccess) { gn_destroy(ctx); return fail(nullptr, GN_ERR_HIP, "hipHostMalloc failed"); }
+  memset(ctx->uncert_host, 0, (size_t)4 * max_batch * sizeof(int32_t));
   for (auto& pd : ctx->cert_pend) {
-    if (hipHostMalloc((void**)&pd.flags, (size_t)3 * max_batch * sizeof(int32_t), hipHostMallocDefault) != hipSuccess ||
+    if (hipHostMalloc((void**)&pd.flags, (size_t)4 * max_batch * sizeof(int32_t), hipHostMallocDefault) != hipSuccess ||
         hipEventCreateWithFlags(&pd.ev, hipEventDisableTiming) != hipSuccess) { gn_destroy(ctx); return fail(nullptr, GN_ERR_HIP, "certificate slots: allocation failed"); }
   }
   ctx->ncu = prop.multiProcessorCount > 0 ? prop.multiProcessorCount : 256;
@@ -1460,7 +1497,7 @@
   }
   if (rc == GN_OK) {
     ctx->loaded[name] = true; ctx->fused_proj_pending = true;
-    ctx->cert_eps_lvl[0] = ctx->cert_eps_lvl[1] = ctx->cert_eps_one = -1.f; ffn_window_reset(ctx, 3);
+    ctx->cert_eps_lvl[0] = ctx->cert_eps_lvl[1] = ctx->cert_eps_one = ctx->cert_eps_proj1 = -1.f; ffn_window_reset(ctx, 3);
     ctx->cert_eps_mid = -1.f;
     if (ctx->cert_eps_src >= 2) { ctx->cert_eps = INFINITY; ctx->cert_eps_src = 3; }
   }
@@ -1572,6 +1609,32 @@
 int gn_set_ffn_level_eps1(gn_ctx* ctx, float eps1) {
   if (!ctx || !(eps1 >= 0.f)) return GN_ERR_ARG;
   ctx->cert_eps_one = std::max(eps1, std::max(ctx->cert_eps_lvl[0], ctx->cert_eps_lvl[1]));
+  if (ctx->cert_eps_proj1 >= 0.f) ctx->cert_eps_proj1 = std::max(ctx->cert_eps_proj1, ctx->cert_eps_one);
+  return GN_OK;
+}
+
+int gn_set_qkv_products(gn_ctx* ctx, int products) {
+  if (!ctx || products < 0 || products > 2) return GN_ERR_ARG;
+  if (products != ctx->qkv_set) {
+    ffn_window_reset(ctx, 3);
+    ctx->fused_proj_pending = true;
+  }
+  ctx->qkv_set = products;
+  return GN_OK;
+}
+
+int gn_set_qkv_level_eps(gn_ctx* ctx, float eps_proj1) {
+  if (!ctx || !(eps_proj1 >= 0.f)) return GN_ERR_ARG;
+  ctx->cert_eps_proj1 = std::max(eps_proj1, std::max(ctx->cert_eps_one, std::max(ctx->cert_eps_lvl[0], ctx->cert_eps_lvl[1])));
+  return GN_OK;
+}
+
+int gn_get_qkv_level(gn_ctx* ctx, int32_t* setting, int32_t* on_rung, float* eps_proj1, int64_t* calls_proj1) {
+  if (!ctx) return GN_ERR_ARG;
+  if (setting) *setting = ctx->qkv_set;
+  if (on_rung) *on_rung = proj_one(ctx) ? 1 : 0;
+  if (eps_proj1) *eps_proj1 = ctx->cert_eps_proj1;
+  if (calls_proj1) *calls_proj1 = ctx->auto_calls_proj1;
   return GN_OK;
 }
 
@@ -1592,9 +1655,26 @@
     const int lvl = c->auto_level;
     if (levels_out) levels_out[i] = lvl;
     const size_t o = (size_t)i * B;
-    ffn_level_update(c.get(), B, f[lvl] + o, f[ffn_alt_level(lvl, 0)] + o, f[ffn_alt_level(lvl, 1)] + o, lvl);
+    ffn_level_update(c.get(), B, f[lvl] + o, f[ffn_alt_level(lvl, 0)] + o, f[ffn_alt_level(lvl, 1)] + o, nullptr, lvl);
   }
   if (out4) { out4[0] = c->auto_level; out4[1] = c->auto_switches; out4[2] = c->auto_calls_lvl[0]; out4[3] = c->auto_calls_one; }
+  return GN_OK;
+}
+
+int gn_debug_ffn_level_sim_rung(int n_calls, int B, const int32_t* f0, const int32_t* f1, const int32_t* f2, const int32_t* f3, int have1, int have0, int32_t* levels_out, int32_t* rung_out, int64_t* out5) {
+  if (n_calls < 0 || B < 1 || !f0 || !f1 || !f2 || !f3) return GN_ERR_ARG;
+  std::unique_ptr<gn_ctx> c(new gn_ctx);
+  c->ffn_products = 0; c->certify = 2; c->precision = GN_PREC_F16X2_BF16_ATTN; c->attn_f16 = 1;
+  c->cert_eps_lvl[0] = 2.f; c->cert_eps_lvl[1] = 1.f; c->cert_eps_one = have1 ? 3.f : -1.f; c->cert_eps_proj1 = have0 ? 4.f : -1.f;
+  const int32_t* f[5] = {nullptr, f1, f2, f3, f0};
+  for (int i = 0; i < n_calls; ++i) {
+    const int st = ffn_auto_state(c.get()), tail = st == kRung ? 1 : st;
+    if (levels_out) levels_out[i] = tail;
+    if (rung_out) rung_out[i] = st == kRung ? 1 : 0;
+    const size_t o = (size_t)i * B;
+    ffn_level_update(c.get(), B, f[st] + o, f[ffn_alt_level(tail, 0)] + o, f[ffn_alt_level(tail, 1)] + o, f[st == kRung ? 1 : (int)kRung] + o, st);
+  }
+  if (out5) { out5[0] = c->auto_level; out5[1] = c->auto_switches; out5[2] = c->auto_calls_lvl[0]; out5[3] = c->auto_calls_one; out5[4] = ffn_auto_state(c.get()) == kRung ? 1 : 0; }
   return GN_OK;
 }
 
@@ -1639,10 +1719,11 @@
   Call v(ctx->feature, ctx->npad, B, kpt_format, desc_q, kpt_q, n_q, stride_q, desc_r, kpt_r, n_r, stride_r);
   v.idx = ctx->ws.e_idx; v.score = ctx->ws.e_score; v.n_match = nm;
   const int setting = ctx->ffn_products;
-  const int n_lv = setting == 0 ? 3 : 1;
-  const int lv[3] = {setting == 0 ? 1 : setting, 2, 3};
+  const bool rung = setting == 0 && ctx->qkv_set == 0 && ctx->attn_f16 == 1 && ctx->qkv_products != 3;
+  const int n_lv = setting == 0 ? (rung ? 4 : 3) : 1;
+  const int lv[4] = {setting == 0 ? 1 : setting, 2, 3, kCalProj1};
   const float L = ctx->threshold > 0.f ? logf(ctx->threshold) : -INFINITY;
-  CalPass whole[4];
+  CalPass whole[5];
   std::vector<int32_t> nv(2 * (size_t)B);
   unsigned int tripped = 0u;
   const bool lad = ctx->ladder && ctx->planes_mode && ctx->attn_f16 != 2;
@@ -1658,7 +1739,7 @@
     tripped |= mid.trip;
     mid_mx = std::max(mid_mx, max_diff(mid, whole[n_lv], nv, mp == 0 ? B : 1, np, true, L));
   }
-  double var_mx[3] = {0.0, 0.0, 0.0};
+  double var_mx[4] = {0.0, 0.0, 0.0, 0.0};
   int32_t* nr1 = nullptr;
   if (rc == GN_OK && !tripped && nv[0] >= 2 && nv[1] >= 2 && hipMalloc((void**)&nr1, sizeof(int32_t)) != hipSuccess) rc = GN_ERR_HIP;
   Call v1 = slice(v, 0, 1);
@@ -1666,7 +1747,7 @@
   for (int var = 0; nr1 && rc == GN_OK && var < 3; ++var) {
     const int32_t nr_cut = var == 0 ? nv[1] : std::min(nv[1], var == 1 ? 128 : 2);
     if (hipMemcpy(nr1, &nr_cut, sizeof nr_cut, hipMemcpyHostToDevice) != hipSuccess) { rc = GN_ERR_HIP; break; }
-    CalPass p[4];
+    CalPass p[5];
     unsigned int trip = 0u;
     for (int pass = 0; pass <= n_lv && rc == GN_OK; ++pass) {
       rc = cal_pass(ctx, v1, pass == n_lv ? kCalExactF32 : lv[pass], false, nullptr, p[pass], s);
@@ -1679,7 +1760,7 @@
   hipFree(nm);
   if (rc != GN_OK) return rc == GN_ERR_HIP ? fail(ctx, rc, "gn_calibrate_certify: a HIP call failed") : rc;
   if (tripped) return fail(ctx, GN_ERR_ARG, "gn_calibrate_certify: the sample left the fp16 range of this precision mode (nothing to calibrate: such calls are re-run as a whole)");
-  float eps_of[3] = {0.f, 0.f, 0.f}, mx_of[3] = {0.f, 0.f, 0.f};
+  float eps_of[4] = {0.f, 0.f, 0.f, 0.f}, mx_of[4] = {0.f, 0.f, 0.f, 0.f};
   for (int k = 0; k < n_lv; ++k) {
     long long rows = 0;
     double mx = max_diff(whole[k], whole[n_lv], nv, B, np, false, L, &rows);
@@ -1691,6 +1772,7 @@
   }
   if (setting == 0) {
     ctx->cert_eps_lvl[1] = eps_of[2]; ctx->cert_eps_lvl[0] = std::max(eps_of[1], eps_of[2]); ctx->cert_eps_one = std::max(eps_of[0], ctx->cert_eps_lvl[0]);
+    ctx->cert_eps_proj1 = rung ? std::max(eps_of[3], ctx->cert_eps_one) : -1.f;
     ffn_window_reset(ctx, 3);
   }
   if (lad && mid_mx >= 0.0) {
@@ -1698,7 +1780,7 @@
     ctx->cert_eps_mid = std::max(floor_eps, safety * (float)mid_mx);
     ctx->cert_mid_measured = (float)mid_mx;
   }
-  const int rep = n_lv - 1;
+  const int rep = setting == 0 ? 2 : 0;
   ctx->cert_eps = eps_of[rep]; ctx->cert_eps_src = 2;
   if (measured_host) *measured_host = mx_of[rep];
   if (eps_host) *eps_host = eps_of[rep];
@@ -1734,7 +1816,7 @@
   if (!ctx) return GN_ERR_ARG;
   ctx->cert_calls = ctx->cert_pairs = ctx->cert_flag_margin = ctx->cert_flag_range = ctx->cert_rerun = ctx->cert_f32_marginal = 0;
   ctx->mid_rerun = ctx->mid_certified = ctx->mid_passed = 0;
-  ctx->auto_calls_lvl[0] = ctx->auto_calls_lvl[1] = ctx->auto_calls_one = ctx->auto_switches = 0;
+  ctx->auto_calls_lvl[0] = ctx->auto_calls_lvl[1] = ctx->auto_calls_one = ctx->auto_calls_proj1 = ctx->auto_switches = 0;
   return GN_OK;
 }
 
@@ -2058,9 +2140,10 @@
     if (ffn_auto(ctx)) {
       GN_HIP(hipMemcpyAsync(p.flags + ctx->max_batch, ctx->ws.uncert_alt, (size_t)B * sizeof(int32_t), hipMemcpyDeviceToHost, s));
       GN_HIP(hipMemcpyAsync(p.flags + 2 * ctx->max_batch, ctx->ws.uncert_alt2, (size_t)B * sizeof(int32_t), hipMemcpyDeviceToHost, s));
-    } else memset(p.flags + ctx->max_batch, 0, (size_t)2 * ctx->max_batch * sizeof(int32_t));
+      GN_HIP(hipMemcpyAsync(p.flags + 3 * ctx->max_batch, ctx->ws.uncert_alt3, (size_t)B * sizeof(int32_t), hipMemcpyDeviceToHost, s));
+    } else memset(p.flags + ctx->max_batch, 0, (size_t)3 * ctx->max_batch * sizeof(int32_t));
     GN_HIP(hipEventRecord(p.ev, s));
-    p.active = true; p.level = ffn_auto(ctx) ? ctx->auto_level : -1; p.npad_run = ctx->npad_run;
+    p.active = true; p.level = ffn_auto(ctx) ? ffn_auto_state(ctx) : -1; p.npad_run = ctx->npad_run;
     p.call = v;
     if (K9) { memcpy(p.K9, K9, sizeof p.K9); p.call.K9 = p.K9; }
     ctx->cert_slot ^= 1;
@@ -2800,7 +2883,7 @@
   else if (which == 23) ctx->attn_split = value;
   else if (which == 25) ctx->dbg_trip_group = value;
   else if (which == 26) ctx->sub_serial = value;
-  else if (which == 27) ctx->qkv_products = value == 3 ? 3 : 2;
+  else if (which == 27) { ctx->qkv_products = value == 3 ? 3 : 2; if (value == 1) ctx->qkv_set = 1; ctx->fused_proj_pending = true; }
   else if (which == 28) ctx->ffn_compose = value;
   else if (which == 31) ctx->use_lists = value;
   else if (which == 32) ctx->qkv_in_tail = value ? 1 : 0;
diff --git a/gisnav_amd/csrc/gn_common.h b/gisnav_amd/csrc/gn_common.h
--- a/gisnav_amd/csrc/gn_common.h
+++ b/gisnav_amd/csrc/gn_common.h
@@ -260,6 +260,8 @@
   float cert_eps_alt = -1.f;
   int32_t* uncert_alt2 = nullptr;
   float cert_eps_alt2 = -1.f;
+  int32_t* uncert_alt3 = nullptr;
+  float cert_eps_alt3 = -1.f;
   float* colbest = nullptr;
   float* col2 = nullptr;
   const int32_t* n_in = nullptr;
diff --git a/gisnav_amd/csrc/gn_ffn128.hip b/gisnav_amd/csrc/gn_ffn128.hip
--- a/gisnav_amd/csrc/gn_ffn128.hip
+++ b/gisnav_amd/csrc/gn_ffn128.hip
@@ -695,11 +695,14 @@
   }
   ovf_commit(a.ovf, amax2);
   if constexpr (QKV != 0) {
-    constexpr bool CROSS = QKV == 2;
+    static_assert(QKV < 3 || PROD == 1, "the one-product projection exists beside the one-product tail only");
+    constexpr bool CROSS = QKV == 2 || QKV == 4;
+    constexpr bool Q1 = QKV >= 3;
+    constexpr int QPL = Q1 ? 1 : 2;
     constexpr int NPASS = CROSS ? 2 : 3;
     constexpr int NQK = CROSS ? kDim : 2 * kDim;
     constexpr int ROT = 8 * KT;
-    constexpr int RQ = 4;
+    constexpr int RQ = Q1 ? 8 : 4;
     const int slot = bm / a.npad, i0 = bm - slot * a.npad;
     f32x4 rq[CROSS ? 1 : 8];
     if constexpr (!CROSS) {
@@ -727,7 +730,7 @@
     }
     window(0);
     window(1);
-    f16x8 qa[RQ][2][2];
+    f16x8 qa[RQ][2][QPL];
     f16x8 qb[3][2];
     auto read_q = [&](int gp) __attribute__((always_inline)) {
       const int ks = gp >> 1, jp = gp & 1;
@@ -749,7 +752,7 @@
 #pragma unroll
         for (int i2 = 0; i2 < 2; ++i2)
 #pragma unroll
-          for (int pl = 0; pl < 2; ++pl) load_q(q, q, i2, pl);
+          for (int pl = 0; pl < QPL; ++pl) load_q(q, q, i2, pl);
       f32x4 bias4[2][4];
       if (!vpass) {
 #pragma unroll
@@ -779,11 +782,15 @@
             for (int jl = 0; jl < 2; ++jl)
 #pragma unroll
               for (int i2 = 0; i2 < 2; ++i2) {
-                const int j = 2 * jp + jl, m = 8 * jp + 4 * p + 2 * jl + i2;
-                const f16x8 w = qa[ks % RQ][i2][p == 0 ? 1 : 0], x = qb[gp % 3][jl];
+                if (Q1 && p == 0) continue;
+                const int j = 2 * jp + jl, m = Q1 ? 4 * jp + 2 * jl + i2 : 8 * jp + 4 * p + 2 * jl + i2;
+                const f16x8 w = qa[ks % RQ][i2][(p == 0 && QPL == 2) ? 1 : 0], x = qb[gp % 3][jl];
                 qacc[i2][j] = vpass ? __builtin_amdgcn_mfma_f32_32x32x16_f16(x, w, qacc[i2][j], 0, 0, 0)
                                     : __builtin_amdgcn_mfma_f32_32x32x16_f16(w, x, qacc[i2][j], 0, 0, 0);
-                if (m % 4 == 1 && ks >= 1 && ks + RQ - 1 < 16) load_q((ks - 1) % RQ, ks + RQ - 1, (m / 4) >> 1, (m / 4) & 1);
+                if (m % 4 == 1 && ks >= 1 && ks + RQ - 1 < 16) {
+                  if (Q1) load_q((ks - 1) % RQ, ks + RQ - 1, m / 4, 0);
+                  else load_q((ks - 1) % RQ, ks + RQ - 1, (m / 4) >> 1, (m / 4) & 1);
+                }
                 GN_PIN();
               }
         }
@@ -877,7 +884,9 @@
 #define GN_F1(Q) do { if (stamps == 8) hipLaunchKernelGGL((k_ffn128<8, true, false, 0, 1>), grid, block, 0, s, b); \
                       else if (walk) hipLaunchKernelGGL((k_ffn128<0, true, true, Q, 1>), grid, block, 0, s, b); \
                       else hipLaunchKernelGGL((k_ffn128<0, true, false, Q, 1>), grid, block, 0, s, b); } while (0)
-  if (qv == 1) { GN_F1(1); g_last_kernel = walk ? "k_ffn128<0, true, true, 1, 1>" : "k_ffn128<0, true, false, 1, 1>"; }
+  if (qv == 3) { GN_F1(3); g_last_kernel = walk ? "k_ffn128<0, true, true, 3, 1>" : "k_ffn128<0, true, false, 3, 1>"; }
+  else if (qv == 4) { GN_F1(4); g_last_kernel = walk ? "k_ffn128<0, true, true, 4, 1>" : "k_ffn128<0, true, false, 4, 1>"; }
+  else if (qv == 1) { GN_F1(1); g_last_kernel = walk ? "k_ffn128<0, true, true, 1, 1>" : "k_ffn128<0, true, false, 1, 1>"; }
   else if (qv == 2) { GN_F1(2); g_last_kernel = walk ? "k_ffn128<0, true, true, 2, 1>" : "k_ffn128<0, true, false, 2, 1>"; }
   else { GN_F1(0); g_last_kernel = walk ? "k_ffn128<0, true, true, 0, 1>" : "k_ffn128<0, true, false, 0, 1>"; }
 #undef GN_F1
diff --git a/gisnav_amd/csrc/gn_match_head.hip b/gisnav_amd/csrc/gn_match_head.hip
--- a/gisnav_amd/csrc/gn_match_head.hip
+++ b/gisnav_amd/csrc/gn_match_head.hip
@@ -131,12 +131,13 @@
   __syncthreads();
   const bool nomatch = (a.n_in ? a.n_in[2 * b] : n0) < 2 || (a.n_in ? a.n_in[2 * b + 1] : n1) < 2 || n0 < 1 || n1 < 1;
   if (nomatch || (a.ovf != nullptr && *a.ovf != 0u)) {
-    if (tid == 0) { a.n_match[b] = 0; if (a.uncert) a.uncert[b] = nomatch ? 0 : 2; if (a.uncert_alt) a.uncert_alt[b] = 0; if (a.uncert_alt2) a.uncert_alt2[b] = 0; }
+    if (tid == 0) { a.n_match[b] = 0; if (a.uncert) a.uncert[b] = nomatch ? 0 : 2; if (a.uncert_alt) a.uncert_alt[b] = 0; if (a.uncert_alt2) a.uncert_alt2[b] = 0; if (a.uncert_alt3) a.uncert_alt3[b] = 0; }
     return;
   }
   if (tid == 0 && a.uncert) a.uncert[b] = 1;
   if (tid == 0 && a.uncert_alt) a.uncert_alt[b] = 1;
   if (tid == 0 && a.uncert_alt2) a.uncert_alt2[b] = 1;
+  if (tid == 0 && a.uncert_alt3) a.uncert_alt3[b] = 1;
   for (int i0 = 0; i0 < n0; i0 += 256) {
     const int i = i0 + tid;
     bool valid = false; int j = 0; float sc = 0.f;
@@ -463,7 +464,8 @@
   const bool cert2 = cert && a.uncert_alt != nullptr && a.cert_eps_alt >= 0.f;
   const float Lth = a.threshold > 0.f ? logf(a.threshold) : -INFINITY;
   const bool cert3 = cert && a.uncert_alt2 != nullptr && a.cert_eps_alt2 >= 0.f;
-  int unc = 0, unc2 = 0, unc3 = 0;
+  const bool cert4 = cert && a.uncert_alt3 != nullptr && a.cert_eps_alt3 >= 0.f;
+  int unc = 0, unc2 = 0, unc3 = 0, unc4 = 0;
   for (int j = tid; j < n1; j += 512) {
     float m = -INFINITY, sm = 0.f; int bi = 0x7fffffff; float m2 = -INFINITY;
     for (int p0 = 0; p0 < nparts; p0 += 16) {
@@ -492,6 +494,7 @@
       if (cert && m >= Lth - a.cert_eps && !(m - m2 > 2.f * a.cert_eps)) unc = 1;
       if (cert2 && m >= Lth - a.cert_eps_alt && !(m - m2 > 2.f * a.cert_eps_alt)) unc2 = 1;
       if (cert3 && m >= Lth - a.cert_eps_alt2 && !(m - m2 > 2.f * a.cert_eps_alt2)) unc3 = 1;
+      if (cert4 && m >= Lth - a.cert_eps_alt3 && !(m - m2 > 2.f * a.cert_eps_alt3)) unc4 = 1;
     }
   }
   stamp(5);
@@ -503,7 +506,7 @@
   if (tid == 0) *base_s = 0;
   __syncthreads();
   if (nomatch || (a.ovf != nullptr && *a.ovf != 0u)) {
-    if (tid == 0) { a.n_match[b] = 0; if (a.uncert) a.uncert[b] = nomatch ? 0 : 2; if (a.uncert_alt) a.uncert_alt[b] = 0; if (a.uncert_alt2) a.uncert_alt2[b] = 0; }
+    if (tid == 0) { a.n_match[b] = 0; if (a.uncert) a.uncert[b] = nomatch ? 0 : 2; if (a.uncert_alt) a.uncert_alt[b] = 0; if (a.uncert_alt2) a.uncert_alt2[b] = 0; if (a.uncert_alt3) a.uncert_alt3[b] = 0; }
     return;
   }
   for (int ib = 0; ib < n0; ib += 512) {
@@ -520,6 +523,7 @@
         if (fabsf(best - Lth) <= a.cert_eps) unc = 1;
         if (cert2 && ((best >= Lth - a.cert_eps_alt && !(best - second > 2.f * a.cert_eps_alt)) || fabsf(best - Lth) <= a.cert_eps_alt)) unc2 = 1;
         if (cert3 && ((best >= Lth - a.cert_eps_alt2 && !(best - second > 2.f * a.cert_eps_alt2)) || fabsf(best - Lth) <= a.cert_eps_alt2)) unc3 = 1;
+        if (cert4 && ((best >= Lth - a.cert_eps_alt3 && !(best - second > 2.f * a.cert_eps_alt3)) || fabsf(best - Lth) <= a.cert_eps_alt3)) unc4 = 1;
       }
     }
     const unsigned long long bal = __ballot(valid);
@@ -548,6 +552,10 @@
     if (a.uncert_alt2) {
       const int any3 = __syncthreads_or(unc3);
       if (tid == 0) a.uncert_alt2[b] = (cert3 && any3) ? 1 : 0;
+    }
+    if (a.uncert_alt3) {
+      const int any4 = __syncthreads_or(unc4);
+      if (tid == 0) a.uncert_alt3[b] = (cert4 && any4) ? 1 : 0;
     }
   }
   stamp(6);
diff --git a/gisnav_amd/csrc/gn_qkv.hip b/gisnav_amd/csrc/gn_qkv.hip
--- a/gisnav_amd/csrc/gn_qkv.hip
+++ b/gisnav_amd/csrc/gn_qkv.hip
@@ -55,8 +55,9 @@
         fb[buf][j][pl] = *reinterpret_cast<const f16x8*>(smem + (ks >> 1) * KT + brow[j] + (((4 * (ks & 1) + 2 * pl + hh) ^ bsw[j]) * 16));
   };
   const uint4* const wf = reinterpret_cast<const uint4*>(a.wf) + lane;
-  constexpr int RA = CROSS ? 8 : 6;
-  f16x8 fa[RA][2];
+  constexpr int NPL = NP == 1 ? 1 : 2;
+  constexpr int RA = (CROSS ? 8 : 6) * (2 / NPL);
+  f16x8 fa[RA][NPL];
   const float ascale = a.acc_scale;
   const int slot = bm / a.npad, i0 = bm - slot * a.npad;
   __syncthreads();
@@ -70,7 +71,7 @@
     const int tile = 8 * pass + wave;
     auto load_a = [&](int slot_, int ks) __attribute__((always_inline)) {
 #pragma unroll
-      for (int pl = 0; pl < 2; ++pl) fa[slot_][pl] = __builtin_bit_cast(f16x8, wf[(size_t)((tile * 16 + ks) * 2 + pl) * 64]);
+      for (int pl = 0; pl < NPL; ++pl) fa[slot_][pl] = __builtin_bit_cast(f16x8, wf[(size_t)((tile * 16 + ks) * 2 + pl) * 64]);
     };
 #pragma unroll
     for (int q = 0; q < RA; ++q) load_a(q, q);
@@ -89,7 +90,8 @@
 #pragma unroll
         for (int j = 0; j < NJ; ++j) {
           if (NP == 2 && p == 1) continue;
-          const f16x8 w = fa[rs][p == 0 ? 1 : 0], x = fb[cb][j][p == 1 ? 1 : 0];
+          if (NP == 1 && p != 2) continue;
+          const f16x8 w = fa[rs][(p == 0 && NPL == 2) ? 1 : 0], x = fb[cb][j][p == 1 ? 1 : 0];
           acc[j] = vpass ? __builtin_amdgcn_mfma_f32_32x32x16_f16(x, w, acc[j], 0, 0, 0)
                          : __builtin_amdgcn_mfma_f32_32x32x16_f16(w, x, acc[j], 0, 0, 0);
         }
@@ -201,6 +203,11 @@
 void launch_qkv(const QkvArgs& a, bool cross, hipStream_t s) {
   const int ncu = a.ncu > 0 ? a.ncu : device_cu_count();
   const dim3 grid(a.tiles != nullptr ? std::min(a.T / TM, ncu) : a.T / TM), block(512);
+  if (a.products == 1) {
+    if (cross) { hipLaunchKernelGGL((k_qkv<true, true, 1>), grid, block, 0, s, a); g_last_kernel = "k_qkv<true, true, 1>"; }
+    else { hipLaunchKernelGGL((k_qkv<false, true, 1>), grid, block, 0, s, a); g_last_kernel = "k_qkv<false, true, 1>"; }
+    return;
+  }
   const int sel = (a.half_fmt ? 4 : 0) | (cross ? 2 : 0) | (a.products == 2 ? 1 : 0);
   switch (sel) {
     case 7: hipLaunchKernelGGL((k_qkv<true, true, 2>), grid, block, 0, s, a); g_last_kernel = "k_qkv<true, true, 2>"; break;
diff --git a/gisnav_amd/engine.py b/gisnav_amd/engine.py
--- a/gisnav_amd/engine.py
+++ b/gisnav_amd/engine.py
@@ -289,6 +289,13 @@
         self._ffn_auto = p == 0
         _lib.check(self.ctx, self.lib.gn_set_ffn_products(self.ctx, p), "gn_set_ffn_products")
 
+    def set_qkv_products(self, products) -> None:
+        p = 0 if products in ("auto", 0) else int(products)
+        _lib.check(self.ctx, self.lib.gn_set_qkv_products(self.ctx, p), "gn_set_qkv_products")
+
+    def set_qkv_level_eps(self, eps_projection: float) -> None:
+        _lib.check(self.ctx, self.lib.gn_set_qkv_level_eps(self.ctx, float(eps_projection)), "gn_set_qkv_level_eps")
+
     def set_ffn_level_eps(self, eps_two: float, eps_three: float, level: int = 3, eps_one: Optional[float] = None) -> None:
         if eps_one is not None:
             _lib.check(self.ctx, self.lib.gn_set_ffn_level_eps1(self.ctx, float(eps_one)), "gn_set_ffn_level_eps1")
@@ -299,9 +306,13 @@
         _lib.check(self.ctx, self.lib.gn_get_ffn_level(self.ctx, C.byref(lvl), C.byref(e2), C.byref(e3), buf), "gn_get_ffn_level")
         e1, c1 = C.c_float(0.0), C.c_int64(0)
         _lib.check(self.ctx, self.lib.gn_get_ffn_level1(self.ctx, C.byref(e1), C.byref(c1)), "gn_get_ffn_level1")
+        qs, qr, e0, c0 = C.c_int32(0), C.c_int32(0), C.c_float(0.0), C.c_int64(0)
+        _lib.check(self.ctx, self.lib.gn_get_qkv_level(self.ctx, C.byref(qs), C.byref(qr), C.byref(e0), C.byref(c0)), "gn_get_qkv_level")
         return {"level": int(lvl.value), "eps_two_products": float(e2.value), "eps_three_products": float(e3.value), "eps_one_product": float(e1.value),
                 "calls_two_products": int(buf[0]), "calls_three_products": int(buf[1]), "calls_one_product": int(c1.value),
-                "switches": int(buf[2]), "automatic": bool(buf[3])}
+                "switches": int(buf[2]), "automatic": bool(buf[3]),
+                "eps_one_product_projection": float(e0.value), "calls_projection_one_product": int(c0.value), "projection_one_product": bool(qr.value),
+                "qkv_products_setting": int(qs.value)}
 
     def calibrate_certify(self, inputs: dict, safety: float = 4.0, floor_eps: float = 1.0e-5) -> Dict[str, float]:
         B = inputs["kpt_q"].shape[0]
@@ -318,6 +329,7 @@
         if getattr(self, "_ffn_auto", False):
             d["eps_two_products"], d["eps_three_products"] = lv["eps_two_products"], lv["eps_three_products"]
             d["eps_one_product"] = lv["eps_one_product"]
+            d["eps_one_product_projection"] = lv["eps_one_product_projection"]
         return d
 
     def set_certify_ladder(self, enable: bool, eps_mid: Optional[float] = None) -> None:
diff --git a/include/gisnav_amd.h b/include/gisnav_amd.h
--- a/include/gisnav_amd.h
+++ b/include/gisnav_amd.h
@@ -48,6 +48,11 @@
 int gn_get_ffn_level1(gn_ctx* ctx, float* eps1, int64_t* calls1);
 int gn_set_ffn_level_eps1(gn_ctx* ctx, float eps1);
 int gn_debug_ffn_level_sim(int n_calls, int B, const int32_t* f1, const int32_t* f2, const int32_t* f3, int have1, int32_t* levels_out, int64_t* out4);
+int gn_set_qkv_products(gn_ctx* ctx, int products);
+int gn_get_qkv_level(gn_ctx* ctx, int32_t* setting, int32_t* on_rung, float* eps_proj1, int64_t* calls_proj1);
+int gn_set_qkv_level_eps(gn_ctx* ctx, float eps_proj1);
+int gn_debug_ffn_level_sim_rung(int n_calls, int B, const int32_t* f0, const int32_t* f1, const int32_t* f2, const int32_t* f3, int have1, int have0,
+                                int32_t* levels_out, int32_t* rung_out, int64_t* out5);
 int gn_fused_projection_status(const gn_ctx* ctx);
 int gn_device_numa_node(int device);
 int gn_get_certify_stats(gn_ctx* ctx, int64_t* out8);
```
